# Nightmare-n/GD-MAE

Hardware: AMD Instinct MI355X
Metric: MAE pre-train frames/sec (Waymo-shape, 180k pts, 75% mask) (higher is better)
Workload: dtype bf16

## Files before the change

### gd-mae_amd/csrc/chamfer.hip

```cpp
#include "common.h"

struct GtParams {
  float lo[3], vs[3];
  int ncols;
  int K;
};

__global__ __launch_bounds__(256) void k_group_gt(const float* __restrict__ pts, const int* __restrict__ pt_off,
                                                  const int* __restrict__ csr, const long long* __restrict__ voxel_coords,
                                                  int M, GtParams P, float* __restrict__ gt, int* __restrict__ gidx) {
  const int lane = threadIdx.x & (GD_WAVE - 1);
  const int wib = threadIdx.x / GD_WAVE;
  for (int p = blockIdx.x * 4 + wib; p < M; p += gridDim.x * 4) {
    const int off = pt_off[p];
    const int cnt = pt_off[p + 1] - off;
    const long long* vc = voxel_coords + 4ll * p;
    const float cx = __fadd_rn(__fmul_rn(__fadd_rn((float)vc[3], 0.5f), P.vs[0]), P.lo[0]);
    const float cy = __fadd_rn(__fmul_rn(__fadd_rn((float)vc[2], 0.5f), P.vs[1]), P.lo[1]);
    const float cz = __fadd_rn(__fmul_rn(__fadd_rn((float)vc[1], 0.5f), P.vs[2]), P.lo[2]);
    for (int k = lane; k < P.K; k += GD_WAVE) {
      const int src = k < cnt ? k : k % cnt;
      const int pid = csr[off + src];
      const float* r = pts + (long long)pid * P.ncols;
      float* o = gt + ((long long)p * P.K + k) * 3;
      o[0] = __fsub_rn(r[1], cx);
      o[1] = __fsub_rn(r[2], cy);
      o[2] = __fsub_rn(r[3], cz);
      if (gidx) gidx[(long long)p * P.K + k] = pid;
    }
  }
}

extern "C" int gdmae_group_gt_points(const float* points, int n_cols, const int* pillar_pt_off, const int* pillar_pts,
                                     const long long* voxel_coords, int M, int K, const float* lo, const float* vs,
                                     float* gt_points, int* gt_index, void* stream) {
  if (M <= 0) return 0;
  GtParams P;
  for (int i = 0; i < 3; ++i) {
    P.lo[i] = lo[i];
    P.vs[i] = vs[i];
  }
  P.ncols = n_cols;
  P.K = K;
  int grid = gd_div_up(M, 4);
  if (grid > 8192) grid = 8192;
  hipLaunchKernelGGL(k_group_gt, dim3(grid), dim3(256), 0, (hipStream_t)stream, points, pillar_pt_off, pillar_pts,
                     voxel_coords, M, P, gt_points, gt_index);
  GD_LAUNCH_CHECK();
  return 0;
}

template <int P1MAX>
__global__ __launch_bounds__(256) void k_chamfer(const float* __restrict__ pred, const float* __restrict__ gt,
                                                 const float* __restrict__ w, int M, int P1, int P2,
                                                 float* __restrict__ term, float* __restrict__ dpred) {
  __shared__ float sx[4][P1MAX * 3];
  const int lane = threadIdx.x & (GD_WAVE - 1);
  const int wib = threadIdx.x / GD_WAVE;
  for (int m = blockIdx.x * 4 + wib; m < M; m += gridDim.x * 4) {
    const float wm = w[m];
    float* dp = dpred + (long long)m * P1 * 3;
    if (wm == 0.f) {
      for (int e = lane; e < P1 * 3; e += GD_WAVE) dp[e] = 0.f;
      if (lane == 0) term[m] = 0.f;
      continue;
    }
    for (int e = lane; e < P1 * 3; e += GD_WAVE) sx[wib][e] = pred[(long long)m * P1 * 3 + e];
    __builtin_amdgcn_wave_barrier();
    const bool has = lane < P2;
    float y0 = 0.f, y1 = 0.f, y2 = 0.f;
    if (has) {
      const float* g = gt + ((long long)m * P2 + lane) * 3;
      y0 = g[0];
      y1 = g[1];
      y2 = g[2];
    }
    float best = INFINITY;
    int besti = 0;
    float sumx = 0.f;
    const float cx = wm / (float)P1, cy = wm / (float)P2;
    for (int i = 0; i < P1; ++i) {
      const float x0 = sx[wib][3 * i], x1 = sx[wib][3 * i + 1], x2 = sx[wib][3 * i + 2];
      const float d0 = x0 - y0, d1 = x1 - y1, d2 = x2 - y2;
      const float d = has ? (d0 * d0 + d1 * d1 + d2 * d2) : INFINITY;
      if (d < best) {
        best = d;
        besti = i;
      }
      const float dmin = gd_wave_min(d);
      const unsigned long long bal = __ballot(d == dmin);
      const int jstar = __ffsll((long long)bal) - 1;
      sumx += dmin;
      const float g0 = 2.f * cx * __shfl(d0, jstar, GD_WAVE);
      const float g1 = 2.f * cx * __shfl(d1, jstar, GD_WAVE);
      const float g2 = 2.f * cx * __shfl(d2, jstar, GD_WAVE);
      if (lane == 0) {
        dp[3 * i] = g0;
        dp[3 * i + 1] = g1;
        dp[3 * i + 2] = g2;
      }
    }
    const float sumy = gd_wave_sum(has ? best : 0.f);
    if (lane == 0) term[m] = cx * sumx + cy * sumy;
    __builtin_amdgcn_fence(__ATOMIC_RELEASE, "workgroup");
    for (int i = 0; i < P1; ++i) {
      const bool mine = has && besti == i;
      const float x0 = sx[wib][3 * i], x1 = sx[wib][3 * i + 1], x2 = sx[wib][3 * i + 2];
      const float a0 = gd_wave_sum(mine ? 2.f * cy * (x0 - y0) : 0.f);
      const float a1 = gd_wave_sum(mine ? 2.f * cy * (x1 - y1) : 0.f);
      const float a2 = gd_wave_sum(mine ? 2.f * cy * (x2 - y2) : 0.f);
      if (lane == 0) {
        dp[3 * i] += a0;
        dp[3 * i + 1] += a1;
        dp[3 * i + 2] += a2;
      }
    }
    __builtin_amdgcn_wave_barrier();
  }
}

template <int N>
__device__ __forceinline__ void ch_tstep(unsigned long long (&k)[16], int mask, int lane) {
  const bool hi = (lane & mask) != 0;
#pragma unroll
  for (int t = 0; t < N; ++t) {
    const unsigned long long send = hi ? k[t] : k[t + N];
    const unsigned long long keep = hi ? k[t + N] : k[t];
    const unsigned long long recv = __shfl_xor(send, mask, GD_WAVE);
    k[t] = keep < recv ? keep : recv;
  }
}

__global__ __launch_bounds__(256) void k_chamfer16(const float* __restrict__ pred, const float* __restrict__ gt,
                                                   const float* __restrict__ w, int M, int P2, float* __restrict__ term,
                                                   float* __restrict__ dpred) {
  __shared__ float sx[4][48];
  __shared__ float sy[4][GD_WAVE * 3];
  __shared__ int sb[4][GD_WAVE];
  __shared__ float sg[4][48];
  const int lane = threadIdx.x & (GD_WAVE - 1);
  const int wib = threadIdx.x / GD_WAVE;
  const int my_i = ((lane >> 5) & 1) * 8 + ((lane >> 4) & 1) * 4 + ((lane >> 3) & 1) * 2 + ((lane >> 2) & 1);
  for (int m = blockIdx.x * 4 + wib; m < M; m += gridDim.x * 4) {
    const float wm = w[m];
    float* dp = dpred + (long long)m * 48;
    if (wm == 0.f) {
      if (lane < 48) dp[lane] = 0.f;
      if (lane == 0) term[m] = 0.f;
      continue;
    }
    if (lane < 48) sx[wib][lane] = pred[(long long)m * 48 + lane];
    const bool has = lane < P2;
    float y0 = 0.f, y1 = 0.f, y2 = 0.f;
    if (has) {
      const float* g = gt + ((long long)m * P2 + lane) * 3;
      y0 = g[0];
      y1 = g[1];
      y2 = g[2];
    }
    __builtin_amdgcn_wave_barrier();
    const float cx = wm / 16.f, cy = wm / (float)P2;
    unsigned long long k[16];
    float best = INFINITY;
    int besti = 0;
#pragma unroll
    for (int i = 0; i < 16; ++i) {
      const float d0 = sx[wib][3 * i] - y0, d1 = sx[wib][3 * i + 1] - y1, d2 = sx[wib][3 * i + 2] - y2;
      const float d = has ? (d0 * d0 + d1 * d1 + d2 * d2) : INFINITY;
      if (d < best) {
        best = d;
        besti = i;
      }
      k[i] = ((unsigned long long)__float_as_uint(d) << 32) | (unsigned)lane;
    }
    ch_tstep<8>(k, 32, lane);
    ch_tstep<4>(k, 16, lane);
    ch_tstep<2>(k, 8, lane);
    ch_tstep<1>(k, 4, lane);
    unsigned long long k0 = k[0];
    {
      unsigned long long o = __shfl_xor(k0, 2, GD_WAVE);
      k0 = k0 < o ? k0 : o;
      o = __shfl_xor(k0, 1, GD_WAVE);
      k0 = k0 < o ? k0 : o;
    }
    const float dmin = __uint_as_float((unsigned)(k0 >> 32));
    const int jstar = (int)(k0 & 63u);
    const float ys0 = __shfl(y0, jstar, GD_WAVE), ys1 = __shfl(y1, jstar, GD_WAVE), ys2 = __shfl(y2, jstar, GD_WAVE);
    if ((lane & 3) == 0) {
      sg[wib][3 * my_i] = 2.f * cx * (sx[wib][3 * my_i] - ys0);
      sg[wib][3 * my_i + 1] = 2.f * cx * (sx[wib][3 * my_i + 1] - ys1);
      sg[wib][3 * my_i + 2] = 2.f * cx * (sx[wib][3 * my_i + 2] - ys2);
    }
    const float sumx = gd_wave_sum((lane & 3) == 0 ? dmin : 0.f);
    const float sumy = gd_wave_sum(has ? best : 0.f);
    if (lane == 0) term[m] = cx * sumx + cy * sumy;
    sy[wib][3 * lane] = y0;
    sy[wib][3 * lane + 1] = y1;
    sy[wib][3 * lane + 2] = y2;
    sb[wib][lane] = has ? besti : -1;
    __builtin_amdgcn_fence(__ATOMIC_RELEASE, "workgroup");
    __builtin_amdgcn_wave_barrier();
    if (lane < 48) {
      const int i = lane / 3, c = lane - 3 * i;
      const float xi = sx[wib][lane];
      float acc = 0.f;
      for (int j = 0; j < P2; ++j) {
        const float v = 2.f * cy * (xi - sy[wib][3 * j + c]);
        acc += sb[wib][j] == i ? v : 0.f;
      }
      dp[lane] = sg[wib][lane] + acc;
    }
    __builtin_amdgcn_wave_barrier();
  }
}

extern "C" int gdmae_chamfer(const float* pred, const float* gt, const float* weights, int M, int P1, int P2, float* term,
                             float* dpred, void* stream) {
  if (M <= 0) return 0;
  GD_REQUIRE(P2 >= 1 && P2 <= GD_WAVE, "NUM_GT_POINTS must be <= 64 (one lane per ground-truth point)");
  GD_REQUIRE(P1 >= 1 && P1 <= 64, "NUM_PRD_POINTS must be <= 64");
  int grid = gd_div_up(M, 4);
  if (grid > 8192) grid = 8192;
  if (P1 == 16)
    hipLaunchKernelGGL(k_chamfer16, dim3(grid), dim3(256), 0, (hipStream_t)stream, pred, gt, weights, M, P2, term, dpred);
  else
    hipLaunchKernelGGL((k_chamfer<64>), dim3(grid), dim3(256), 0, (hipStream_t)stream, pred, gt, weights, M, P1, P2, term,
                       dpred);
  GD_LAUNCH_CHECK();
  return 0;
}
```

### gd-mae_amd/csrc/conv_tiles.hip

```cpp
#include "conv_tiles.h"

typedef float f32x16 __attribute__((ext_vector_type(16)));
typedef __bf16 bf16x8 __attribute__((ext_vector_type(8)));
typedef _Float16 f16x8 __attribute__((ext_vector_type(8)));
union CtFrag {
  uint4 q;
  bf16x8 v;
  f16x8 h;
};

#define CT_C 128
#define CT_SITE_PITCH 272
#ifndef CT_CH
#define CT_CH 128
#endif
#ifndef CT_RING
#define CT_RING 8
#endif
#define CT_HALVES (CT_C / CT_CH)
#define CT_KS (CT_CH / 16)
#define CT_NSTEP (9 * CT_KS)
#define CT_CPS (CT_CH / 8)
#define CT_PSITE (CT_CH * 2 + 16)
#define CT_ROW_PITCH (CT_CH == 128 ? 2944 : 1664)
// ... 423 lines not shown
    const int r0 = blockIdx.x * chunk, r1 = r0 + chunk < n_act ? r0 + chunk : n_act;
    float a0 = 0.f, a1 = 0.f, a2 = 0.f, a3 = 0.f;
    int r = r0;
    for (; r + 15 < r1; r += 16) {
      float v[16];
#pragma unroll
      for (int u = 0; u < 16; ++u) v[u] = part[(long long)(r + u) * 256 + tid];
#pragma unroll
      for (int u = 0; u < 16; u += 4) {
        a0 += v[u];
        a1 += v[u + 1];
        a2 += v[u + 2];
        a3 += v[u + 3];
      }
    }
    for (; r + 3 < r1; r += 4) {
      a0 += part[(long long)r * 256 + tid];
      a1 += part[(long long)(r + 1) * 256 + tid];
      a2 += part[(long long)(r + 2) * 256 + tid];
      a3 += part[(long long)(r + 3) * 256 + tid];
    }
    for (; r < r1; ++r) a0 += part[(long long)r * 256 + tid];
    red[(long long)blockIdx.x * 256 + tid] = (a0 + a1) + (a2 + a3);
    return;
  }
  __shared__ int cnt[9];
  if (tid < 9) cnt[tid] = 0;
  __syncthreads();
  int c[9];
#pragma unroll
  for (int k = 0; k < 9; ++k) c[k] = 0;
  for (int i0 = tid; i0 < n_act; i0 += 8 * 256) {
   int tl[8];
#pragma unroll
   for (int u = 0; u < 8; ++u) tl[u] = tile_list[i0 + u * 256 < n_act ? i0 + u * 256 : n_act - 1];
#pragma unroll
   for (int u = 0; u < 8; ++u) {
    if (i0 + u * 256 >= n_act) continue;
    const int tile = tl[u];
    const int tx = tile % TW, ty = (tile / TW) % TH;
    const int y0 = ty * 8, y1 = y0 + 8 < H ? y0 + 8 : H, x0 = tx * 8, x1 = x0 + 8 < W ? x0 + 8 : W;
    const int ry[3] = {y0 == 0 ? 1 : 0, 0, y1 == H ? 1 : 0};
    const int rx[3] = {x0 == 0 ? 1 : 0, 0, x1 == W ? 1 : 0};
    const int my = (y1 - y0) - ry[0] - ry[2], mx = (x1 - x0) - rx[0] - rx[2];
#pragma unroll
    for (int cy = 0; cy < 3; ++cy)
#pragma unroll
      for (int cx = 0; cx < 3; ++cx) c[cy * 3 + cx] += (cy == 1 ? my : ry[cy]) * (cx == 1 ? mx : rx[cx]);
   }
  }
#pragma unroll
  for (int k = 0; k < 9; ++k)
    if (c[k]) atomicAdd(&cnt[k], c[k]);
  __syncthreads();
  const int stat = tid >> 7, ch = tid & 127;
  double acc = 0.0;
#pragma unroll
  for (int cy = 0; cy < 3; ++cy)
#pragma unroll
    for (int cx = 0; cx < 3; ++cx) {
      const long long total = (long long)B * (cy == 1 ? H - 2 : 1) * (cx == 1 ? W - 2 : 1);
      const double n = (double)(total - cnt[cy * 3 + cx]);
      const double v = (double)ct_bf2f(ybg[(cy * 3 + cx) * CT_C + ch]);
      acc += n * (stat ? v * v : v);
    }
  const float hi = (float)acc;
  red[(long long)CT_NRED * 256 + tid] = hi;
  red[(long long)(CT_NRED + 1) * 256 + tid] = (float)(acc - (double)hi);
}

int gd_bn_fold_from_partials(hipStream_t st, const float* part, int nblk, int C, double count, const float* gamma,
                             const float* beta, double eps, double momentum, float* running_mean, float* running_var,
                             long long* num_batches, double* stats, float* ab, float* mv);

extern "C" size_t gdmae_conv3x3_tiles_workspace_bytes(int n_act) {
  return gd_align((size_t)(n_act > 0 ? n_act : 1) * 256 * sizeof(float)) + gd_align((size_t)(CT_NRED + 2) * 256 * sizeof(float));
}

extern "C" int gdmae_conv3x3_tiles_fwd(const void* const* P, const int* const* maps, const float* const* a, const float* const* b,
                                       const int* strides, int k, const void* Wp, const void* ybg, const int* tile_list, int n_act,
                                       int B, int H, int W, void* Yc, const float* gamma, const float* beta, double eps,
                                       double momentum, float* running_mean, float* running_var, long long* num_batches,
                                       double* stats, float* ab, float* mv, void* workspace, void* stream) {
  GD_REQUIRE(k >= 1 && k <= CT_MAX_SRC, "conv3x3_tiles: 1..3 source stages");
  GD_REQUIRE(H >= 2 && W >= 2, "conv3x3_tiles: map too small");
  hipStream_t st = (hipStream_t)stream;
  CtArgs A;
  A.k = k;
  for (int g = 0; g < CT_MAX_SRC; ++g) {
    if (g < k) {
      const int s = strides[g];
      GD_REQUIRE((s == 1 || s == 2 || s == 4 || s == 8) && H % s == 0 && W % s == 0, "conv3x3_tiles: stride");
      A.src[g].P = (const unsigned short*)P[g];
      A.src[g].map = maps[g];
      A.src[g].a = a[g];
      A.src[g].b = b[g];
      A.src[g].ls = s == 1 ? 0 : (s == 2 ? 1 : (s == 4 ? 2 : 3));
    } else {
      A.src[g].P = nullptr; A.src[g].map = nullptr; A.src[g].a = nullptr; A.src[g].b = nullptr; A.src[g].ls = 0;
    }
  }
  A.Wp = (const uint4*)Wp;
  A.tile_list = tile_list;
  A.n_act = n_act;
  A.H = H; A.W = W; A.TH = (H + 7) / 8; A.TW = (W + 7) / 8;
  A.Yc = (unsigned short*)Yc;
  GdArena ar(workspace, gdmae_conv3x3_tiles_workspace_bytes(n_act));
  float* part = ar.take<float>((size_t)(n_act > 0 ? n_act : 1) * 256);
  float* red = ar.take<float>((size_t)(CT_NRED + 2) * 256);
  A.part = part;
  if (n_act > 0) {
    static bool once = false;
    if (!once) {
      GD_CHECK(hipFuncSetAttribute((const void*)k_conv3x3_tiles, hipFuncAttributeMaxDynamicSharedMemorySize, CT_LDS_BYTES));
      once = true;
    }
    hipLaunchKernelGGL(k_conv3x3_tiles, dim3((n_act + CT_TPW - 1) / CT_TPW), dim3(CT_THREADS), CT_LDS_BYTES, st, A);
    GD_LAUNCH_CHECK();
  }
  hipLaunchKernelGGL(k_ct_stats_reduce, dim3(CT_NRED + 1), dim3(256), 0, st, (const float*)part, n_act, tile_list,
                     (const unsigned short*)ybg, B, H, W, A.TH, A.TW, red);
  GD_LAUNCH_CHECK();
  return gd_bn_fold_from_partials(st, red, CT_NRED + 2, CT_C, (double)B * H * W, gamma, beta, eps, momentum, running_mean,
                                  running_var, num_batches, stats, ab, mv);
}

template <int ES>
__global__ __launch_bounds__(256) void k_tiles_gather_rows(const void* __restrict__ Yc, GdTiles T, const int* __restrict__ cell,
                                                           long long n, int H, int W, int C, uint4* __restrict__ out) {
  const int cv = C * ES / 16;
  const long long total = n * cv;
  for (long long i = blockIdx.x * (long long)blockDim.x + threadIdx.x; i < total; i += (long long)gridDim.x * blockDim.x) {
    const long long r = total < (1ll << 31) ? (long long)((unsigned)i / (unsigned)cv) : i / cv;
    const int v = (int)(i - r * cv);
    const int s = cell[r];
    const int x = s % W, q = s / W, y = q % H, b = q / H;
    out[i] = ((const uint4*)gd_y_row<ES>(Yc, T, b, y, x, H, W, C))[v];
  }
}

extern "C" int gdmae_tiles_gather_rows(const void* Yc, const int* tile_slot, const void* ybg, const int* cell, long long n, int H,
                                       int W, int C, int elem_bytes, void* out, void* stream) {
  GD_REQUIRE(tile_slot != nullptr && (elem_bytes == 2 || elem_bytes == 4) && (C * elem_bytes) % 16 == 0, "tiles_gather_rows");
  if (n <= 0) return 0;
  GdTiles T{tile_slot, ybg, (H + 7) / 8, (W + 7) / 8};
  long long g = (n * (C * elem_bytes / 16) + 255) / 256;
  if (g > 16384) g = 16384;
  if (elem_bytes == 2) hipLaunchKernelGGL(k_tiles_gather_rows<2>, dim3((int)g), dim3(256), 0, (hipStream_t)stream, Yc, T, cell, n, H, W, C, (uint4*)out);
  else hipLaunchKernelGGL(k_tiles_gather_rows<4>, dim3((int)g), dim3(256), 0, (hipStream_t)stream, Yc, T, cell, n, H, W, C, (uint4*)out);
  GD_LAUNCH_CHECK();
  return 0;
}

template <int ES>
__global__ __launch_bounds__(256) void k_tiles_to_dense(const void* __restrict__ Yc, GdTiles T, int B, int H, int W, int C,
                                                        uint4* __restrict__ out) {
  const int cv = C * ES / 16;
  const long long total = (long long)B * H * W * cv;
  for (long long i = blockIdx.x * (long long)blockDim.x + threadIdx.x; i < total; i += (long long)gridDim.x * blockDim.x) {
    const long long s = i / cv;
    const int v = (int)(i % cv);
    const int x = (int)(s % W);
    const long long q = s / W;
    const int y = (int)(q % H), b = (int)(q / H);
    out[i] = ((const uint4*)gd_y_row<ES>(Yc, T, b, y, x, H, W, C))[v];
  }
}

__global__ __launch_bounds__(256) void k_tiles_to_dense_affine_relu(const void* __restrict__ Yc, GdTiles T, int B, int H, int W, int C,
                                                                    const float* __restrict__ a, const float* __restrict__ bsh,
                                                                    float* __restrict__ out) {
  const int cv = C / 8;
  const long long total = (long long)B * H * W * cv;
  const unsigned total32 = (unsigned)total, ucv = (unsigned)cv, uW = (unsigned)W, uH = (unsigned)H;
  for (unsigned i = blockIdx.x * blockDim.x + threadIdx.x; i < total32; i += gridDim.x * blockDim.x) {
    const unsigned s32 = i / ucv;
    const int v = (int)(i - s32 * ucv);
    const unsigned q32 = s32 / uW;
    const int x = (int)(s32 - q32 * uW);
    const unsigned b32 = q32 / uH;
    const int y = (int)(q32 - b32 * uH), b = (int)b32;
    const long long s = s32;
    const uint4 u = ((const uint4*)gd_y_row<2>(Yc, T, b, y, x, H, W, C))[v];
    float f[8];
    ct_unpack8(u, f);
    const float4 a0 = *(const float4*)(a + 8 * v), a1 = *(const float4*)(a + 8 * v + 4);
    const float4 b0 = *(const float4*)(bsh + 8 * v), b1 = *(const float4*)(bsh + 8 * v + 4);
    float4 o0, o1;
    o0.x = fmaxf(fmaf(a0.x, f[0], b0.x), 0.f); o0.y = fmaxf(fmaf(a0.y, f[1], b0.y), 0.f);
    o0.z = fmaxf(fmaf(a0.z, f[2], b0.z), 0.f); o0.w = fmaxf(fmaf(a0.w, f[3], b0.w), 0.f);
    o1.x = fmaxf(fmaf(a1.x, f[4], b1.x), 0.f); o1.y = fmaxf(fmaf(a1.y, f[5], b1.y), 0.f);
    o1.z = fmaxf(fmaf(a1.z, f[6], b1.z), 0.f); o1.w = fmaxf(fmaf(a1.w, f[7], b1.w), 0.f);
    typedef float f4v __attribute__((ext_vector_type(4)));
    __builtin_nontemporal_store(f4v{o0.x, o0.y, o0.z, o0.w}, (f4v*)(out + s * C + 8 * v));
    __builtin_nontemporal_store(f4v{o1.x, o1.y, o1.z, o1.w}, (f4v*)(out + s * C + 8 * v + 4));
  }
}

extern "C" int gdmae_tiles_to_dense_affine_relu(const void* Yc, const int* tile_slot, const void* ybg, int B, int H, int W, int C, const float* a,
                                                const float* b, float* out, void* stream) {
  GD_REQUIRE(tile_slot != nullptr && C % 8 == 0 && a != nullptr && b != nullptr, "tiles_to_dense_affine_relu");
  GD_REQUIRE((long long)B * H * W * (C / 8) < (1ll << 31), "tiles_to_dense_affine_relu: B H W C / 8 must fit 31 bits");
  GdTiles T{tile_slot, ybg, (H + 7) / 8, (W + 7) / 8};
  hipLaunchKernelGGL(k_tiles_to_dense_affine_relu, dim3(16384), dim3(256), 0, (hipStream_t)stream, Yc, T, B, H, W, C, a, b, out);
  GD_LAUNCH_CHECK();
  return 0;
}

extern "C" int gdmae_tiles_to_dense(const void* Yc, const int* tile_slot, const void* ybg, int B, int H, int W, int C, int elem_bytes,
                                    void* out, void* stream) {
  GD_REQUIRE(tile_slot != nullptr && (elem_bytes == 2 || elem_bytes == 4) && (C * elem_bytes) % 16 == 0, "tiles_to_dense");
  GdTiles T{tile_slot, ybg, (H + 7) / 8, (W + 7) / 8};
  if (elem_bytes == 2) hipLaunchKernelGGL(k_tiles_to_dense<2>, dim3(16384), dim3(256), 0, (hipStream_t)stream, Yc, T, B, H, W, C, (uint4*)out);
  else hipLaunchKernelGGL(k_tiles_to_dense<4>, dim3(16384), dim3(256), 0, (hipStream_t)stream, Yc, T, B, H, W, C, (uint4*)out);
  GD_LAUNCH_CHECK();
  return 0;
}
```

### gd-mae_amd/csrc/decoder.hip

```cpp
#include "common.h"
#include "conv_tiles.h"

__device__ inline float dec_bf2f(unsigned short h) { return __uint_as_float(((unsigned)h) << 16); }
__device__ inline unsigned short dec_f2bf(float f) { return gd_to_bf16(f); }
template <bool BF>
__device__ inline float dec_ld(const void* p, long long i) {
  return BF ? dec_bf2f(((const unsigned short*)p)[i]) : ((const float*)p)[i];
}
template <bool BF>
__device__ inline void dec_st(void* p, long long i, float v) {
  if (BF) ((unsigned short*)p)[i] = dec_f2bf(v);
  else ((float*)p)[i] = v;
}

template <bool BF>
__device__ inline void dec_ld8(const void* p, long long i, float (&v)[8]) {
  if (BF) {
    const uint4 q = *reinterpret_cast<const uint4*>((const unsigned short*)p + i);
    const unsigned w[4] = {q.x, q.y, q.z, q.w};
#pragma unroll
    for (int j = 0; j < 4; ++j) {
      v[2 * j] = __uint_as_float(w[j] << 16);
      v[2 * j + 1] = __uint_as_float(w[j] & 0xFFFF0000u);
    }
// ... 504 lines not shown
    ia[j] = fabsf(av[j]) >= 1e-30f ? 1.f / av[j] : 0.f;
  }
  for (long long p = r0 + tr; p < r1; p += rows_per_iter) {
    const long long q = p * C + c;
    float ov[8], gv[8];
    dec_ld8<false>(out, q, ov);
    dec_ld8<false>(dout, q, gv);
#pragma unroll
    for (int j = 0; j < 8; ++j)
      if (ov[j] > 0.f) {
        const float xr = (ov[j] - bv[j]) * ia[j];
        const bool recon = ia[j] != 0.f && (fabsf(bv[j]) + ov[j]) * fabsf(ia[j]) <= GD_SEGMAX_RECON_ULPS * fabsf(xr);
        const float xv = recon ? xr : dec_ld<XBF>(x, (long long)arg[q + j] * C + c + j);
        s0[j] += gv[j];
        s1[j] = fmaf(gv[j], xv, s1[j]);
      }
  }
#pragma unroll
  for (int j = 0; j < 8; ++j) {
    sh[(tr * 2 + 0) * C + c + j] = s0[j];
    sh[(tr * 2 + 1) * C + c + j] = s1[j];
  }
  __syncthreads();
  for (int q = threadIdx.x; q < 2 * C; q += 256) {
    float acc = 0.f;
    for (int rr = 0; rr < rows_per_iter; ++rr) acc += sh[rr * 2 * C + q];
    part[(long long)blockIdx.x * 2 * C + q] = acc;
  }
}

extern "C" int gdmae_segmax_bwd_stats(const void* x, int x_bf16, const float* out, const int* arg, const float* dout,
                                      long long M, int C, const float* a, const float* b,
                                      double* sums , void* workspace, void* stream) {
  GD_REQUIRE(C >= 1 && C <= 256, "C <= 256");
  hipStream_t st = (hipStream_t)stream;
  int nblk = (int)(M / 32 > 512 ? 512 : (M / 32 > 0 ? M / 32 : 1));
  const int rpi = 256 / C > 0 ? 256 / C : 1;
  const size_t lds = (size_t)rpi * 2 * C * sizeof(float);
  float* part = (float*)workspace;
  if (a && b && C % 8 == 0 && 256 % (C / 8) == 0) {
    const size_t lds8 = (size_t)(256 / (C / 8)) * 2 * C * sizeof(float);
    if (x_bf16)
      hipLaunchKernelGGL((k_segmax_bwd_stats_v8<true>), dim3(nblk), dim3(256), lds8, st, x, out, arg, dout, M, C, a, b, part);
    else
      hipLaunchKernelGGL((k_segmax_bwd_stats_v8<false>), dim3(nblk), dim3(256), lds8, st, x, out, arg, dout, M, C, a, b, part);
  } else if (x_bf16)
    hipLaunchKernelGGL((k_segmax_bwd_stats<true>), dim3(nblk), dim3(256), lds, st, x, out, arg, dout, M, C, part);
  else
    hipLaunchKernelGGL((k_segmax_bwd_stats<false>), dim3(nblk), dim3(256), lds, st, x, out, arg, dout, M, C, part);
  GD_LAUNCH_CHECK();
  hipLaunchKernelGGL(k_partials_to_f64, dim3(gd_div_up(2 * C, 16)), dim3(256), 0, st, part, nblk, 2 * C, sums);
  GD_LAUNCH_CHECK();
  return 0;
}

extern "C" int gdmae_segmax_bn_bwd(const void* x, int x_bf16, const float* out, const int* arg, const float* dout,
                                   const int* inverse32, long long N, int C, const float* a, const float* c0, const float* c1,
                                   void* dx, int dx_bf16, void* stream) {
  if (N <= 0) return 0;
  hipStream_t st = (hipStream_t)stream;
  const dim3 grid(dec_grid(N * C)), block(256);
  const bool v8 = C % 8 == 0;
  const dim3 grid8(dec_grid(N * C / 8));
#define GD_SB(XB, OB)                                                                                                              \
  do {                                                                                                                             \
    if (v8) hipLaunchKernelGGL((k_segmax_bn_bwd_v8<XB, OB>), grid8, block, 0, st, x, out, arg, dout, inverse32, N, C, a, c0, c1, dx); \
    else hipLaunchKernelGGL((k_segmax_bn_bwd<XB, OB>), grid, block, 0, st, x, out, arg, dout, inverse32, N, C, a, c0, c1, dx);      \
  } while (0)
  if (x_bf16) { if (dx_bf16) GD_SB(true, true); else GD_SB(true, false); }
  else { if (dx_bf16) GD_SB(false, true); else GD_SB(false, false); }
#undef GD_SB
  GD_LAUNCH_CHECK();
  return 0;
}

template <bool BF>
__global__ __launch_bounds__(256) void k_conv_grad_taps(const void* __restrict__ Ymap, GdTiles T, const float* __restrict__ k0,
                                                        const float* __restrict__ k1, const float* __restrict__ rows,
                                                        const int* __restrict__ cell2pillar, const int* __restrict__ site,
                                                        long long n, int H, int W, int C, void* __restrict__ out) {
  const int cv = C >> 3;
  const long long total = n * 9 * cv;
  for (long long i = blockIdx.x * (long long)blockDim.x + threadIdx.x; i < total; i += (long long)gridDim.x * blockDim.x) {
    const int v = (int)(i % cv);
    const long long tk = i / cv;
    const int k = (int)(tk % 9);
    const long long t = tk / 9;
    const int s = site[t];
    const int x = s % W;
    const int r = s / W;
    const int y = r % H;
    const int uy = y - (k / 3 - 1), ux = x - (k % 3 - 1);
    float o[8];
#pragma unroll
    for (int j = 0; j < 8; ++j) o[j] = 0.f;
    if (uy >= 0 && uy < H && ux >= 0 && ux < W) {
      const long long u = (long long)(r - y + uy) * W + ux;
      const int c0 = v * 8;
      float yv[8];
      const char* yrow = gd_y_row<BF ? 2 : 4>(Ymap, T, (r - y) / H, uy, ux, H, W, C);
      if (BF) {
        const uint4 q = ((const uint4*)yrow)[c0 >> 3];
        const unsigned w4[4] = {q.x, q.y, q.z, q.w};
#pragma unroll
        for (int j = 0; j < 4; ++j) {
          yv[2 * j] = __uint_as_float(w4[j] << 16);
          yv[2 * j + 1] = __uint_as_float(w4[j] & 0xFFFF0000u);
        }
      } else {
        const float4 q0 = ((const float4*)yrow)[c0 >> 2], q1 = ((const float4*)yrow)[(c0 >> 2) + 1];
        yv[0] = q0.x; yv[1] = q0.y; yv[2] = q0.z; yv[3] = q0.w; yv[4] = q1.x; yv[5] = q1.y; yv[6] = q1.z; yv[7] = q1.w;
      }
      const float4 ka = ((const float4*)k0)[c0 >> 2], kb = ((const float4*)k0)[(c0 >> 2) + 1];
      const float4 la = ((const float4*)k1)[c0 >> 2], lb = ((const float4*)k1)[(c0 >> 2) + 1];
      const float kk0[8] = {ka.x, ka.y, ka.z, ka.w, kb.x, kb.y, kb.z, kb.w};
      const float kk1[8] = {la.x, la.y, la.z, la.w, lb.x, lb.y, lb.z, lb.w};
#pragma unroll
      for (int j = 0; j < 8; ++j) o[j] = fmaf(kk1[j], yv[j], kk0[j]);
      const int p = cell2pillar[u];
      if (p >= 0) {
        const float4 r0 = ((const float4*)rows)[((long long)p * C + c0) >> 2], r1 = ((const float4*)rows)[(((long long)p * C + c0) >> 2) + 1];
        o[0] += r0.x; o[1] += r0.y; o[2] += r0.z; o[3] += r0.w; o[4] += r1.x; o[5] += r1.y; o[6] += r1.z; o[7] += r1.w;
      }
    }
    if (BF) {
      uint4 q;
      q.x = dec_f2bf(o[0]) | ((unsigned)dec_f2bf(o[1]) << 16);
      q.y = dec_f2bf(o[2]) | ((unsigned)dec_f2bf(o[3]) << 16);
      q.z = dec_f2bf(o[4]) | ((unsigned)dec_f2bf(o[5]) << 16);
      q.w = dec_f2bf(o[6]) | ((unsigned)dec_f2bf(o[7]) << 16);
      ((uint4*)out)[i] = q;
    } else {
      ((float4*)out)[2 * i] = make_float4(o[0], o[1], o[2], o[3]);
      ((float4*)out)[2 * i + 1] = make_float4(o[4], o[5], o[6], o[7]);
    }
  }
}

extern "C" int gdmae_conv3x3_grad_taps(const void* Ymap, int y_bf16, const int* tile_slot, const void* ybg, const float* k0,
                                       const float* k1, const float* rows, const int* cell2pillar, const int* site, long long n,
                                       int H, int W, int C, void* out, void* stream) {
  GD_REQUIRE(C % 8 == 0, "C must be a multiple of 8");
  if (n <= 0) return 0;
  long long g = (n * 9 * (C / 8) + 255) / 256;
  if (g > 65536) g = 65536;
  const GdTiles T{tile_slot, ybg, (H + 7) / 8, (W + 7) / 8};
  if (y_bf16) hipLaunchKernelGGL(k_conv_grad_taps<true>, dim3((int)g), dim3(256), 0, (hipStream_t)stream, Ymap, T, k0, k1, rows, cell2pillar, site, n, H, W, C, out);
  else hipLaunchKernelGGL(k_conv_grad_taps<false>, dim3((int)g), dim3(256), 0, (hipStream_t)stream, Ymap, T, k0, k1, rows, cell2pillar, site, n, H, W, C, out);
  GD_LAUNCH_CHECK();
  return 0;
}

#define DEC_BORDER_CHUNKS 64
template <bool BF>
__global__ __launch_bounds__(256) void k_border_partial(const void* __restrict__ Y, GdTiles T, const float* __restrict__ rows,
                                                        const int* __restrict__ pillar_cell, int M, int B, int H, int W, int C,
                                                        float* __restrict__ part_edge, float* __restrict__ part_rows) {
  extern __shared__ float sh[];
  const int cv = C >> 3;
  if ((int)blockIdx.x < 4 * B) {
    const int e = blockIdx.x / B, b = blockIdx.x % B;
    const int len = e < 2 ? W : H;
    const int slots = 256 / cv;
    const int tr = threadIdx.x / cv, c = (threadIdx.x % cv) << 3;
    float acc[8];
#pragma unroll
    for (int j = 0; j < 8; ++j) acc[j] = 0.f;
    if (tr < slots)
      for (int i0 = tr; i0 < len; i0 += 4 * slots) {
        float v[4][8];
#pragma unroll
        for (int u = 0; u < 4; ++u) {
          const int i = i0 + u * slots < len ? i0 + u * slots : len - 1;
          const int y = e == 0 ? 0 : (e == 1 ? H - 1 : i);
          const int x = e == 2 ? 0 : (e == 3 ? W - 1 : i);
          dec_ld8<BF>(gd_y_row<BF ? 2 : 4>(Y, T, b, y, x, H, W, C), c, v[u]);
        }
#pragma unroll
        for (int u = 0; u < 4; ++u) {
          const bool ok = i0 + u * slots < len;
#pragma unroll
          for (int j = 0; j < 8; ++j) acc[j] = ok ? acc[j] + v[u][j] : acc[j];
        }
      }
    if (tr < slots) {
#pragma unroll
      for (int j = 0; j < 8; ++j) sh[tr * C + c + j] = acc[j];
    }
    __syncthreads();
    for (int q = threadIdx.x; q < C; q += 256) {
      float s = 0.f;
      for (int r = 0; r < slots; ++r) s += sh[r * C + q];
      part_edge[(long long)blockIdx.x * C + q] = s;
    }
    return;
  }
  const int lane = threadIdx.x & 63;
  const int bb = (int)blockIdx.x - 4 * B;
  const int chunk = bb >> 1;
  const int reg = (bb & 1) * 4 + (threadIdx.x >> 6);
  const int per = ((M + DEC_BORDER_CHUNKS - 1) / DEC_BORDER_CHUNKS + 63) / 64 * 64;
  const int pb = chunk * per, pe = pb + per < M ? pb + per : M;
  float acc[4] = {0.f, 0.f, 0.f, 0.f};
  for (int p0 = pb; p0 < pe; p0 += 64) {
    const int p = p0 + lane;
    bool in = false;
    if (p < pe) {
      const int cell = pillar_cell[p];
      const int x = cell % W, y = (cell / W) % H;
      const bool y0 = y == 0, yl = y == H - 1, x0 = x == 0, xl = x == W - 1;
      in = reg == 0 ? y0 : reg == 1 ? yl : reg == 2 ? x0 : reg == 3 ? xl : reg == 4 ? (y0 && x0) : reg == 5 ? (y0 && xl)
                                                                         : reg == 6 ? (yl && x0) : (yl && xl);
    }
    unsigned long long m = __ballot(in);
    while (m) {
      const int k = __ffsll((long long)m) - 1;
      m &= m - 1;
      const float* rp = rows + (long long)(p0 + k) * C;
#pragma unroll
      for (int j = 0; j < 4; ++j)
        if (lane + 64 * j < C) acc[j] += rp[lane + 64 * j];
    }
  }
#pragma unroll
  for (int j = 0; j < 4; ++j)
    if (lane + 64 * j < C) part_rows[((long long)chunk * 8 + reg) * C + lane + 64 * j] = acc[j];
}

template <bool BF>
__global__ __launch_bounds__(256) void k_border_final(const void* __restrict__ Y, GdTiles T, const float* __restrict__ part_edge,
                                                      const float* __restrict__ part_rows, int B, int H, int W, int C,
                                                      double* __restrict__ out) {
  for (int q = blockIdx.x * blockDim.x + threadIdx.x; q < 8 * C; q += gridDim.x * blockDim.x) {
    const int r = q / C, c = q % C;
    double s = 0.0;
    if (r < 4) {
      for (int b = 0; b < B; ++b) s += (double)part_edge[(long long)(r * B + b) * C + c];
    } else {
      const int y = (r == 4 || r == 5) ? 0 : H - 1, x = (r == 4 || r == 6) ? 0 : W - 1;
      for (int b = 0; b < B; ++b) s += (double)dec_ld<BF>(gd_y_row<BF ? 2 : 4>(Y, T, b, y, x, H, W, C), c);
    }
    out[q] = s;
    double t = 0.0;
    for (int ch = 0; ch < DEC_BORDER_CHUNKS; ++ch) t += (double)part_rows[(long long)ch * 8 * C + q];
    out[8 * C + q] = t;
  }
}

extern "C" size_t gdmae_border_sums_workspace_bytes(int B, int C) {
  return (size_t)(4 * B + 8 * DEC_BORDER_CHUNKS) * C * sizeof(float);
}

extern "C" int gdmae_border_sums(const void* Y, int y_bf16, const int* tile_slot, const void* ybg, const float* rows,
                                 const int* pillar_cell, int M, int B, int H, int W, int C, double* out ,
                                 void* workspace, void* stream) {
  const GdTiles T{tile_slot, ybg, (H + 7) / 8, (W + 7) / 8};
  GD_REQUIRE(C % 8 == 0 && C <= 256 && 256 % (C / 8) == 0, "border_sums: C in {64, 128, 256}");
  hipStream_t st = (hipStream_t)stream;
  float* part_edge = (float*)workspace;
  float* part_rows = part_edge + (size_t)4 * B * C;
  const size_t lds = (size_t)(256 / (C / 8)) * C * sizeof(float);
  if (y_bf16) hipLaunchKernelGGL((k_border_partial<true>), dim3(4 * B + 2 * DEC_BORDER_CHUNKS), dim3(256), lds, st, Y, T, rows, pillar_cell, M, B, H, W, C, part_edge, part_rows);
  else hipLaunchKernelGGL((k_border_partial<false>), dim3(4 * B + 2 * DEC_BORDER_CHUNKS), dim3(256), lds, st, Y, T, rows, pillar_cell, M, B, H, W, C, part_edge, part_rows);
  GD_LAUNCH_CHECK();
  if (y_bf16) hipLaunchKernelGGL((k_border_final<true>), dim3(gd_div_up(8 * C, 256)), dim3(256), 0, st, Y, T, part_edge, part_rows, B, H, W, C, out);
  else hipLaunchKernelGGL((k_border_final<false>), dim3(gd_div_up(8 * C, 256)), dim3(256), 0, st, Y, T, part_edge, part_rows, B, H, W, C, out);
  GD_LAUNCH_CHECK();
  return 0;
}

__global__ __launch_bounds__(256) void k_dec_region_S(const double* __restrict__ stats2, const float* __restrict__ ab2,
                                                      const double* __restrict__ st2, const float* __restrict__ k01,
                                                      const double* __restrict__ reg, const double* __restrict__ tap_region,
                                                      const double* __restrict__ cnt, double R, int C2, double* __restrict__ S) {
  const int o = blockIdx.x * blockDim.x + threadIdx.x;
  if (o >= C2) return;
  const double k0 = (double)k01[o], k1 = (double)k01[C2 + o];
  double regD[9];
#pragma unroll
  for (int r = 0; r < 9; ++r) {
    const double y = r == 0 ? stats2[o] * R : reg[(r - 1) * C2 + o];
    const double rr = r == 0 ? (double)ab2[o] * st2[o] : reg[(8 + r - 1) * C2 + o];
    regD[r] = cnt[r] * k0 + y * k1 + rr;
  }
#pragma unroll
  for (int k = 0; k < 9; ++k) {
    double a = 0.0;
#pragma unroll
    for (int r = 0; r < 9; ++r) a += tap_region[k * 9 + r] * regD[r];
    S[k * C2 + o] = a;
  }
}

template <bool BF>
__global__ __launch_bounds__(128) void k_dec_region_W(const double* __restrict__ S, const float* __restrict__ conv_w,
                                                      const void* __restrict__ bgz, int C2, int Cin, float* __restrict__ dWk,
                                                      void* __restrict__ Wd, double* __restrict__ tot_part) {
  const int i = blockIdx.x * 128 + threadIdx.x, oc = blockIdx.y * 8;
  if (i >= Cin) return;
  const double bg = (double)dec_ld<BF>(bgz, i);
  double acc = 0.0;
  for (int oo = 0; oo < 8; ++oo) {
    const int o = oc + oo;
    const float* w = conv_w + ((long long)o * Cin + i) * 9;
#pragma unroll
    for (int k = 0; k < 9; ++k) {
      const float wv = w[k];
      const double s = S[k * C2 + o];
      acc += s * (double)wv;
      const long long e = ((long long)k * C2 + o) * Cin + i;
      dWk[e] = (float)(s * bg);
      dec_st<BF>(Wd, e, wv);
    }
  }
  tot_part[(long long)blockIdx.y * Cin + i] = acc;
}

__global__ __launch_bounds__(256) void k_dec_region_tot(const double* __restrict__ tot_part, int nchunk, int Cin,
                                                        double* __restrict__ tot) {
  const int i = blockIdx.x * blockDim.x + threadIdx.x;
  if (i >= Cin) return;
  double a = 0.0;
  for (int c = 0; c < nchunk; ++c) a += tot_part[(long long)c * Cin + i];
  tot[i] = a;
}

extern "C" size_t gdmae_decoder_region_workspace_bytes(int C2, int Cin) { return (size_t)(C2 / 8 + 1) * Cin * sizeof(double); }

extern "C" int gdmae_decoder_region_algebra(const double* stats2, const float* ab2, const double* st2, const float* k01,
                                            const double* reg, const double* tap_region, const double* cnt, double R, int C2,
                                            int Cin, const float* conv_w, const void* bgz, int cdt_bf16, double* S, double* tot,
                                            float* dWk, void* Wd, void* workspace, void* stream) {
  GD_REQUIRE(C2 > 0 && C2 % 8 == 0 && Cin > 0, "decoder region algebra: C2 must be a multiple of 8");
  hipStream_t st = (hipStream_t)stream;
  hipLaunchKernelGGL(k_dec_region_S, dim3(gd_div_up(C2, 256)), dim3(256), 0, st, stats2, ab2, st2, k01, reg, tap_region, cnt, R, C2, S);
  GD_LAUNCH_CHECK();
  const dim3 grid(gd_div_up(Cin, 128), C2 / 8);
  double* part = (double*)workspace;
  if (cdt_bf16) hipLaunchKernelGGL((k_dec_region_W<true>), grid, dim3(128), 0, st, (const double*)S, conv_w, bgz, C2, Cin, dWk, Wd, part);
  else hipLaunchKernelGGL((k_dec_region_W<false>), grid, dim3(128), 0, st, (const double*)S, conv_w, bgz, C2, Cin, dWk, Wd, part);
  GD_LAUNCH_CHECK();
  hipLaunchKernelGGL(k_dec_region_tot, dim3(gd_div_up(Cin, 256)), dim3(256), 0, st, (const double*)part, C2 / 8, Cin, tot);
  GD_LAUNCH_CHECK();
  return 0;
}


__global__ __launch_bounds__(256) void k_decoder_dy(const unsigned short* __restrict__ Yc, const int* __restrict__ tile_list, int n_act,
                                                    const float* __restrict__ k0, const float* __restrict__ k1,
                                                    const float* __restrict__ rows, const int* __restrict__ cell2pillar, int H, int W,
                                                    int TH, int TW, int C, unsigned short* __restrict__ dYc) {
  const unsigned cv = (unsigned)C >> 3;
  const unsigned total = (unsigned)n_act * GD_TILE_SITES * cv;
  for (unsigned i = blockIdx.x * blockDim.x + threadIdx.x; i < total; i += gridDim.x * blockDim.x) {
    const unsigned row32 = i / cv;
    const int v = (int)(i - row32 * cv);
    const long long row = row32;
    const int slot = (int)(row32 >> 6), loc = (int)(row32 & 63);
    const int tile = tile_list[slot];
    const int tx = tile % TW, r = tile / TW, ty = r % TH, b = r / TH;
    const int y = ty * GD_TILE + (loc >> 3), x = tx * GD_TILE + (loc & 7);
    uint4 q = make_uint4(0u, 0u, 0u, 0u);
    if (y < H && x < W) {
      const int c0 = v * 8;
      const uint4 yq = reinterpret_cast<const uint4*>(Yc + row * C)[v];
      const unsigned w4[4] = {yq.x, yq.y, yq.z, yq.w};
      float yv[8], o[8];
#pragma unroll
      for (int j = 0; j < 4; ++j) {
        yv[2 * j] = __uint_as_float(w4[j] << 16);
        yv[2 * j + 1] = __uint_as_float(w4[j] & 0xFFFF0000u);
      }
      const float4 ka = ((const float4*)k0)[c0 >> 2], kb = ((const float4*)k0)[(c0 >> 2) + 1];
      const float4 la = ((const float4*)k1)[c0 >> 2], lb = ((const float4*)k1)[(c0 >> 2) + 1];
      const float kk0[8] = {ka.x, ka.y, ka.z, ka.w, kb.x, kb.y, kb.z, kb.w};
      const float kk1[8] = {la.x, la.y, la.z, la.w, lb.x, lb.y, lb.z, lb.w};
#pragma unroll
      for (int j = 0; j < 8; ++j) o[j] = fmaf(kk1[j], yv[j], kk0[j]);
      const int p = cell2pillar[((long long)b * H + y) * W + x];
      if (p >= 0) {
        const float4 r0 = ((const float4*)rows)[((long long)p * C + c0) >> 2], r1 = ((const float4*)rows)[(((long long)p * C + c0) >> 2) + 1];
        o[0] += r0.x; o[1] += r0.y; o[2] += r0.z; o[3] += r0.w; o[4] += r1.x; o[5] += r1.y; o[6] += r1.z; o[7] += r1.w;
      }
      q.x = dec_f2bf(o[0]) | ((unsigned)dec_f2bf(o[1]) << 16);
      q.y = dec_f2bf(o[2]) | ((unsigned)dec_f2bf(o[3]) << 16);
      q.z = dec_f2bf(o[4]) | ((unsigned)dec_f2bf(o[5]) << 16);
      q.w = dec_f2bf(o[6]) | ((unsigned)dec_f2bf(o[7]) << 16);
    }
    reinterpret_cast<uint4*>(dYc + row * C)[v] = q;
  }
}
extern "C" int gdmae_decoder_dy(const void* Yc, const int* tile_list, int n_act, const float* k0, const float* k1, const float* rows,
                                const int* cell2pillar, int H, int W, int C, void* dYc, void* stream) {
  GD_REQUIRE(C % 8 == 0, "decoder_dy: C must be a multiple of 8");
  if (n_act <= 0) return 0;
  GD_REQUIRE((long long)n_act * GD_TILE_SITES * (C / 8) < (1ll << 31), "decoder_dy: active tiles x 64 x C / 8 must fit 31 bits");
  long long g = ((long long)n_act * GD_TILE_SITES * (C / 8) + 255) / 256;
  if (g > 65536) g = 65536;
  hipLaunchKernelGGL(k_decoder_dy, dim3((int)g), dim3(256), 0, (hipStream_t)stream, (const unsigned short*)Yc, tile_list, n_act, k0, k1, rows,
                     cell2pillar, H, W, (H + 7) / 8, (W + 7) / 8, C, (unsigned short*)dYc);
  GD_LAUNCH_CHECK();
  return 0;
}

__global__ __launch_bounds__(256) void k_decoder_site_rulebook(const int* __restrict__ site, const int* __restrict__ n_dev, int sites_per_tok,
                                                               const int* __restrict__ tile_slot, int H, int W, int TH, int TW,
                                                               int* __restrict__ nbr) {
  const long long total = (long long)(*n_dev) * sites_per_tok * 9;
  for (long long i = blockIdx.x * (long long)blockDim.x + threadIdx.x; i < total; i += (long long)gridDim.x * blockDim.x) {
    const long long t = total < (1ll << 31) ? (long long)((unsigned)i / 9u) : i / 9;
    const int k = (int)(i - t * 9);
    const int s = site[t];
    const int x = s % W, r = s / W, y = r % H, b = r / H;
    const int uy = y - (k / 3 - 1), ux = x - (k % 3 - 1);
    int v = -1;
    if (uy >= 0 && uy < H && ux >= 0 && ux < W) {
      const int sl = tile_slot[(b * TH + (uy >> 3)) * TW + (ux >> 3)];
      if (sl >= 0) v = sl * GD_TILE_SITES + (uy & 7) * GD_TILE + (ux & 7);
    }
    nbr[i] = v;
  }
}
int gd_decoder_site_rulebook(const int* site, const int* n_dev, int sites_per_tok, long long cap_sites, const int* tile_slot, int H, int W,
                             int* nbr, hipStream_t st) {
  long long g = (cap_sites * 9 + 255) / 256;
  if (g > 4096) g = 4096;
  if (g < 1) g = 1;
  hipLaunchKernelGGL(k_decoder_site_rulebook, dim3((int)g), dim3(256), 0, st, site, n_dev, sites_per_tok, tile_slot, H, W, (H + 7) / 8,
                     (W + 7) / 8, nbr);
  GD_LAUNCH_CHECK();
  return 0;
}
extern "C" int gdmae_decoder_site_rulebook(const int* site, const int* n_dev, int sites_per_tok, long long cap_sites, const int* tile_slot,
                                           int H, int W, int* nbr, void* stream) {
  return gd_decoder_site_rulebook(site, n_dev, sites_per_tok, cap_sites, tile_slot, H, W, nbr, (hipStream_t)stream);
}
```

### gd-mae_amd/gdmae_hip/decoder.py

```python
from __future__ import annotations

import os
from collections import namedtuple
from dataclasses import dataclass
from types import SimpleNamespace
from typing import Optional

import torch
import torch.nn.functional as F

from . import bn as gbn
from . import lib as L
from . import ops, packing
from . import plan as gplan
from . import timing

CONV_BWD = os.environ.get("GDMAE_DEC_BWD", "implicit")
BLOCK_BWD = os.environ.get("GDMAE_DEC_BLOCK", "1")



def colstats(x2d: torch.Tensor):
    R, C = x2d.shape
    assert x2d.is_contiguous() and x2d.dtype in (torch.float32, torch.bfloat16)
    out = torch.empty(2 * C, dtype=torch.float64, device=x2d.device)
    ws = torch.empty(L.load().gdmae_colstats_workspace_bytes(C), dtype=torch.uint8, device=x2d.device)
    L.call("gdmae_colstats", L.ptr(x2d), R, C, int(x2d.dtype == torch.bfloat16), L.ptr(out), L.ptr(ws), L.stream())
    return out[:C], out[C:]


def _gather_slice(table2d, idx, col0, ncol):
    es = table2d.element_size()
    out = torch.empty(idx.numel(), ncol, dtype=table2d.dtype, device=table2d.device)
    L.call("gdmae_gather_rows_strided", L.ptr(table2d), L.ptr(idx), idx.numel(), ncol * es, table2d.shape[1] * es,
           col0 * es, L.ptr(out), L.stream())
    return out


def _scatter_slice(src2d, idx, table2d, col0):
    es = table2d.element_size()
    src2d = src2d.contiguous()
    assert src2d.dtype == table2d.dtype
    L.call("gdmae_scatter_rows_strided", L.ptr(src2d), L.ptr(idx), idx.numel(), src2d.shape[1] * es,
           table2d.shape[1] * es, col0 * es, L.ptr(table2d), L.stream())


def _bf(t):
    return int(t.dtype == torch.bfloat16)


_TAP_REGION = torch.zeros(9, 9, dtype=torch.float64)
for _ky in (-1, 0, 1):
    for _kx in (-1, 0, 1):
        _k = (_ky + 1) * 3 + (_kx + 1)
        _TAP_REGION[_k, 0] = 1
        if _ky:
            _TAP_REGION[_k, 1 if _ky < 0 else 2] = -1
        if _kx:
            _TAP_REGION[_k, 3 if _kx < 0 else 4] = -1
        if _ky and _kx:
            _TAP_REGION[_k, 5 + (0 if _ky < 0 else 2) + (0 if _kx < 0 else 1)] = 1


_REGION_CONSTS = {}


def _region_consts(dev, B, H, W):
    key = (dev, B, H, W)
    if key not in _REGION_CONSTS:
        R = B * H * W
        cnt = torch.tensor([R, B * W, B * W, B * H, B * H, B, B, B, B], dtype=torch.float64)
        _REGION_CONSTS[key] = (_TAP_REGION.to(dev), cnt.to(dev))
    return _REGION_CONSTS[key]


@dataclass(frozen=True, eq=False)
class TileConv:
    tiles: gplan.DecoderTiles
    maps: list
    ups: list


@dataclass(frozen=True, eq=False)
class DecoderGeom:
    B: int
    H: int
    W: int
    eps1: float
    eps2: float
    cdt: torch.dtype
    tile_conv: Optional[TileConv] = None


_Forward = namedtuple("_Forward", "y2 yrows stats2 ab2 mv2 Z tile_slot ybg bgz")


def _forward_tiles(geom, pre_conv_hook, conv_w, gamma2, beta2, pillar_cell, Ps, widths, ab_l, bn2):
    B, H, W, cdt, tc = geom.B, geom.H, geom.W, geom.cdt, geom.tile_conv
    dt, k, dev = tc.tiles, len(Ps), Ps[0].device
    lib = L.load()
    Cin = sum(widths)
    C2 = 128
    Wp = torch.empty(lib.gdmae_conv3x3_tiles_packed_bytes(k), dtype=torch.uint8, device=dev)
    bgz = torch.empty(Cin, dtype=cdt, device=dev)
    ybg = torch.empty(9, C2, dtype=cdt, device=dev)
    a_l, b_l = [ab[:w] for ab, w in zip(ab_l, widths)], [ab[w:] for ab, w in zip(ab_l, widths)]
    L.call("gdmae_conv3x3_tiles_pack", L.ptr(conv_w), C2, Cin, L.host_ptrs(b_l), k, L.ptr(Wp), L.ptr(bgz), L.ptr(ybg),
           L.stream())
    y2 = torch.empty(max(dt.n_act, 1) * 64, C2, dtype=cdt, device=dev)
    stats2 = torch.empty(2 * C2, dtype=torch.float64, device=dev)
    ab2 = torch.empty(2 * C2, dtype=torch.float32, device=dev)
    mv2 = torch.empty(2 * C2, dtype=torch.float32, device=dev)
    ws = torch.empty(lib.gdmae_conv3x3_tiles_workspace_bytes(dt.n_act), dtype=torch.uint8, device=dev)
    rm, rv, nb, mom = gbn.running_stats(bn2)
    flops = 2.0 * dt.n_act * 64 * C2 * 9 * Cin
    if pre_conv_hook is not None:
        pre_conv_hook()
    with timing.kernel("k_conv3x3_tiles", dt.n_act * 64 * (Cin + C2) * 2, flops,
                       {"dense_equivalent_TFLOPs_per_launch": round(2.0 * B * H * W * C2 * 9 * Cin / 1e12, 4), "active_tiles": dt.n_act}):
        L.call("gdmae_conv3x3_tiles_fwd", L.host_ptrs([P.contiguous() for P in Ps]), L.host_ptrs(tc.maps), L.host_ptrs(a_l),
               L.host_ptrs(b_l), L.host_i32(tc.ups), k, L.ptr(Wp), L.ptr(ybg), L.ptr(dt.tile_list), dt.n_act, B, H, W,
               L.ptr(y2), L.ptr(gamma2), L.ptr(beta2), float(geom.eps2), mom, L.ptr(rm), L.ptr(rv), L.ptr(nb), L.ptr(stats2),
               L.ptr(ab2), L.ptr(mv2), L.ptr(ws), L.stream())
    M = pillar_cell.numel()
    yrows = torch.empty(M, C2, dtype=cdt, device=dev)
    L.call("gdmae_tiles_gather_rows", L.ptr(y2), L.ptr(dt.tile_slot), L.ptr(ybg), L.ptr(pillar_cell), M, H, W, C2, 2,
           L.ptr(yrows), L.stream())
    return _Forward(y2, yrows, stats2, ab2, mv2, None, dt.tile_slot, ybg, bgz)


def _forward_dense_map(geom, conv_w, gamma2, beta2, pillar_cell, sites, Ps, widths, ab_l, bn2):
    B, H, W, cdt = geom.B, geom.H, geom.W, geom.cdt
    R = B * H * W
    bgz = torch.relu(torch.cat([ab[w:] for ab, w in zip(ab_l, widths)])).to(cdt)
    Z = torch.empty(R, sum(widths), dtype=cdt, device=Ps[0].device)
    L.call("gdmae_fill_rows", L.ptr(bgz), R, Z.shape[1], Z.element_size(), L.ptr(Z), L.stream())
    col = 0
    for P, st, ab, w in zip(Ps, sites, ab_l, widths):
        L.call("gdmae_rows_affine_relu_scatter", L.ptr(P), _bf(P), L.ptr(st), P.shape[0], w, L.ptr(ab), L.ptr(ab[w:]), L.ptr(Z), _bf(Z),
               Z.shape[1], col, L.stream())
        col += w
    from . import dense as gdense
    C2o = conv_w.shape[0]
    if cdt == torch.bfloat16 and Z.shape[1] % 64 == 0 and conv_w.dtype == torch.float32:
        y2 = gdense.Conv3x3Dense.apply(Z.view(B, H, W, -1).permute(0, 3, 1, 2), conv_w.detach(), None, 1, None).permute(0, 2, 3, 1)
    elif cdt == torch.float32 and Z.shape[1] % 64 == 0:
        y2 = gdense.conv3x3_f32_rows(Z.view(B, H, W, -1), conv_w.detach().float().contiguous(), None, 1)[..., :C2o]
    else:
        wc = ops.shadow(conv_w, cdt)
        with torch.autocast("cuda", enabled=False):
            y2 = F.conv2d(Z.view(B, H, W, -1).permute(0, 3, 1, 2), wc, None, 1, 1).permute(0, 2, 3, 1)
    if not y2.is_contiguous():
        y2 = y2.contiguous()
    y2 = y2.view(R, -1)
    stats2, ab2, mv2 = gbn.fold(y2, R, gamma2, beta2, geom.eps2, bn2)
    yrows = ops.gather_rows_raw(y2, pillar_cell)
    return _Forward(y2, yrows, stats2, ab2, mv2, Z, None, None, bgz)


def _backward_schedule(geom, conv_w, sites, Ps, widths, fwd):
    C2 = fwd.y2.shape[1]
    native = conv_w.dtype == torch.float32 and conv_w.is_contiguous() and C2 % 8 == 0
    tc = geom.tile_conv
    if not (CONV_BWD == "implicit" and fwd.tile_slot is not None and fwd.y2.dtype == torch.bfloat16 and native and C2 == 128
            and all(w == 128 for w in widths) and tc is not None):
        return native, ["taps"] * len(widths)
    stage_bwd = []
    for P, st, u in zip(Ps, sites, tc.ups):
        n, u = P.shape[0], int(u)
        block = (BLOCK_BWD != "0" and u in (2, 4) and P.dtype == torch.bfloat16 and P.is_contiguous() and st.numel() >= n
                 and int(L.load().gdmae_decoder_block_dw_workspace_bytes(n, u)) > 0)
        stage_bwd.append("block" if block else "rulebook")
    return native, stage_bwd


def _save(ctx, **named):
    ctx.saved_names = [(name, len(v) if isinstance(v, (list, tuple)) else None) for name, v in named.items()]
    ctx.save_for_backward(*[t for v in named.values() for t in (v if isinstance(v, (list, tuple)) else (v,))])


def _saved(ctx) -> SimpleNamespace:
    sv, out, j = ctx.saved_tensors, SimpleNamespace(), 0
    for name, n in ctx.saved_names:
        setattr(out, name, sv[j] if n is None else sv[j:j + n])
        j += 1 if n is None else n
    return out


def _bn2_backward(s, dout, R, direct):
    yrows, ab2 = s.yrows, s.ab2
    M, C2 = yrows.shape
    dev = yrows.device
    dout = dout.float().contiguous()
    st2 = torch.empty(3 * C2, dtype=torch.float64, device=dev)
    ws = torch.empty(L.load().gdmae_rows_bwd_stats_workspace_bytes(C2), dtype=torch.uint8, device=dev)
    L.call("gdmae_rows_bwd_stats", L.ptr(yrows), _bf(yrows), None, M, C2, L.ptr(ab2), L.ptr(ab2[C2:]), L.ptr(dout), 0, C2, 0,
           L.ptr(st2), L.ptr(ws), L.stream())
    dgamma2, dbeta2, k01 = gbn.bwd_coeffs(st2, 3, s.stats2, ab2, s.gamma2, R, None, direct)
    zero = torch.zeros(2 * C2, dtype=torch.float32, device=dev)
    rows = torch.empty(M, C2, dtype=torch.float32, device=dev)
    L.call("gdmae_rows_bwd", L.ptr(yrows), _bf(yrows), None, M, C2, L.ptr(ab2), L.ptr(ab2[C2:]), L.ptr(zero), L.ptr(zero[C2:]),
           L.ptr(dout), 0, C2, 0, L.ptr(rows), 0, L.stream())
    return rows, st2, k01, dgamma2, dbeta2


def _region_sums(s, rows, B, H, W):
    y2 = s.y2
    C2 = y2.shape[1]
    reg = torch.empty(16, C2, dtype=torch.float64, device=y2.device)
    ws = torch.empty(L.load().gdmae_border_sums_workspace_bytes(B, C2), dtype=torch.uint8, device=y2.device)
    L.call("gdmae_border_sums", L.ptr(y2), _bf(y2), L.ptr(s.tile_slot), L.ptr(s.ybg), L.ptr(rows), L.ptr(s.pillar_cell),
           rows.shape[0], B, H, W, C2, L.ptr(reg), L.ptr(ws), L.stream())
    return reg



def region_algebra_native(stats2, ab2, st2, k01, reg, tap_region, cnt, R, conv_w, bgz, cdt):
    C2, Cin, dev = conv_w.shape[0], bgz.numel(), conv_w.device
    S = torch.empty(9, C2, dtype=torch.float64, device=dev)
    tot = torch.empty(Cin, dtype=torch.float64, device=dev)
    dWk = torch.empty(9, C2, Cin, dtype=torch.float32, device=dev)
    Wd = torch.empty(9, C2, Cin, dtype=cdt, device=dev)
    ws = torch.empty(L.load().gdmae_decoder_region_workspace_bytes(C2, Cin), dtype=torch.uint8, device=dev)
    L.call("gdmae_decoder_region_algebra", L.ptr(stats2), L.ptr(ab2), L.ptr(st2), L.ptr(k01), L.ptr(reg),
           L.ptr(tap_region), L.ptr(cnt), float(R), C2, Cin, L.ptr(conv_w), L.ptr(bgz), _bf(Wd), L.ptr(S), L.ptr(tot),
           L.ptr(dWk), L.ptr(Wd), L.ptr(ws), L.stream())
    return S, tot, dWk, Wd


def region_algebra_torch(stats2, ab2, st2, k01, reg, tap_region, cnt, R, conv_w, bgz, cdt):
    C2, Cin = conv_w.shape[0], bgz.numel()
    k0, k1 = k01[:C2].double(), k01[C2:].double()
    regY = torch.cat([(stats2[:C2] * R)[None], reg[:8]])
    regR = torch.cat([(ab2[:C2].double() * st2[:C2])[None], reg[8:]])
    regD = cnt[:, None] * k0[None, :] + regY * k1[None, :] + regR
    S = tap_region @ regD
    Wk = conv_w.permute(2, 3, 0, 1).reshape(9, C2, Cin)
    tot = torch.einsum('ko,koi->i', S, Wk.double()).contiguous()
    dWk = (S[:, :, None] * bgz.double()[None, None, :]).to(torch.promote_types(torch.float32, conv_w.dtype))
    Wd = Wk.to(cdt)
    return S, tot, dWk, Wd


def _stage_dx_spconv(b, i, col):
    n, w, C2 = b.Ps[i].shape[0], b.widths[i], b.y2.shape[1]
    nbr = b.tiles.nbr[i]
    assert nbr.shape[0] == n, (nbr.shape, n)
    dX = torch.empty(n, w, dtype=b.cdt, device=b.y2.device)
    L.call("gdmae_spconv", L.ptr(b.dYc), 0, L.ptr(nbr), b.packed.data_ptr() + i * 9 * w * C2 * 2, n, C2, w, L.ptr(dX), 8, L.stream())
    return dX


def _stage_grads_block(b, i, col):
    dX = _stage_dx_spconv(b, i, col)
    P, ab, w, u = b.Ps[i], b.ab_l[i], b.widths[i], int(b.ups[i])
    n = P.shape[0]
    ws = torch.empty(int(L.load().gdmae_decoder_block_dw_workspace_bytes(n, u)), dtype=torch.uint8, device=P.device)
    L.call("gdmae_decoder_block_dw", L.ptr(P), L.ptr(ab), L.ptr(ab[w:]), L.ptr(b.bgz[col:col + w]), L.ptr(b.sites[i]), n, u, L.ptr(b.dYc),
           L.ptr(b.tile_slot), b.H, b.W, L.ptr(b.dWk), b.bgz.numel(), col, L.ptr(ws), L.stream())
    return dX, None


def _stage_grads_rulebook(b, i, col):
    dX = _stage_dx_spconv(b, i, col)
    P, ab, w, C2 = b.Ps[i], b.ab_l[i], b.widths[i], b.y2.shape[1]
    n = P.shape[0]
    n_pad = int(L.load().gdmae_tap_dw_rows(n, w, C2))
    Zd = torch.empty(n_pad, w, dtype=b.cdt, device=P.device)
    L.call("gdmae_rows_affine_relu_sub", L.ptr(P), _bf(P), None, n, w, L.ptr(ab), L.ptr(ab[w:]), L.ptr(b.bgz[col:col + w]), L.ptr(Zd),
           _bf(Zd), w, 0, L.stream())
    ws = torch.empty(L.load().gdmae_tap_dw_workspace_bytes(n, w, C2), dtype=torch.uint8, device=P.device)
    L.call("gdmae_tap_dw", L.ptr(Zd), n, n_pad, w, L.ptr(b.dYc), L.ptr(b.tiles.nbr[i]), C2, L.ptr(b.dWk), b.bgz.numel(), col, L.ptr(ws),
           L.stream())
    return dX, None


def _stage_grads_taps(b, i, col):
    P, ab, w, C2, cdt = b.Ps[i], b.ab_l[i], b.widths[i], b.y2.shape[1], b.cdt
    n, dev = P.shape[0], P.device
    G = torch.empty(n, 9 * C2, dtype=cdt, device=dev)
    with timing.kernel("k_conv_grad_taps", 2.0 * n * 9 * C2 * G.element_size()):
        L.call("gdmae_conv3x3_grad_taps", L.ptr(b.y2), _bf(b.y2), L.ptr(b.tile_slot), L.ptr(b.ybg), L.ptr(b.k01), L.ptr(b.k01[C2:]),
               L.ptr(b.rows), L.ptr(b.cell2pillar), L.ptr(b.sites[i]), n, b.H, b.W, C2, L.ptr(G), L.stream())
    dX = ops.mm(G, b.Wd[:, :, col:col + w].reshape(9 * C2, w))
    bg = b.bgz[col:col + w]
    if b.Z is not None:
        Zd = _gather_slice(b.Z, b.sites[i], col, w) - bg
    else:
        Zd = torch.empty(n, w, dtype=cdt, device=dev)
        L.call("gdmae_rows_affine_relu_sub", L.ptr(P), _bf(P), None, n, w, L.ptr(ab), L.ptr(ab[w:]), L.ptr(bg), L.ptr(Zd),
               _bf(Zd), w, 0, L.stream())
    return dX, ops.splitk_tn(G, Zd)


_STAGE_GRADS = {"block": _stage_grads_block, "rulebook": _stage_grads_rulebook, "taps": _stage_grads_taps}


def _stage_bn_backward(b, i, col, dX, R, direct):
    P, ab, w = b.Ps[i], b.ab_l[i], b.widths[i]
    n = P.shape[0]
    ws = torch.empty(L.load().gdmae_rows_bwd_stats_workspace_bytes(w), dtype=torch.uint8, device=P.device)
    L.call("gdmae_rows_bwd_stats", L.ptr(P), _bf(P), None, n, w, L.ptr(ab), L.ptr(ab[w:]), L.ptr(dX), _bf(dX), w, 0,
           None, L.ptr(ws), L.stream())
    dgamma, dbeta, c01 = gbn.bwd_coeffs((ws, L.load().gdmae_rows_bwd_stats_rows(n)), 3, b.stats_l[i], ab, b.gammas[i], R,
                                        b.tot[col:col + w], direct)
    dP = torch.empty_like(P)
    L.call("gdmae_rows_bwd", L.ptr(P), _bf(P), None, n, w, L.ptr(ab), L.ptr(ab[w:]), L.ptr(c01), L.ptr(c01[w:]), L.ptr(dX),
           _bf(dX), w, 0, L.ptr(dP), _bf(dP), L.stream())
    return dP, dgamma, dbeta


class DecoderHead(torch.autograd.Function):

    @staticmethod
    def forward(ctx, geom, pre_conv_hook, conv_w, gamma2, beta2, pillar_cell, cell2pillar, bn_mods, *args):
        R = geom.B * geom.H * geom.W
        k = len(args) // 4
        sites, Ps, gammas, betas = args[0::4], args[1::4], args[2::4], args[3::4]
        widths = [int(P.shape[1]) for P in Ps]
        bns = list(bn_mods) if bn_mods is not None else [None] * (k + 1)
        ab_l, stats_l, mv_out = [], [], []
        for i in range(k):
            stats, ab, mv = gbn.fold(Ps[i].contiguous(), R, gammas[i], betas[i], geom.eps1, bns[i])
            ab_l.append(ab), stats_l.append(stats)
            mv_out += [mv[:widths[i]], mv[widths[i]:]]
        use_tiles = (geom.tile_conv is not None and geom.cdt == torch.bfloat16 and all(w == 128 for w in widths) and conv_w.shape[0] == 128
                     and conv_w.dtype == torch.float32 and conv_w.is_contiguous() and all(P.dtype == torch.bfloat16 for P in Ps))
        if use_tiles:
            f = _forward_tiles(geom, pre_conv_hook, conv_w, gamma2, beta2, pillar_cell, Ps, widths, ab_l, bns[k])
        else:
            f = _forward_dense_map(geom, conv_w, gamma2, beta2, pillar_cell, sites, Ps, widths, ab_l, bns[k])
        M, C2 = f.yrows.shape
        out = torch.empty(M, C2, dtype=torch.float32, device=f.yrows.device)
        L.call("gdmae_rows_affine_relu_scatter", L.ptr(f.yrows), _bf(f.yrows), None, M, C2, L.ptr(f.ab2), L.ptr(f.ab2[C2:]), L.ptr(out), 0,
               C2, 0, L.stream())
        _save(ctx, sites=sites, Ps=Ps, ab_l=ab_l, stats_l=stats_l, gammas=[g.detach() for g in gammas], Z=f.Z, y2=f.y2, bgz=f.bgz,
              yrows=f.yrows, ab2=f.ab2, stats2=f.stats2, pillar_cell=pillar_cell, cell2pillar=cell2pillar, gamma2=gamma2.detach(),
              conv_w=conv_w.detach(), tile_slot=f.tile_slot, ybg=f.ybg)
        ctx.geom, ctx.widths = geom, widths
        ctx.native_region, ctx.stage_bwd = _backward_schedule(geom, conv_w, sites, Ps, widths, f)
        ctx.direct = [gbn.direct_pair(g, be) for g, be in zip(gammas, betas)] + [gbn.direct_pair(gamma2, beta2)]
        ctx.direct_w = ops.direct_grad(conv_w)
        ctx.conv_param = conv_w
        mean2, var2 = f.mv2[:C2], f.mv2[C2:]
        ctx.mark_non_differentiable(f.y2, mean2, var2, *mv_out, *([] if f.ybg is None else [f.ybg]))
        ctx.set_materialize_grads(False)
        return (out, f.y2, mean2, var2, *mv_out, f.ybg)

    @staticmethod
    def backward(ctx, dout, *_):
        geom, widths, stage_bwd = ctx.geom, ctx.widths, ctx.stage_bwd
        B, H, W = geom.B, geom.H, geom.W
        R, k = B * H * W, len(widths)
        b = _saved(ctx)
        b.H, b.W, b.cdt, b.widths = H, W, geom.cdt, widths
        b.rows, st2, b.k01, dgamma2, dbeta2 = _bn2_backward(b, dout, R, ctx.direct[k])
        reg = _region_sums(b, b.rows, B, H, W)
        tap_region, cnt = _region_consts(reg.device, B, H, W)
        algebra = region_algebra_native if ctx.native_region else region_algebra_torch
        S, b.tot, b.dWk, b.Wd = algebra(b.stats2, b.ab2, st2, b.k01, reg, tap_region, cnt, R, b.conv_w, b.bgz, geom.cdt)
        if stage_bwd[0] != "taps":
            b.packed = packing.decoder_conv_packed(ctx.conv_param, widths, ctx.direct_w is not None)
            if b.packed is None:
                stage_bwd = ["taps"] * k
            else:
                b.tiles, b.ups = geom.tile_conv.tiles, geom.tile_conv.ups
                if b.tiles.nbr is None:
                    b.tiles.nbr = gplan.decoder_site_rulebooks(b.tiles, b.sites, b.ups)
                C2 = b.y2.shape[1]
                b.dYc = torch.empty_like(b.y2)
                L.call("gdmae_decoder_dy", L.ptr(b.y2), L.ptr(b.tiles.tile_list), b.tiles.n_act, L.ptr(b.k01), L.ptr(b.k01[C2:]),
                       L.ptr(b.rows), L.ptr(b.cell2pillar), H, W, C2, L.ptr(b.dYc), L.stream())
        grads = [None] * 8
        dW_rows = []
        col = 0
        for i, w in enumerate(widths):
            dX, dW = _STAGE_GRADS[stage_bwd[i]](b, i, col)
            if dW is not None:
                dW_rows.append(dW)
            grads += [None, *_stage_bn_backward(b, i, col, dX, R, ctx.direct[i])]
            col += w
        dWk = b.dWk
        if dW_rows:
            dWk = dWk + torch.cat(dW_rows, dim=1).view(dWk.shape)
        dW = dWk.permute(1, 2, 0).reshape(b.conv_w.shape[0], b.conv_w.shape[1], 3, 3)
        if ctx.direct_w is not None:
            ctx.direct_w.add_(dW)
        else:
            grads[2] = dW.to(b.conv_w.dtype)
        grads[3], grads[4] = dgamma2, dbeta2
        return tuple(grads)


class DeconvRowsFn(torch.autograd.Function):

    @staticmethod
    def forward(ctx, x, weight, direct):
        cin, cout, s, _ = weight.shape
        n = x.shape[0]
        dev = x.device
        x = x.contiguous()
        nb = L.load().gdmae_deconv_rows_packed_bytes(cin, cout, s)
        pf = torch.empty(nb, dtype=torch.uint8, device=dev)
        pb = torch.empty(nb, dtype=torch.uint8, device=dev)
        L.call("gdmae_deconv_rows_pack", L.ptr(weight), cin, cout, s, L.ptr(pf), L.ptr(pb), L.stream())
        P = torch.empty(n * s * s, cout, dtype=torch.bfloat16, device=dev)
        L.call("gdmae_deconv_rows_fwd", L.ptr(x), n, cin, cout, s, L.ptr(pf), L.ptr(P), L.stream())
        ctx.save_for_backward(x, pb)
        ctx.meta = (cin, cout, s, direct)
        return P

    @staticmethod
    def backward(ctx, dP):
        x, pb = ctx.saved_tensors
        cin, cout, s, direct = ctx.meta
        n = x.shape[0]
        dP = dP.contiguous()
        if dP.dtype != torch.bfloat16:
            dP = dP.to(torch.bfloat16)
        dx = None
        if ctx.needs_input_grad[0]:
            dx = torch.empty(n, cin, dtype=torch.bfloat16, device=x.device)
            L.call("gdmae_deconv_rows_bwd_input", L.ptr(dP), n, cin, cout, s, L.ptr(pb), L.ptr(dx), L.stream())
        ws = torch.empty(L.load().gdmae_deconv_rows_dw_workspace_bytes(n, cin, cout, s), dtype=torch.uint8, device=x.device)
        L.call("gdmae_deconv_rows_bwd_weight", L.ptr(x), L.ptr(dP), n, cin, cout, s, L.ptr(direct), L.ptr(ws), L.stream())
        return dx, None, None


DECONV_ROWS = os.environ.get("GDMAE_DECONV_ROWS", "1") != "0"


def deconv_rows(x, deconv):
    w = deconv.weight
    s = int(deconv.stride[0])
    cin, cout = w.shape[0], w.shape[1]
    direct = ops.direct_grad(w)
    if (DECONV_ROWS and x.is_cuda and torch.is_autocast_enabled() and x.dtype == torch.bfloat16 and direct is not None and w.dtype == torch.float32
            and w.is_contiguous() and cin in (128, 256) and cout == 128 and s in (1, 2, 4) and x.shape[0] > 0):
        return DeconvRowsFn.apply(x, w, direct)
    wmat = w.permute(0, 2, 3, 1).reshape(cin, s * s * cout)
    return ops.linear(x, wmat.t()).view(-1, cout)


class PredHeadFn(torch.autograd.Function):

    @staticmethod
    def forward(ctx, x, weight, bias, direct):
        n, n_out = x.shape[0], weight.shape[0]
        x = x.contiguous()
        packed = torch.empty(L.load().gdmae_pred_head_packed_bytes(), dtype=torch.uint8, device=x.device)
        L.call("gdmae_pred_head_pack", L.ptr(weight), None if bias is None else L.ptr(bias), weight.shape[1], n_out, L.ptr(packed), L.stream())
        xb = torch.empty(n, x.shape[1], dtype=torch.bfloat16, device=x.device)
        y = torch.empty(n, n_out, dtype=torch.float32, device=x.device)
        L.call("gdmae_pred_head_fwd", L.ptr(x), n, n_out, L.ptr(packed), None, L.ptr(xb), L.ptr(y), L.stream())
        ctx.save_for_backward(xb, packed)
        ctx.meta = (n_out, direct, weight.shape, None if bias is None else bias.shape)
        return y

    @staticmethod
    def backward(ctx, dy):
        x, packed = ctx.saved_tensors
        n_out, direct, wshape, bshape = ctx.meta
        n = x.shape[0]
        dy = dy.contiguous()
        if dy.dtype not in (torch.bfloat16, torch.float32):
            dy = dy.float()
        f32 = dy.dtype == torch.float32
        dyb = torch.empty(dy.shape, dtype=torch.bfloat16, device=x.device) if f32 else None
        dx = torch.empty(x.shape, dtype=torch.float32, device=x.device) if ctx.needs_input_grad[0] else None
        if direct is not None:
            dW, db = direct
            ret = (None, None)
        else:
            dW = torch.zeros(wshape, dtype=torch.float32, device=x.device)
            db = None if bshape is None else torch.zeros(bshape, dtype=torch.float32, device=x.device)
            ret = (dW, db)
        ws = torch.empty(L.load().gdmae_pred_head_bwd_workspace_bytes(n), dtype=torch.uint8, device=x.device)
        scale = ops.LAZY_SCALE.pop(dy.data_ptr(), None) if f32 else None
        if scale is None and ops.LAZY_SCALE:
            raise RuntimeError("an unscaled Chamfer gradient was handed over (ops.LAZY_SCALE) but did not arrive here as the same tensor")
        L.call("gdmae_pred_head_bwd", L.ptr(dy), int(f32), None if dyb is None else L.ptr(dyb), None if scale is None else L.ptr(scale[0]),
               None if scale is None else L.ptr(scale[1]), L.ptr(x), n, n_out, L.ptr(packed),
               None if dx is None else L.ptr(dx), L.ptr(dW), None if db is None else L.ptr(db), L.ptr(ws), L.stream())
        return (dx, *ret, None)


def pred_head(x, linear):
    w, b = linear.weight, linear.bias
    if (DECONV_ROWS and x.is_cuda and torch.is_autocast_enabled() and x.dtype == torch.float32 and w.dtype == torch.float32 and w.is_contiguous()
            and w.shape[1] == 128 and 8 <= w.shape[0] <= 64 and w.shape[0] % 8 == 0 and x.shape[0] > 0):
        dw, db = ops.direct_grad(w), (ops.direct_grad(b) if b is not None else None)
        direct = (dw, db) if (dw is not None and (b is None or db is not None)) else None
        y = PredHeadFn.apply(x, w, b, direct)
        y._gd_pred_head = True
        return y
    return ops.linear(x, w, b)


def upsampled_sites(stage_plan, s: int, Y: int, X: int) -> torch.Tensor:
    if s == 1:
        return stage_plan.tok_cell
    pre = getattr(stage_plan, "_up_sites", None)
    if pre is not None and pre[0] == s and stage_plan.Y * s == Y and stage_plan.X * s == X:
        return pre[1]
    return gplan.upsample_cells(stage_plan.tok_cell, stage_plan.Y, stage_plan.X, s).reshape(-1).contiguous()


def expand_dense(y2, ybg, tiles, a2, b2, B, Y, X):
    R = B * Y * X
    C2 = y2.shape[1]
    compact = ybg is not None
    assert y2.shape[0] == (max(tiles.n_act, 1) * 64 if compact else R), (y2.shape, R, compact)
    if compact and y2.dtype == torch.bfloat16 and C2 % 8 == 0:
        dmap = torch.empty(R, C2, dtype=torch.float32, device=y2.device)
        L.call("gdmae_tiles_to_dense_affine_relu", L.ptr(y2), L.ptr(tiles.tile_slot), L.ptr(ybg), B, Y, X, C2,
               L.ptr(a2), L.ptr(b2), L.ptr(dmap), L.stream())
        return dmap.view(B, Y, X, -1).permute(0, 3, 1, 2)
    if compact:
        yd = torch.empty(R, C2, dtype=y2.dtype, device=y2.device)
        L.call("gdmae_tiles_to_dense", L.ptr(y2), L.ptr(tiles.tile_slot), L.ptr(ybg), B, Y, X, C2, y2.element_size(),
               L.ptr(yd), L.stream())
        y2 = yd
    return torch.relu(y2.float() * a2 + b2).view(B, Y, X, -1).permute(0, 3, 1, 2)


# ... 30 lines not shown
```

### gd-mae_amd/gdmae_hip/lib.py

```python
from __future__ import annotations

import ctypes as C
import os

import torch

_HERE = os.path.dirname(os.path.abspath(__file__))
LIB_PATH = os.path.abspath(os.path.join(_HERE, "..", "csrc", "libgdmae_hip.so"))
if os.environ.get("GDMAE_LIB"):
    LIB_PATH = os.path.abspath(os.environ["GDMAE_LIB"])


class GdmaeHipError(RuntimeError):
    pass


_P, _I, _L, _F, _D, _Z = C.c_void_p, C.c_int, C.c_longlong, C.c_float, C.c_double, C.c_size_t

SIGNATURES = {
    "gdmae_abi_version": (_I, []),
    "gdmae_target_arch": (C.c_char_p, []),
    "gdmae_last_error": (C.c_char_p, []),
    "gdmae_voxelize_workspace_bytes": (_Z, [_L, _I, _I, _I, _I]),
    "gdmae_voxelize": (_I, [_P, _L, _I, _P, _P, _P, _I, _P, _P, _P, _P, _P, _P, _P, _P, _P, _P, _P, _P, _P, _P, _Z, _P]),
    "gdmae_decorate_points": (_I, [_P, _P, _P, _P, _L, _I, _P, _P, _P, _P]),
    "gdmae_vfe_infer": (_I, [_P, _P, _P, _P, _L, _L, _I, _P, _P, _P, _P, _I, _P, _P, _I, _P, _P]),
    "gdmae_vfe_point_layer_workspace_bytes": (_Z, [_I]),
    "gdmae_pillar_major_rows": (_I, [_P, _I, _P, _P, _P, _L, _P, _P, _P]),
    "gdmae_vfe_point_layer_fwd": (_I, [_P, _P, _P, _P, _I, _L, _I, _P, _P, _P, _I, _P, _P, _D, _D, _P, _P, _P, _P, _P, _P, _P, _I, _P, _P]),
    "gdmae_vfe_point_layer_bwd": (_I, [_P, _P, _P, _P, _I, _L, _I, _P, _P, _P, _I, _P, _P, _P, _P, _I, _P, _P, _P, _I, _P, _P]),
    "gdmae_vfe_max_layer_workspace_bytes": (_Z, []),
    "gdmae_vfe_max_layer_fwd": (_I, [_P, _L, _P, _P, _P, _I, _P, _P, _D, _D, _P, _P, _P, _P, _P, _P, _P, _P, _P, _P]),
    "gdmae_vfe_max_layer_bwd": (_I, [_P, _L, _P, _P, _I, _P, _P, _P, _P, _P, _P, _P, _P, _P, _P, _P, _I, _P, _P]),
    "gdmae_vfe_max_layer_fwd_f16": (_I, [_P, _L, _P, _P, _P, _I, _P, _P, _D, _D, _P, _P, _P, _P, _P, _P, _P, _P, _P, _P]),
    "gdmae_vfe_max_layer_bwd_f16": (_I, [_P, _L, _P, _P, _I, _P, _P, _P, _P, _P, _P, _P, _P, _P, _P, _P, _I, _P, _P]),
    "gdmae_vfe_max_layer_vis_fwd": (_I, [_P, _L, _P, _P, _P, _L, _I, _P, _P, _D, _D, _P, _P, _P, _P, _P, _P, _P, _P, _P, _P]),
    "gdmae_vfe_max_layer_vis_fwd_f16": (_I, [_P, _L, _P, _P, _P, _L, _I, _P, _P, _D, _D, _P, _P, _P, _P, _P, _P, _P, _P, _P, _P]),
    "gdmae_vfe_max_layer_vis_bwd": (_I, [_P, _L, _P, _P, _P, _I, _I, _P, _P, _P, _P, _P, _P, _P, _P, _P, _P, _P, _I, _P, _P]),
    "gdmae_vfe_max_layer_vis_bwd_f16": (_I, [_P, _L, _P, _P, _P, _I, _I, _P, _P, _P, _P, _P, _P, _P, _P, _P, _P, _P, _I, _P, _P]),
    "gdmae_fill_rows": (_I, [_P, _L, _I, _I, _P, _P]),
    "gdmae_weighted_mean_finish": (_I, [_P, _P, _L, _P, _P]),
    "gdmae_decoder_region_workspace_bytes": (_Z, [_I, _I]),
    "gdmae_decoder_region_algebra": (_I, [_P, _P, _P, _P, _P, _P, _P, _D, _I, _I, _P, _P, _I, _P, _P, _P, _P, _P, _P]),
    "gdmae_segment_max": (_I, [_P, _P, _P, _I, _I, _P, _P, _P]),
    "gdmae_segment_max_bwd": (_I, [_P, _P, _P, _L, _I, _P, _P]),
    "gdmae_random_mask": (_I, [_P, _P, _I, _D, _P, _P, _P]),
    "gdmae_visible_tokens": (_I, [_P, _P, _P, _L, _L, _P, _P, _P, _P, _P, _P]),
    "gdmae_downsample_tokens": (_I, [_P, _P, _L, _I, _I, _I, _P, _P, _P, _P, _P, _P]),
    "gdmae_rulebook": (_I, [_P, _P, _L, _I, _I, _I, _I, _I, _P, _I, _P, _P]),
    "gdmae_window_workspace_bytes": (_Z, [_I, _I, _I, _I, _I]),
    "gdmae_window_partition": (_I, [_P, _I, _I, _I, _I, _I, _I, _I, _P, _P, _P, _P, _P, _P, _P, _P, _P, _P, _P, _P, _Z, _P]),
    "gdmae_gather_rows": (_I, [_P, _P, _L, _I, _P, _P]),
    "gdmae_scatter_rows": (_I, [_P, _P, _L, _I, _P, _P]),
    "gdmae_gather_rows_strided": (_I, [_P, _P, _L, _I, _I, _I, _P, _P]),
    "gdmae_scatter_rows_strided": (_I, [_P, _P, _L, _I, _I, _I, _P, _P]),
    "gdmae_colstats_workspace_bytes": (_Z, [_I]),
    "gdmae_colstats": (_I, [_P, _L, _I, _I, _P, _P, _P]),
    "gdmae_rows_affine_relu_scatter": (_I, [_P, _I, _P, _L, _I, _P, _P, _P, _I, _I, _I, _P]),
    "gdmae_rows_affine_relu_sub": (_I, [_P, _I, _P, _L, _I, _P, _P, _P, _P, _I, _I, _I, _P]),
    "gdmae_rows_affine_relu_add": (_I, [_P, _I, _L, _I, _P, _P, _P, _P, _I, _P]),
    "gdmae_rows_bwd_stats_workspace_bytes": (_Z, [_I]),
    "gdmae_rows_bwd_stats": (_I, [_P, _I, _P, _L, _I, _P, _P, _P, _I, _I, _I, _P, _P, _P]),
    "gdmae_bn_fold": (_I, [_P, _L, _I, _I, _D, _P, _P, _D, _D, _P, _P, _P, _P, _P, _P, _P, _P]),
    "gdmae_bn_bwd_coeffs": (_I, [_P, _I, _P, _P, _P, _I, _D, _P, _P, _P, _I, _P, _P]),
    "gdmae_rows_bwd_stats_rows": (_I, [_L]),
    "gdmae_bn_bwd_coeffs_rows": (_I, [_P, _I, _I, _P, _P, _P, _I, _D, _P, _P, _P, _I, _P, _P]),
    "gdmae_border_sums_workspace_bytes": (_Z, [_I, _I]),
    "gdmae_border_sums": (_I, [_P, _I, _P, _P, _P, _P, _I, _I, _I, _I, _I, _P, _P, _P]),
    "gdmae_conv3x3_grad_taps": (_I, [_P, _I, _P, _P, _P, _P, _P, _P, _P, _L, _I, _I, _I, _P, _P]),
    "gdmae_decoder_tiles_workspace_bytes": (_Z, [_I, _I, _I]),
    "gdmae_decoder_tiles": (_I, [_P, _P, _I, _I, _I, _I, _P, _P, _P, _P, _P]),
    "gdmae_conv3x3_tiles_packed_bytes": (_Z, [_I]),
    "gdmae_conv3x3_tiles_pack": (_I, [_P, _I, _I, _P, _I, _P, _P, _P, _P]),
    "gdmae_conv3x3_tiles_workspace_bytes": (_Z, [_I]),
    "gdmae_conv3x3_tiles_fwd": (_I, [_P, _P, _P, _P, _P, _I, _P, _P, _P, _I, _I, _I, _I, _P, _P, _P, _D, _D, _P, _P, _P, _P, _P, _P,
                                     _P, _P]),
    "gdmae_tiles_gather_rows": (_I, [_P, _P, _P, _P, _L, _I, _I, _I, _I, _P, _P]),
    "gdmae_tiles_to_dense": (_I, [_P, _P, _P, _I, _I, _I, _I, _I, _P, _P]),
    "gdmae_tiles_to_dense_affine_relu": (_I, [_P, _P, _P, _I, _I, _I, _I, _P, _P, _P, _P]),
    "gdmae_rows_bwd": (_I, [_P, _I, _P, _L, _I, _P, _P, _P, _P, _P, _I, _I, _I, _P, _I, _P]),
    "gdmae_segment_max_affine": (_I, [_P, _I, _P, _P, _I, _I, _P, _P, _P, _P, _P]),
    "gdmae_segmax_bwd_stats": (_I, [_P, _I, _P, _P, _P, _L, _I, _P, _P, _P, _P, _P]),
    "gdmae_segmax_bn_bwd": (_I, [_P, _I, _P, _P, _P, _P, _L, _I, _P, _P, _P, _P, _I, _P]),
    "gdmae_window_attention_fwd": (_I, [_P, _P, _P, _I, _P, _P, _P, _I, _I, _I, _I, _P, _F, _P]),
    "gdmae_window_attention_bwd": (_I, [_P, _P, _P, _P, _P, _I, _P, _P, _P, _P, _I, _I, _I, _I, _P, _F, _P]),
    "gdmae_window_attention_levels_writes_lse": (_I, [_I, _I, _P, _I, _I]),
    "gdmae_window_attention_levels_fwd": (_I, [_P, _P, _P, _I, _P, _P, _P, _I, _P, _P, _I, _I, _P, _F, _P, _P]),
    "gdmae_window_attention_levels_bwd": (_I, [_P, _P, _P, _P, _P, _I, _P, _P, _P, _P, _I, _P, _P, _I, _I, _P, _F, _P, _P, _P]),
    "gdmae_conv3x3_dense_packed_bytes": (_Z, [_I, _I]),
    "gdmae_conv3x3_dense_pack": (_I, [_P, _I, _I, _I, _I, _P, _P]),
    "gdmae_conv3x3_dense": (_I, [_P, _I, _I, _I, _I, _I, _I, _P, _P, _P, _P]),
    "gdmae_conv3x3_dense_add": (_I, [_P, _I, _I, _I, _I, _I, _I, _P, _P, _P, _P, _P]),
    "gdmae_conv3x3_dense_relu": (_I, [_P, _I, _I, _I, _I, _I, _I, _P, _P, _P, _P, _P]),
    "gdmae_conv3x3_dense_stats_workspace_bytes": (_Z, [_I, _I, _I, _I]),
    "gdmae_conv3x3_dense_stat_rows": (_I, []),
    "gdmae_conv3x3_dense_stats": (_I, [_P, _I, _I, _I, _I, _I, _I, _P, _P, _P, _P, _P, _P]),
    "gdmae_bn_fold_partials": (_I, [_P, _I, _I, _D, _P, _P, _D, _D, _P, _P, _P, _P, _P, _P, _P]),
    "gdmae_conv3x3_dense_f32out": (_I, [_P, _I, _I, _I, _I, _I, _I, _P, _P, _P, _I, _P]),
    "gdmae_conv3x3_dense_dw_workspace_bytes": (_Z, [_I, _I, _I, _I, _I]),
    "gdmae_conv3x3_dense_bwd_weight": (_I, [_P, _P, _I, _I, _I, _I, _I, _I, _I, _I, _P, _P, _P]),
    "gdmae_attention_timing": (_I, [_I]),
    "gdmae_attention_timing_read": (_I, [_I, _P, _P]),
    "gdmae_kernel_timing": (_I, [_I]),
    "gdmae_kernel_timing_slots": (_I, []),
    "gdmae_kernel_timing_name": (C.c_char_p, [_I]),
    "gdmae_kernel_timing_read": (_I, [_I, _P, _P, _P, _P]),
    "gdmae_kernel_timing_read_side": (_I, [_I, _P]),
    "gdmae_add_layernorm_workspace_bytes": (_Z, [_I]),
    "gdmae_add_layernorm_fwd": (_I, [_P, _P, _I, _P, _P, _L, _I, _F, _P, _P, _P, _P]),
    "gdmae_add_layernorm_bwd": (_I, [_P, _P, _I, _P, _P, _P, _P, _I, _L, _I, _P, _P, _P, _P, _P]),
    "gdmae_prep_tokens": (_I, [_P, _P, _P, _L, _I, _P, _P, _I, _P]),
    "gdmae_sum_bf16": (_I, [_P, _I, _L, _P, _P]),
    "gdmae_add3": (_I, [_P, _P, _I, _P, _I, _L, _P, _P]),
    "gdmae_add3_to": (_I, [_P, _P, _I, _P, _I, _L, _P, _I, _P]),
    "gdmae_set_attention_impl": (_I, [_I]),
    "gdmae_sum_partials": (_I, [_P, _L, _F, _P, _I, _P]),
    "gdmae_sum_partials_gated": (_I, [_P, _L, _F, _P, _P, _F, _P]),
    "gdmae_gemm_workspace_bytes": (_Z, []),
    "gdmae_gemm_stats": (_I, [_P]),
    "gdmae_gemm_tuning": (_I, [_I]),
    "gdmae_gemm": (_I, [_P, _P, _P, _L, _L, _L, _I, _I, _I, _I, _P, _P, _P]),
    "gdmae_gemm_tn_splitk_workspace_bytes": (_Z, [_L, _I, _I]),
    "gdmae_gemm_tn_splitk": (_I, [_P, _P, _P, _L, _I, _I, _I, _I, _P, _P]),
    "gdmae_conv_block_scratch_bytes": (_Z, [_L, _L, _I, _I, _I]),
    "gdmae_spconv_packed_bytes": (_Z, [_I, _I]),
    "gdmae_spconv_pack_jobs": (_I, [_P, _I, _I, _I, _P, _P]),
    "gdmae_spconv": (_I, [_P, _I, _P, _P, _L, _I, _I, _P, _I, _P]),
    "gdmae_spconv_bias_relu": (_I, [_P, _I, _P, _P, _P, _L, _I, _I, _P, _P]),
    "gdmae_spconv_stat_rows": (_I, [_I, _I, _I]),
    "gdmae_spconv_stats": (_I, [_P, _I, _P, _P, _L, _I, _I, _P, _P, _P]),
    "gdmae_decoder_dy": (_I, [_P, _P, _I, _P, _P, _P, _P, _I, _I, _I, _P, _P]),
    "gdmae_decoder_site_rulebook": (_I, [_P, _P, _I, _L, _P, _I, _I, _P, _P]),
    "gdmae_tap_dw_rows": (_L, [_L, _I, _I]),
    "gdmae_tap_dw_workspace_bytes": (_Z, [_L, _I, _I]),
    "gdmae_tap_dw": (_I, [_P, _L, _L, _I, _P, _P, _I, _P, _I, _I, _P, _P]),
    "gdmae_decoder_block_dw_workspace_bytes": (_Z, [_L, _I]),
    "gdmae_decoder_block_dw": (_I, [_P, _P, _P, _P, _P, _L, _I, _P, _P, _I, _I, _P, _I, _I, _P, _P]),
    "gdmae_conv_block_fwd": (_I, [_P, _P]),
    "gdmae_conv_block_bwd": (_I, [_P, _P]),
    "gdmae_encoder_layer_bytes": (_I, [_L, _I, _I, _I, _I, _P, _P, _P]),
    "gdmae_dw_gemm_workspace_bytes": (_Z, [_L, _I, _I]),
    "gdmae_dw_gemm": (_I, [_P, _P, _L, _I, _I, _P, _P, _P, _P]),
    "gdmae_layer_packed_bytes": (_Z, [_I, _I]),
    "gdmae_layer_pack_jobs": (_I, [_P, _P, _P, _P, _I, _I, _P, _P]),
    "gdmae_layer_pack_job_count": (_I, [_I, _I]),
    "gdmae_tok_gemm_pack": (_I, [_P, _I, _P]),
    "gdmae_tok_gemm": (_I, [_P, _P, _P, _L, _L, _I, _I, _I, _P, _P, _P, _P, _P, _P, _F, _P, _P, _P, _P, _P, _P, _P]),
    "gdmae_tok_gemm_qkv": (_I, [_P, _P, _P, _P, _P, _L, _I, _P, _P, _P]),
    "gdmae_tok_gemm_ffn": (_I, [_P, _P, _P, _P, _P, _L, _L, _I, _P, _P, _P, _P, _F, _P, _P, _P, _P, _P, _P, _P, _P]),
    "gdmae_tok_gemm_ln_bwd_rows": (_I, [_I]),
    "gdmae_tok_gemm_ln_bwd": (_I, [_P, _P, _L, _L, _I, _I, _P, _P, _P, _P, _P, _P, _P, _P, _P, _P]),
    "gdmae_encoder_layer_fwd": (_I, [_P, _P]),
    "gdmae_encoder_layer_bwd": (_I, [_P, _P]),
    "gdmae_encoder_stage_fwd": (_I, [_P, _I, _P]),
    "gdmae_encoder_stage_bwd": (_I, [_P, _I, _P]),
    "gdmae_deconv_rows_packed_bytes": (_Z, [_I, _I, _I]),
    "gdmae_deconv_rows_pack": (_I, [_P, _I, _I, _I, _P, _P, _P]),
    "gdmae_deconv_rows_fwd": (_I, [_P, _L, _I, _I, _I, _P, _P, _P]),
    "gdmae_deconv_rows_bwd_input": (_I, [_P, _L, _I, _I, _I, _P, _P, _P]),
    "gdmae_deconv_rows_dw_workspace_bytes": (_Z, [_L, _I, _I, _I]),
    "gdmae_deconv_rows_bwd_weight": (_I, [_P, _P, _L, _I, _I, _I, _P, _P, _P]),
    "gdmae_pred_head_packed_bytes": (_Z, []),
    "gdmae_pred_head_pack": (_I, [_P, _P, _I, _I, _P, _P]),
    "gdmae_pred_head_fwd": (_I, [_P, _L, _I, _P, _P, _P, _P, _P]),
    "gdmae_pred_head_bwd_workspace_bytes": (_Z, [_L]),
    "gdmae_pred_head_bwd": (_I, [_P, _I, _P, _P, _P, _P, _L, _I, _P, _P, _P, _P, _P, _P]),
    "gdmae_encoder_set_layer_path": (_I, [_I]),
    "gdmae_encoder_stage_fused": (_I, [_P, _I]),
    "gdmae_group_gt_points": (_I, [_P, _I, _P, _P, _P, _I, _I, _P, _P, _P, _P, _P]),
    "gdmae_chamfer": (_I, [_P, _P, _P, _I, _I, _I, _P, _P, _P]),
    "gdmae_augment_collate_workspace_bytes": (_Z, [_L]),
    "gdmae_augment_collate": (_I, [_P, _L, _I, _P, _I, _P, _P, _P, _P, _P, _P]),
    "gdmae_gt_sample_workspace_bytes": (_Z, [_L]),
    "gdmae_gt_sample_select": (_I, [_P, _P, _P, _P, _I, _I, _P, _P, _P, _I, _I, _P, _P, _P, _P, _P, _P]),
    "gdmae_gt_sample_collate": (_I, [_P, _P, _I, _P, _I, _L, _I, _P, _P, _P, _P, _P, _P, _P, _P, _P, _P]),
    "gdmae_group_workspace_bytes": (_Z, [_L, _L]),
    "gdmae_ingroup_inds": (_I, [_P, _L, _L, _P, _P, _Z, _P]),
    "gdmae_group_inner_inds": (_I, [_P, _L, _L, _I, _P, _P, _Z, _P]),
    "gdmae_center_head_targets_workspace_bytes": (_Z, [_I, _I]),
    "gdmae_center_head_targets": (_I, [_P, _I, _I, _I, _P, _I, _I, _P, _P, _F, _I, _I, _I, _D, _I, _P, _P, _P, _P, _P, _P]),
    "gdmae_center_head_targets_iou": (_I, [_P, _I, _I, _I, _P, _I, _I, _P, _P, _F, _I, _I, _I, _D, _I, _P, _P, _P, _P, _P, _P, _P]),
    "gdmae_focal_loss_rows": (_I, []),
    "gdmae_focal_loss_fwd": (_I, [_P, _I, _P, _P, _I, _I, _I, _I, _P, _P, _P, _P]),
    "gdmae_focal_loss_bwd": (_I, [_P, _I, _P, _P, _I, _I, _I, _I, _P, _P, _P, _I, _P]),
    "gdmae_center_head_decode": (_I, [_P, _P, _P, _P, _P, _P, _P, _P, _I, _I, _I, _I, _P, _P, _F, _P, _F, _I, _P, _P, _P, _P, _P]),
    "gdmae_center_head_detect_workspace_bytes": (_Z, [_I, _I, _I]),
    "gdmae_center_head_detect": (_I, [_P] * 8 + [_I] * 4 + [_P, _P, _F, _P, _F, _I, _I, _P, _P, _P, _P, _P, _I, _I] + [_P] * 6),
    "gdmae_anchor_targets_workspace_bytes": (_Z, [_I, _I, _I]),
    "gdmae_anchor_targets": (_I, [_P, _I, _I, _I, _I, _I, _I, _I, _I, _P, _P, _P, _P, _P, _P, _P, _P, _P, _F, _I, _P, _P, _P, _P, _P, _P, _P]),
    "gdmae_anchor_loss_rows": (_I, []),
    "gdmae_anchor_loss_fwd": (_I, [_P, _I, _I, _I, _I, _I, _I, _I, _P, _P, _P, _P, _P, _P, _P, _P, _P]),
    "gdmae_anchor_loss_bwd": (_I, [_P, _I, _I, _I, _I, _I, _I, _I, _P, _P, _P, _P, _P, _P, _P, _P, _P]),
    "gdmae_anchor_decode": (_I, [_P, _I, _I, _I, _I, _I, _I, _I, _I, _P, _P, _P, _F, _F, _P, _P, _P]),
    "gdmae_anchor_select": (_I, [_P, _I, _I, _I, _I, _F, _P, _P, _P, _P, _P]),
    "gdmae_anchor_head_infer_packed_bytes": (_Z, [_I]),
    "gdmae_anchor_head_infer_pack": (_I, [_P, _P, _P, _P, _P, _P, _I, _I, _I, _I, _P, _P]),
    "gdmae_anchor_head_infer_workspace_bytes": (_Z, [_I, _I, _I, _I]),
    "gdmae_anchor_head_infer": (_I, [_P, _I, _I, _I, _I, _I, _I, _I, _P, _P, _P, _P, _F, _F, _F, _P, _P, _P, _P, _P, _P, _P, _P]),
    "gdmae_anchor_detect_workspace_bytes": (_Z, [_I, _I]),
    "gdmae_anchor_detect": (_I, [_P, _P, _P, _P, _I, _I, _I, _I, _F, _I, _P, _P, _P, _P, _P, _P]),
    "gdmae_boxes_bev_pairs": (_I, [_P, _I, _P, _I, _I, _P, _P]),
    "gdmae_nms_workspace_bytes": (_Z, [_I]),
    "gdmae_nms_bev": (_I, [_P, _I, _F, _I, _P, _P, _P, _P]),
    "gdmae_geometry_plan_layout": (_I, [_P, _P, _I, _P, _P]),
    "gdmae_geometry_plan": (_I, [_P, _P, _P, _P, _Z, _P]),
    "gdmae_grad_sq_norm": (_I, [_P, _L, _P, _P, _P]),
    "gdmae_adam_step": (_I, [_P, _P, _P, _P, _P, _I, _F, _F, _F, _F, _F, _I, _F, _F, _P, _P]),
    "gdmae_adam_step_shadow": (_I, [_P, _P, _P, _P, _P, _I, _F, _F, _F, _F, _F, _I, _F, _F, _P, _P, _P]),
    "gdmae_roi_dfvs_pool_workspace_bytes": (_Z, [_L, _I, _I, _I, _I]),
    "gdmae_roi_dfvs_pool": (_I, [_P, _L, _I, _P, _I, _I, _I, _P, _P, _I, _I, _P, _I, _I, _I, _F, _F, _I, _I, _P, _P, _P, _P, _P, _Z, _P]),
    "gdmae_roi_targets_workspace_bytes": (_Z, [_I, _I]),
    "gdmae_roi_targets": (_I, [_P, _P, _P, _I, _I, _I, _P, _I, _P, _P, _P, _I, _I, _F, _F, _F, _F, _I, _I, _P, _P, _P, _P, _P, _P, _P, _P, _P, _P, _Z, _P]),
    "gdmae_recall_record": (_I, [_P, _P, _I, _I, _I, _P, _P, _I, _I, _P, _I, _I, _P, _I, _P, _P, _P]),
    "gdmae_kitti_eval_frames_per_chunk": (_I, []),
    "gdmae_kitti_eval_workspace_bytes": (_Z, [_I, _I]),
    "gdmae_kitti_eval": (_I, [_I, _I, _I] + [_P] * 21 + [_I] + [_P] * 9 + [_Z, _P]),
    "gdmae_kitti_annos": (_I, [_P, _I, _P, _P, _P, _P, _P, _I, _I, _I, _P, _I, _P, _I, _P, _P, _P, _P, _P, _P, _P, _P]),
    "gdmae_once_eval_frames_per_chunk": (_I, []),
    "gdmae_once_eval_workspace_bytes": (_Z, [_I, _I]),
    "gdmae_once_eval": (_I, [_I] * 6 + [_P] * 22 + [_Z, _P]),
    "gdmae_roi_graph_folded_floats": (_Z, []),
    "gdmae_roi_graph_packed_bytes": (_Z, []),
    "gdmae_roi_graph_workspace_bytes": (_Z, [_L]),
    "gdmae_roi_graph_pack": (_I, [_P, _P, _P]),
    "gdmae_roi_graph_forward": (_I, [_P, _P, _P, _I, _P, _I, _I, _I, _P, _P, _P, _P, _P, _P, _P, _Z, _P]),
}

class LayerArgs(C.Structure):
    _fields_ = ([("n", _L), ("d", _I), ("ff", _I), ("nhead", _I), ("bf16", _I), ("eps", _F), ("tau_min", _F), ("n_levels", _I),
                 ("n_win", _I * 4), ("max_tokens", _I * 4)]
                + [(k, _P) for k in ("tok_pos", "csr_tok", "win_start", "win_len", "pos_table", "Win", "bin", "Wo", "bo", "W1", "b1",
                                     "W2", "b2", "g1", "be1", "g2", "be2", "tau", "x", "y", "dy", "dx", "dWin", "dbin", "dtau", "dWo",
                                     "dbo", "dW1", "db1", "dW2", "db2", "dg1", "dbe1", "dg2", "dbe2", "saved", "scratch", "packed")]
                + [("x_bf16", _I), ("res_out", _P), ("dres", _P), ("dx_bf16", _P), ("path", _I)])


class PlanParams(C.Structure):
    _fields_ = [("n_points", _L), ("n_cols", _I), ("batch_size", _I), ("lo", _F * 3), ("vs", _F * 3), ("grid", _I * 3), ("n_stages", _I),
                ("stride", _I * 4), ("win_x", _I * 4), ("win_y", _I * 4), ("n_levels", _I * 4), ("drop_lo", (_I * 3) * 4),
                ("drop_hi", (_I * 3) * 4), ("max_tokens", (_I * 3) * 4), ("masked", _I), ("keep_frac", _D), ("n_dec", _I),
                ("dec_sources", _I * 4), ("want_pm", _I), ("cap_points", _L)]


class PlanBuffer(C.Structure):
    _fields_ = [("name", C.c_char * 40), ("offset", _L), ("bytes", _L)]


class ConvBlockArgs(C.Structure):
    _fields_ = ([("n_in", _L), ("n_out", _L), ("cin", _I), ("cout", _I), ("bf16", _I), ("x_f32", _I), ("g_f32", _I),
                 ("eps", _F), ("momentum", _F)]
                + [(k, _P) for k in ("x", "nbr", "nbr_t", "W", "gamma", "beta", "running_mean", "running_var", "num_batches", "cols",
                                     "y", "stats", "ab", "mv", "out", "g", "dx", "dW", "dgamma", "dbeta", "scratch", "packed_fwd", "packed_bwd")]
                + [("out_f32", _I)])


_lib = None


def load():
    global _lib
    if _lib is not None:
        return _lib
    if not os.path.exists(LIB_PATH):
        raise GdmaeHipError(f"{LIB_PATH} not found - build it with `python -m gdmae_hip.build` "
                            "(__graft_entry__.build()); there is no CPU fallback for the product path")
    lib = C.CDLL(LIB_PATH)
    for name, (res, args) in SIGNATURES.items():
        fn = getattr(lib, name)
        fn.restype = res
        fn.argtypes = args
    _lib = lib
    return lib


def ptr(t):
    if t is None:
        return None
    assert t.is_cuda and t.is_contiguous(), "HIP entry points need contiguous device tensors"
    return t.data_ptr()


_raw_stream = getattr(torch._C, "_cuda_getCurrentRawStream", None)


def stream():
    if _raw_stream is not None:
        return _raw_stream(torch.cuda.current_device())
    return torch.cuda.current_stream().cuda_stream


def call(name, *args):
    lib = load()
    rc = getattr(lib, name)(*args)
    if rc != 0:
        raise GdmaeHipError(f"{name} failed ({rc}): {lib.gdmae_last_error().decode()}")


def host_f32(vals):
    return (C.c_float * len(vals))(*[float(v) for v in vals])


def host_i32(vals):
    return (C.c_int * len(vals))(*[int(v) for v in vals])


def host_i64(vals):
    return (C.c_longlong * len(vals))(*[int(v) for v in vals])


def ptr_any(t):
    assert t.is_cuda
    return t.data_ptr()


def host_ptrs(tensors):
    return (C.c_void_p * len(tensors))(*[ptr(t) for t in tensors])


def host_ptrs_any(tensors):
    return (C.c_void_p * len(tensors))(*[ptr_any(t) for t in tensors])
```

### gd-mae_amd/gdmae_hip/ops.py

```python
from __future__ import annotations

import torch

from . import lib as L
from . import timing

I32 = torch.int32


def _f32c(t):
    assert t.dtype == torch.float32
    return t.contiguous()


def gather_rows_raw(src: torch.Tensor, idx: torch.Tensor) -> torch.Tensor:
    src = src.contiguous()
    C = src.shape[-1]
    rb = C * src.element_size()
    out = torch.empty(tuple(idx.shape) + (C,), dtype=src.dtype, device=src.device)
    L.call("gdmae_gather_rows", L.ptr(src), L.ptr(idx.contiguous()), idx.numel(), rb, L.ptr(out), L.stream())
    return out


def scatter_rows_raw(src: torch.Tensor, idx: torch.Tensor, dst: torch.Tensor) -> torch.Tensor:
    src = src.contiguous()
    rb = src.shape[-1] * src.element_size()
    L.call("gdmae_scatter_rows", L.ptr(src), L.ptr(idx.contiguous()), idx.numel(), rb, L.ptr(dst), L.stream())
    return dst


class ScatterToDense(torch.autograd.Function):

    @staticmethod
    def forward(ctx, feat, idx, n_rows):
        ctx.save_for_backward(idx)
        dst = torch.zeros(n_rows, feat.shape[1], dtype=feat.dtype, device=feat.device)
        return scatter_rows_raw(feat, idx, dst)

    @staticmethod
    def backward(ctx, g):
        (idx,) = ctx.saved_tensors
        return gather_rows_raw(g, idx), None, None


class GatherUnique(torch.autograd.Function):

    @staticmethod
    def forward(ctx, dense, idx):
        ctx.save_for_backward(idx)
        ctx.n_rows = dense.shape[0]
        return gather_rows_raw(dense, idx)

    @staticmethod
    def backward(ctx, g):
        (idx,) = ctx.saved_tensors
        dst = torch.zeros(ctx.n_rows, g.shape[1], dtype=g.dtype, device=g.device)
        return scatter_rows_raw(g, idx, dst), None


_BMM_OUT_DTYPE_OK = None
_GEMM_WS = {}


def _gemm_ws(dev, nbytes):
    t = _GEMM_WS.get(dev.index)
    if t is None or t.numel() < nbytes:
        t = torch.empty(int(nbytes), dtype=torch.uint8, device=dev)
        _GEMM_WS[dev.index] = t
    return t


def _gemm_ok(*ts):
    dt = ts[0].dtype
    return dt in (torch.bfloat16, torch.float32) and all(t.dtype == dt and t.is_contiguous() and t.dim() == 2 for t in ts)


def mm(a: torch.Tensor, b: torch.Tensor, trans_b: bool = False, bias: torch.Tensor | None = None) -> torch.Tensor:
    M, K = a.shape
    N = b.shape[0] if trans_b else b.shape[1]
    if not (_gemm_ok(a, b) and K % 8 == 0 and N % 8 == 0 and M > 0 and (bias is None or (bias.dtype == a.dtype and bias.is_contiguous()))):
        y = a @ (b.t() if trans_b else b)
        return y if bias is None else y + bias
    out = torch.empty(M, N, dtype=a.dtype, device=a.device)
    ws = _gemm_ws(a.device, L.load().gdmae_gemm_workspace_bytes())
    L.call("gdmae_gemm", L.ptr(a), L.ptr(b), L.ptr(out), M, N, K, 0, int(trans_b), int(a.dtype == torch.bfloat16), 0,
           None if bias is None else L.ptr(bias), L.ptr(ws), L.stream())
    return out


def splitk_tn_acc(a: torch.Tensor, b: torch.Tensor, dst: torch.Tensor) -> bool:
    K, m = a.shape
    n = b.shape[1]
    if not (_gemm_ok(a, b) and m % 8 == 0 and n % 8 == 0 and K >= 1 and dst.is_contiguous() and dst.dtype == torch.float32
            and dst.numel() == m * n):
        return False
    ws = _gemm_ws(a.device, L.load().gdmae_gemm_tn_splitk_workspace_bytes(K, m, n))
    L.call("gdmae_gemm_tn_splitk", L.ptr(a), L.ptr(b), L.ptr(dst), K, m, n, int(a.dtype == torch.bfloat16), 1, L.ptr(ws), L.stream())
    return True


def splitk_tn(a: torch.Tensor, b: torch.Tensor) -> torch.Tensor:
    K, m = a.shape
    n = b.shape[1]
    if not (_gemm_ok(a, b) and m % 8 == 0 and n % 8 == 0 and K >= 1):
        return _splitk_tn_torch(a, b)
    out = torch.empty(m, n, dtype=torch.float32, device=a.device)
    ws = _gemm_ws(a.device, L.load().gdmae_gemm_tn_splitk_workspace_bytes(K, m, n))
    L.call("gdmae_gemm_tn_splitk", L.ptr(a), L.ptr(b), L.ptr(out), K, m, n, int(a.dtype == torch.bfloat16), 0, L.ptr(ws), L.stream())
    return out


def _splitk_tn_torch(a: torch.Tensor, b: torch.Tensor) -> torch.Tensor:
    global _BMM_OUT_DTYPE_OK
    K, m = a.shape
    n = b.shape[1]
    tiles = max(1, (m + 127) // 128) * max(1, (n + 127) // 128)
    S = max(1, min(K // 256, (1024 + tiles - 1) // tiles, 256))
    if S <= 1:
        return (a.t() @ b).float()
    kc = K // S
    K0 = kc * S
    a3 = a[:K0].view(S, kc, m).transpose(1, 2)
    b3 = b[:K0].view(S, kc, n)
    out = None
    if a.dtype != torch.float32 and _BMM_OUT_DTYPE_OK is not False:
        try:
            out = torch.bmm(a3, b3, out_dtype=torch.float32).sum(0)
            _BMM_OUT_DTYPE_OK = True
        except (TypeError, RuntimeError):
            _BMM_OUT_DTYPE_OK = False
    if out is None:
        out = torch.bmm(a3, b3).sum(0, dtype=torch.float32)
    if K0 < K:
        out = out + (a[K0:].t() @ b[K0:]).float()
    return out


def shadow(t: torch.Tensor, dtype) -> torch.Tensor:
    if t.dtype == dtype:
        return t
    base = t._base if t._base is not None else t
    sh = getattr(base, "_gd_shadow", None)
    if sh is not None and dtype == torch.bfloat16 and sh[1] == base._version:
        s16 = sh[0]
        if t is base:
            return s16
        return s16.as_strided(t.shape, t.stride(), s16.storage_offset() + t.storage_offset() - base.storage_offset())
    return t.to(dtype)


def direct_grad(p):
    g = getattr(p, "_gd_flat_grad", None)
    return g if (g is not None and p.grad is g) else None
# ... 93 lines not shown
        return ga, (ga if ctx.b_dtype == torch.float32 else (g if g.dtype == ctx.b_dtype else g.to(ctx.b_dtype)))


def linear(x, weight, bias=None):
    return LinearSplitK.apply(x, weight, bias)


class SparseConv3x3(torch.autograd.Function):

    @staticmethod
    def forward(ctx, x, weight, nbr, nbr_t):
        cout, _, _, cin = weight.shape
        cdt = torch.bfloat16 if torch.is_autocast_enabled() else x.dtype
        cols = gather_rows_raw(x.to(cdt), nbr).view(nbr.shape[0], 9 * cin)
        wc = shadow(weight, cdt)
        ctx.save_for_backward(cols, wc, nbr_t)
        ctx.w_dtype = weight.dtype
        return mm(cols, wc.reshape(cout, 9 * cin), trans_b=True)

    @staticmethod
    def backward(ctx, g):
        cols, wc, nbr_t = ctx.saved_tensors
        cout, _, _, cin = wc.shape
        g = g.contiguous().to(cols.dtype)
        dw = splitk_tn(g, cols).view(cout, 3, 3, cin).to(ctx.w_dtype)
        gcols = gather_rows_raw(g, nbr_t).view(nbr_t.shape[0], 9 * cout)
        wt = wc.permute(1, 2, 0, 3).reshape(9 * cout, cin)
        return mm(gcols, wt), dw, None, None


class SegmentMax(torch.autograd.Function):
    @staticmethod
    def forward(ctx, x, pt_off, pillar_pts, inverse32):
        x = _f32c(x)
        M = pt_off.numel() - 1
        C = x.shape[1]
        out = torch.empty(M, C, dtype=torch.float32, device=x.device)
        arg = torch.empty(M, C, dtype=I32, device=x.device)
        L.call("gdmae_segment_max", L.ptr(x), L.ptr(pt_off), L.ptr(pillar_pts), M, C, L.ptr(out), L.ptr(arg), L.stream())
        ctx.save_for_backward(arg, inverse32)
        ctx.shape = x.shape
        return out

    @staticmethod
    def backward(ctx, g):
        arg, inv = ctx.saved_tensors
        N, C = ctx.shape
        dx = torch.empty(N, C, dtype=torch.float32, device=g.device)
        L.call("gdmae_segment_max_bwd", L.ptr(_f32c(g)), L.ptr(arg), L.ptr(inv), N, C, L.ptr(dx), L.stream())
        return dx, None, None, None


def decorate_points(vox) -> torch.Tensor:
    F = vox.n_cols - 1
    out = torch.empty(vox.N, F + 6, dtype=torch.float32, device=vox.points.device)
    L.call("gdmae_decorate_points", L.ptr(vox.points), L.ptr(vox.point_coords), L.ptr(vox.inverse32),
           L.ptr(vox.pillar_mean), vox.N, vox.n_cols, L.host_f32(vox.lo), L.host_f32(vox.vs), L.ptr(out), L.stream())
    return out


class AddLayerNorm(torch.autograd.Function):

    @staticmethod
    def forward(ctx, a, b, gamma, beta, eps):
        ctx.a_dtype = a.dtype
        a = a.float().contiguous()
        b = b.contiguous()
        assert b.dtype in (torch.float32, torch.bfloat16) and a.shape == b.shape
        n, d = a.shape
        y = torch.empty_like(a)
        stats = torch.empty(n, 2, dtype=torch.float32, device=a.device)
        L.call("gdmae_add_layernorm_fwd", L.ptr(a), L.ptr(b), int(b.dtype == torch.bfloat16), L.ptr(gamma.detach().contiguous()),
               L.ptr(beta.detach().contiguous()), n, d, float(eps), L.ptr(y), L.ptr(stats), None, L.stream())
        ctx.save_for_backward(a, b, gamma, stats)
        return y

    @staticmethod
    def backward(ctx, g):
        a, b, gamma, stats = ctx.saved_tensors
        n, d = a.shape
        dx = torch.empty_like(a)
        dgb = torch.empty(3 * d, dtype=torch.float32, device=a.device)
        ws = torch.empty(L.load().gdmae_add_layernorm_workspace_bytes(d), dtype=torch.uint8, device=a.device)
        L.call("gdmae_add_layernorm_bwd", L.ptr(a), L.ptr(b), int(b.dtype == torch.bfloat16), L.ptr(gamma.detach().contiguous()),
               L.ptr(stats), L.ptr(_f32c(g)), None, 0, n, d, L.ptr(dx), None, L.ptr(dgb), L.ptr(ws), L.stream())
        return dx.to(ctx.a_dtype), dx.to(b.dtype), dgb[:d], dgb[d:2 * d], None


def add_layer_norm(a, b, norm: torch.nn.LayerNorm):
    return AddLayerNorm.apply(a, b, norm.weight, norm.bias, norm.eps)


class WindowCosineAttention(torch.autograd.Function):

    @staticmethod
    def forward(ctx, qk, v, tau, wplan, nhead, tau_min):
        assert qk.dtype == v.dtype and qk.dtype in (torch.float32, torch.bfloat16)
        qk, v = qk.contiguous(), v.contiguous()
        bf = int(qk.dtype == torch.bfloat16)
        es = qk.element_size()
        n, d = v.shape
        out = torch.empty(n, d, dtype=v.dtype, device=v.device)
        tau_flat = tau.detach().reshape(1).float().contiguous()
        nl = len(wplan.n_win)
        has_lse = bool(L.load().gdmae_window_attention_levels_writes_lse(bf, nl, L.host_i32(wplan.max_tokens), d, nhead))
        lse = torch.empty(n, nhead, dtype=torch.float32, device=v.device) if has_lse else None
        with timing.kernel("k_win_attn_fwd", n * (4 * d * es + 4) + 8 * sum(wplan.n_win)):
            L.call("gdmae_window_attention_levels_fwd", L.ptr(qk), L.ptr(v), L.ptr(out), bf, L.ptr(wplan.csr_tok), L.ptr(wplan.win_start),
                   L.ptr(wplan.win_len), nl, L.host_i32(wplan.n_win), L.host_i32(wplan.max_tokens), d, nhead, L.ptr(tau_flat), float(tau_min),
                   L.ptr(lse), L.stream())
        ctx.has_lse = has_lse
        if has_lse:
            ctx.save_for_backward(qk, v, tau_flat, out, lse)
        else:
            ctx.save_for_backward(qk, v, tau_flat)
        ctx.wplan, ctx.nhead, ctx.tau_min, ctx.tau_shape, ctx.tau_dtype = wplan, nhead, tau_min, tau.shape, tau.dtype
        return out

    @staticmethod
    def backward(ctx, g):
        if ctx.has_lse:
            qk, v, tau_flat, out, lse = ctx.saved_tensors
        else:
            (qk, v, tau_flat), out, lse = ctx.saved_tensors, None, None
        wplan, H = ctx.wplan, ctx.nhead
        n, d = v.shape
        g = g.contiguous().to(v.dtype)
        bf = int(v.dtype == torch.bfloat16)
        es = v.element_size()
        dqk = torch.empty_like(qk)
        dv = torch.empty_like(v)
        n_items = [nw * H for nw in wplan.n_win]
        part = torch.zeros(max(sum(n_items), 1), dtype=torch.float32, device=v.device)
        pbase = sum(n_items)
        with timing.kernel("k_win_attn_bwd", n * (7 * d * es + 4) + 8 * sum(wplan.n_win)):
            L.call("gdmae_window_attention_levels_bwd", L.ptr(qk), L.ptr(v), L.ptr(g), L.ptr(dqk), L.ptr(dv), bf, L.ptr(part), L.ptr(wplan.csr_tok),
                   L.ptr(wplan.win_start), L.ptr(wplan.win_len), len(wplan.n_win), L.host_i32(wplan.n_win), L.host_i32(wplan.max_tokens), d, H,
                   L.ptr(tau_flat), float(ctx.tau_min), L.ptr(out), L.ptr(lse), L.stream())
        dtau = torch.empty(1, dtype=torch.float32, device=v.device)
        L.call("gdmae_sum_partials_gated", L.ptr(part), pbase, 1.0, L.ptr(dtau), L.ptr(tau_flat), float(ctx.tau_min),
               L.stream())
        return dqk, dv, dtau.view(ctx.tau_shape).to(ctx.tau_dtype), None, None, None


def group_gt_points(vox, K: int, want_index: bool = False):
    dev = vox.points.device
    gt = torch.empty(vox.M, K, 3, dtype=torch.float32, device=dev)
    gi = torch.empty(vox.M, K, dtype=I32, device=dev) if want_index else None
    L.call("gdmae_group_gt_points", L.ptr(vox.points), vox.n_cols, L.ptr(vox.pt_off), L.ptr(vox.pillar_pts),
           L.ptr(vox.voxel_coords), vox.M, K, L.host_f32(vox.lo), L.host_f32(vox.vs), L.ptr(gt), L.ptr(gi), L.stream())
    return (gt, gi) if want_index else gt


LAZY_SCALE = {}


class ChamferLoss(torch.autograd.Function):

    @staticmethod
    def forward(ctx, pred, gt, weights, lazy_scale=False):
        ctx.pred_dtype = pred.dtype
        ctx.lazy = bool(lazy_scale and pred.dtype == torch.float32)
        pred, gt, weights = _f32c(pred.float()), _f32c(gt), _f32c(weights)
        M, P1, _ = pred.shape
        P2 = gt.shape[1]
        term = torch.empty(max(M, 1), dtype=torch.float32, device=pred.device)
        dpred = torch.empty_like(pred)
        L.call("gdmae_chamfer", L.ptr(pred), L.ptr(gt), L.ptr(weights), M, P1, P2, L.ptr(term), L.ptr(dpred), L.stream())
        res = torch.empty(2, dtype=torch.float32, device=pred.device)
        L.call("gdmae_weighted_mean_finish", L.ptr(term), L.ptr(weights), M, L.ptr(res), L.stream())
        ctx.save_for_backward(dpred, res)
        return res[0]

    @staticmethod
    def backward(ctx, g):
        dpred, res = ctx.saved_tensors
        inv = res[1]
        if ctx.lazy:
            LAZY_SCALE.clear()
            LAZY_SCALE[dpred.data_ptr()] = (g.detach().reshape(1).float().contiguous(), res[1:2])
            return dpred, None, None, None
        if ctx.pred_dtype == torch.float32:
            return dpred * (g * inv), None, None, None
        out = torch.empty_like(dpred, dtype=ctx.pred_dtype)
        torch.mul(dpred, g * inv, out=out)
        return out, None, None, None
```

### gd-mae_amd/pcdet/models/backbones_3d/spt_backbone_mae.py

```python
import torch
import torch.nn as nn

from .spt_backbone import SSTBlockV1, build_decoder, run_decoder, stage_plan_args
from ...utils.spconv_utils import SparseConvTensor
from gdmae_hip import decoder as gdec, ops, plan as gplan


def _only_the_pred_head_sees_the_gradient(pred) -> bool:
    fn = pred.grad_fn
    if fn is None or not type(fn).__name__.startswith('ViewBackward') or pred._backward_hooks or pred.retains_grad:
        return False
    nxt = [f for f, _ in fn.next_functions if f is not None]
    if len(nxt) != 1 or 'PredHeadFn' not in type(nxt[0]).__name__:
        return False
    return not getattr(nxt[0], '_tensor_pre_hooks', None) and not getattr(nxt[0], '_pre_hooks', None) and not getattr(nxt[0], '_retains_grad_hooks', None)


class _DeferredPlan:
    __slots__ = ("_mod", "_args", "_pf")

    def __init__(self, mod, args):
        self._mod, self._args, self._pf = mod, args, None

    def __call__(self):
        if self._pf is None and self._args is not None:
            points, batch_size, noise, ready = self._args
            self._args = None
            self._pf = self._mod.prefetch_plan(points, batch_size, noise=noise, ready=ready)

    def ensure_issued(self):
        if self._mod is not None and getattr(self._mod, '_pre_conv_hook', None) is self:
            self._mod._pre_conv_hook = None
        self()

    def finish(self):
        self.ensure_issued()
        pf, self._pf, self._mod = self._pf, None, None
        return pf.finish()


class SPTBackboneMAE(nn.Module):
    decoder_impl = 'sparse'
    dense_spatial_features = True
    decoder_conv_impl = 'tiles'

    def __init__(self, model_cfg, input_channels, grid_size, voxel_size, point_cloud_range, **kwargs):
        super().__init__()
        self.model_cfg, self.grid_size, self.voxel_size, self.point_cloud_range = model_cfg, grid_size, voxel_size, point_cloud_range
        self.sparse_shape = grid_size[[1, 0]]
        self.mask_cfg = model_cfg.get('MASK_CONFIG', None)
        self.mask_ratio = self.mask_cfg.RATIO if self.mask_cfg is not None else 0.0
        c = input_channels
        self.sst_blocks = nn.ModuleList()
        for b in model_cfg.SST_BLOCK_LIST:
            self.sst_blocks.append(SSTBlockV1(b, c, b.NAME))
            c = b.ENCODER.D_MODEL
        self.decoder_deblocks, self.decoder_conv_out, c = build_decoder(model_cfg)
        self.decoder_pred = nn.Linear(c, self.mask_cfg.NUM_PRD_POINTS * 3, bias=True)
        self.forward_ret_dict = {}
        self.num_point_features = c

    def get_loss(self, tb_dict=None):
        tb_dict = {} if tb_dict is None else tb_dict
        r = self.forward_ret_dict
        pred = r['pred_points']
        lazy = bool(r.get('pred_lazy_scale', False)) and _only_the_pred_head_sees_the_gradient(pred)
        return ops.ChamferLoss.apply(pred, r['gt_points'], r['mask'], lazy), tb_dict

    def forward(self, batch_dict):
        vox = batch_dict['_gdmae_vox']
        all_feat, all_coords = batch_dict['voxel_features'], batch_dict['voxel_coords']
        ep = batch_dict.get('_gdmae_plan', None)
        if ep is None:
            ep = gplan.encoder_plan(vox, *stage_plan_args(self.model_cfg.SST_BLOCK_LIST),
                                    keep_frac=1 - self.mask_ratio, noise=batch_dict.get('mae_noise', None),
                                    dec_sources=self._dec_sources())
        batch_dict['voxel_mae_mask'] = ep.mask
        batch_dict['_gdmae_plan'] = ep
        tok = batch_dict.pop('_gdmae_tok_features', None)
        if tok is not None:
            if tok[1] is not ep:
                raise RuntimeError("DynVFE's token features belong to another geometry plan than batch_dict['_gdmae_plan']")
            tok_feat = tok[0]
        else:
            tok_feat = ops.GatherUnique.apply(all_feat, ep.tok_pillar)
        x = SparseConvTensor(tok_feat, ep, 0)
        sync = batch_dict.get('_gdmae_grad_sync', None)
        hidden = []
        for i, blk in enumerate(self.sst_blocks):
            if sync is not None:
                sync.mark(x.features, [f'backbone_3d.sst_blocks.{i}'])
            x = blk(x)
            hidden.append(x)
        if sync is not None:
            sync.mark(x.features, ['backbone_3d.decoder'])
        feats, strides = {}, {}
        Y0 = int(self.sparse_shape[0])
        for i, h in enumerate(hidden):
            feats[f'x_conv{i + 1}'] = h
            strides[f'x_conv{i + 1}'] = Y0 // h.spatial_shape[0]
        B, X, Y = int(batch_dict['batch_size']), int(self.grid_size[0]), int(self.grid_size[1])
        if self.decoder_impl == 'sparse' and self.training:
            hook, self._pre_conv_hook = getattr(self, '_pre_conv_hook', None), None
            pyramid, sf = gdec.sparse_decoder(self.model_cfg, self.decoder_deblocks, self.decoder_conv_out, hidden,
                                              vox.pillar_cell, vox.cell2pillar, B, Y, X,
                                              want_dense=self.dense_spatial_features, conv_impl=self.decoder_conv_impl,
                                              pre_conv_hook=hook)
        else:
            sf = run_decoder(self.model_cfg, self.decoder_deblocks, self.decoder_conv_out, hidden)
            assert sf.shape[0] == B and sf.shape[2] == Y and sf.shape[3] == X
            pyramid = ops.GatherUnique.apply(sf.permute(0, 2, 3, 1).reshape(B * Y * X, sf.shape[1]), vox.pillar_cell)
        src0 = self.model_cfg.FEATURES_SOURCE[0]
        batch_dict.update({'encoded_spconv_tensor': hidden[-1], 'encoded_spconv_tensor_stride': Y0 // hidden[-1].spatial_shape[0],
                           'multi_scale_3d_features': feats, 'multi_scale_3d_strides': strides, 'spatial_features': sf,
                           'spatial_features_stride': strides[src0] // self.model_cfg.FUSE_LAYER[src0].UPSAMPLE_STRIDE})
        batch_dict.update({'voxel_features': pyramid, 'voxel_coords': all_coords,
                           'voxel_shuffle_inds': torch.arange(all_coords.shape[0], device=all_coords.device)})
        self.forward_ret_dict = self.target_assigner(batch_dict)
        return batch_dict

    def prefetch_plan(self, points, batch_size, noise=None, ready=None):
        return gplan.PlanPrefetch(points, self.point_cloud_range, self.voxel_size, self.grid_size, int(batch_size),
                                  *stage_plan_args(self.model_cfg.SST_BLOCK_LIST), keep_frac=1 - self.mask_ratio, noise=noise,
                                  ready=ready, dec_sources=self._dec_sources())

    def prefetch_plan_under_decoder(self, points, batch_size, noise=None, ready=None):
        self._pre_conv_hook = d = _DeferredPlan(self, (points, batch_size, noise, ready))
        return d

    def _dec_sources(self):
        if self.decoder_impl != 'sparse' or self.decoder_conv_impl != 'tiles':
            return None
        return [int(src[-1]) - 1 for src in self.model_cfg.FEATURES_SOURCE]

    def target_assigner(self, batch_dict):
        vox = batch_dict['_gdmae_vox']
        gt = ops.group_gt_points(vox, self.mask_cfg.NUM_GT_POINTS)
        flat = gdec.pred_head(batch_dict['voxel_features'], self.decoder_pred)
        return {'pred_points': flat.view(vox.M, -1, 3), 'gt_points': gt, 'mask': batch_dict['voxel_mae_mask'],
                'pred_lazy_scale': bool(getattr(flat, '_gd_pred_head', False))}
```

### include/gdmae_hip.h

```cpp
#ifndef GDMAE_HIP_H
#define GDMAE_HIP_H

#include <stddef.h>
#include <stdint.h>

#ifdef __cplusplus
extern "C" {
#endif

int gdmae_abi_version(void);
const char* gdmae_target_arch(void);
const char* gdmae_last_error(void);

size_t gdmae_voxelize_workspace_bytes(long long n_points, int batch_size, int gx, int gy, int gz);
int gdmae_voxelize(const float* points, long long n_points, int n_cols, const float* lo, const float* vs,
                   const int* grid_xyz, int batch_size, float* points_out, long long* point_coords,
                   long long* inverse, int* inverse32, long long* voxel_coords, int* pillar_cell,
                   int* pillar_pt_off, int* pillar_pts, int* point_rank, int* sample_pillar_off,
                   float* pillar_mean, int* cell2pillar, int* counts, void* workspace, size_t workspace_bytes,
                   void* stream);

int gdmae_decorate_points(const float* points, const long long* point_coords, const int* inverse32,
                          const float* pillar_mean, long long N, int n_cols, const float* lo, const float* vs,
                          float* out, void* stream);
int gdmae_pillar_major_rows(const float* points, int n_cols, const int* pillar_pts, const int* inverse32, const int* n_dev,
                            long long capacity, float* points_pm, int* row_pillar, void* stream);
int gdmae_vfe_infer(const float* points_pm, const long long* voxel_coords, const int* row_pillar, const float* pillar_mean,
                    long long N, long long M, int n_cols, const float* lo, const float* vs, const float* W1, const float* b1,
                    int c1, const float* W2, const float* b2, int c2, float* out, void* stream);
size_t gdmae_vfe_point_layer_workspace_bytes(int n_cols);
int gdmae_vfe_point_layer_fwd(const float* points, const long long* point_coords, const int* inverse32,
                              const float* pillar_mean, int coords_per_pillar, long long N, int n_cols, const float* lo,
                              const float* vs,
                              const float* W, int C, const float* gamma, const float* beta, double eps, double momentum,
                              float* running_mean, float* running_var, long long* num_batches, double* stats, float* ab,
                              float* mv, void* out, int out_bf16, void* workspace, void* stream);
int gdmae_vfe_point_layer_bwd(const float* points, const long long* point_coords, const int* inverse32,
                              const float* pillar_mean, int coords_per_pillar, long long N, int n_cols, const float* lo,
                              const float* vs,
                              const float* W, int C, const float* gamma, const double* stats, const float* ab,
                              const void* g, int g_bf16, float* dgamma, float* dbeta, float* dW, int accumulate,
                              void* workspace, void* stream);
size_t gdmae_vfe_max_layer_workspace_bytes(void);
int gdmae_vfe_max_layer_fwd(const void* y1, long long N, const void* W, const int* pillar_pt_off, const int* row_pillar,
                            int M, const float* gamma, const float* beta, double eps, double momentum,
                            float* running_mean, float* running_var, long long* num_batches, double* stats, float* ab,
                            float* mv, float* out, int* arg, void* workspace, void* stream);
int gdmae_vfe_max_layer_bwd(const void* y1, long long N, const void* W, const int* row_pillar, int M, const float* gamma,
                            const double* stats, const float* ab, const float* out, const int* arg, const float* g, void* gm,
                            void* dy1, float* dgamma, float* dbeta, float* dW, int accumulate,
                            void* workspace, void* stream);
int gdmae_vfe_max_layer_fwd_f16(const void* y1, long long N, const float* W, const int* pillar_pt_off, const int* row_pillar,
                                int M, const float* gamma, const float* beta, double eps, double momentum,
                                float* running_mean, float* running_var, long long* num_batches, double* stats, float* ab,
                                float* mv, float* out, int* arg, void* workspace, void* stream);
int gdmae_vfe_max_layer_bwd_f16(const void* y1, long long N, const float* W, const int* row_pillar, int M, const float* gamma,
                                const double* stats, const float* ab, const float* out, const int* arg, const float* g, void* gm,
                                void* dy1, float* dgamma, float* dbeta, float* dW, int accumulate,
                                void* workspace, void* stream);
int gdmae_vfe_max_layer_vis_fwd(const void* y1, long long N, const void* W, const int* vis_rows, const int* vis_tok, long long Nv,
                                int n_tok, const float* gamma, const float* beta, double eps, double momentum,
                                float* running_mean, float* running_var, long long* num_batches, double* stats, float* ab,
                                float* mv, float* out, int* arg, void* workspace, void* stream);
int gdmae_vfe_max_layer_vis_fwd_f16(const void* y1, long long N, const float* W, const int* vis_rows, const int* vis_tok, long long Nv,
                                    int n_tok, const float* gamma, const float* beta, double eps, double momentum,
                                    float* running_mean, float* running_var, long long* num_batches, double* stats, float* ab,
                                    float* mv, float* out, int* arg, void* workspace, void* stream);
int gdmae_vfe_max_layer_vis_bwd(const void* y1, long long N, const void* W, const int* row_tok, const int* tok_pillar, int n_tok, int M,
                                const float* gamma, const double* stats, const float* ab, const float* out, const int* arg,
                                const float* g, void* gm, void* dy1, float* dgamma, float* dbeta, float* dW, int accumulate,
                                void* workspace, void* stream);
int gdmae_vfe_max_layer_vis_bwd_f16(const void* y1, long long N, const float* W, const int* row_tok, const int* tok_pillar, int n_tok, int M,
                                    const float* gamma, const double* stats, const float* ab, const float* out, const int* arg,
                                    const float* g, void* gm, void* dy1, float* dgamma, float* dbeta, float* dW, int accumulate,
                                    void* workspace, void* stream);
int gdmae_segment_max(const float* x, const int* pillar_pt_off, const int* pillar_pts, int M, int C, float* out,
                      int* arg, void* stream);
int gdmae_segment_max_bwd(const float* dout, const int* arg, const int* inverse32, long long N, int C, float* dx,
                          void* stream);

int gdmae_random_mask(const float* noise, const int* sample_pillar_off, int batch_size, double keep_frac,
                      float* mask_out, int* len_keep_out, void* stream);

int gdmae_visible_tokens(const float* mask, const int* pillar_cell, const int* vox_counts, long long m_cap,
                         long long n_cells, int* tok_pillar, int* tok_cell, int* map, int* n_tok, void* scan_ws,
                         void* stream);
int gdmae_downsample_tokens(const int* n_in, const int* tok_cell_in, long long cap_in, int B, int Yi, int Xi,
                            int* tok_cell_out, int* map_out, int* n_out, int* flag_ws, void* scan_ws, void* stream);
int gdmae_rulebook(const int* n_tok, const int* tok_cell, long long cap, int B, int Yt, int Xt, int Ym, int Xm,
                   const int* map, int mode, int* nbr, void* stream);

size_t gdmae_window_workspace_bytes(int B, int Y, int X, int wx, int wy);
int gdmae_window_partition(const int* map, int B, int Y, int X, int wx, int wy, int shifted, int nlev,
                           const int* drop_lo, const int* drop_hi, const int* max_tokens, int* tok_win,
                           int* tok_level, int* tok_slot, int* tok_pos, int* csr_tok, int* win_start, int* win_len,
                           int* counts, void* workspace, size_t workspace_bytes, void* stream);

int gdmae_gather_rows(const void* src, const int* idx, long long n_slots, int row_bytes, void* out, void* stream);
int gdmae_scatter_rows(const void* src, const int* idx, long long n_rows, int row_bytes, void* dst, void* stream);

int gdmae_gather_rows_strided(const void* src, const int* idx, long long n_slots, int row_bytes, int table_row_bytes,
                              int table_col_bytes, void* out, void* stream);
int gdmae_scatter_rows_strided(const void* src, const int* idx, long long n_rows, int row_bytes, int table_row_bytes,
                               int table_col_bytes, void* dst, void* stream);
size_t gdmae_colstats_workspace_bytes(int C);
int gdmae_colstats(const void* x, long long R, int C, int is_bf16, double* out, void* workspace, void* stream);

size_t gdmae_decoder_region_workspace_bytes(int C2, int Cin);
int gdmae_decoder_region_algebra(const double* stats2, const float* ab2, const double* st2, const float* k01,
                                 const double* reg, const double* tap_region, const double* cnt, double R, int C2, int Cin,
                                 const float* conv_w, const void* bgz, int cdt_bf16, double* S, double* tot, float* dWk,
                                 void* Wd, void* workspace, void* stream);
int gdmae_fill_rows(const void* v, long long R, int C, int elem_bytes, void* Z, void* stream);
int gdmae_rows_affine_relu_scatter(const void* P, int p_bf16, const int* site, long long n, int C, const float* a,
                                   const float* b, void* Z, int z_bf16, int z_row_elems, int col0, void* stream);
int gdmae_rows_affine_relu_sub(const void* P, int p_bf16, const int* site, long long n, int C, const float* a, const float* b,
                               const void* sub, void* Z, int z_bf16, int z_row_elems, int col0, void* stream);
int gdmae_rows_affine_relu_add(const void* P, int p_bf16, long long n, int C, const float* a, const float* b, const void* R, void* Z,
                               int z_bf16, void* stream);
size_t gdmae_rows_bwd_stats_workspace_bytes(int C);
int gdmae_rows_bwd_stats(const void* P, int p_bf16, const int* site, long long n, int C, const float* a, const float* b,
                         const void* dZ, int z_bf16, int z_row_elems, int col0, double* out, void* workspace, void* stream);
int gdmae_rows_bwd(const void* P, int p_bf16, const int* site, long long n, int C, const float* a, const float* b,
                   const float* c0, const float* c1, const void* dZ, int z_bf16, int z_row_elems, int col0, void* dP,
                   int dp_bf16, void* stream);

int gdmae_bn_fold(const void* x, long long R, int C, int is_bf16, double count, const float* gamma, const float* beta,
                  double eps, double momentum, float* running_mean, float* running_var, long long* num_batches,
                  double* stats, float* ab, float* mv, void* workspace, void* stream);
int gdmae_bn_fold_partials(const float* part, int nblk, int C, double count, const float* gamma, const float* beta, double eps,
                           double momentum, float* running_mean, float* running_var, long long* num_batches, double* stats, float* ab,
                           float* mv, void* stream);
int gdmae_bn_bwd_coeffs(const double* st, int n_st, const double* stats, const float* ab, const float* gamma, int C,
                        double count, const double* tot, float* dgamma, float* dbeta, int accumulate, float* c01,
                        void* stream);
int gdmae_rows_bwd_stats_rows(long long n);
int gdmae_bn_bwd_coeffs_rows(const float* part, int nblk, int n_st, const double* stats, const float* ab, const float* gamma, int C,
                             double count, const double* tot, float* dgamma, float* dbeta, int accumulate, float* c01,
                             void* stream);

int gdmae_conv3x3_grad_taps(const void* Y, int y_bf16, const int* tile_slot, const void* ybg, const float* k0,
                            const float* k1, const float* rows, const int* cell2pillar, const int* site, long long n, int H,
                            int W, int C, void* out, void* stream);

size_t gdmae_border_sums_workspace_bytes(int B, int C);
int gdmae_border_sums(const void* Y, int y_bf16, const int* tile_slot, const void* ybg, const float* rows,
                      const int* pillar_cell, int M, int B, int H, int W, int C, double* out, void* workspace, void* stream);

size_t gdmae_decoder_tiles_workspace_bytes(int B, int H, int W);
int gdmae_decoder_tiles(const int* const* maps, const int* strides, int k, int B, int H, int W, int* tile_slot, int* tile_list,
                        int* n_act, void* workspace, void* stream);
size_t gdmae_conv3x3_tiles_packed_bytes(int k);
int gdmae_conv3x3_tiles_pack(const float* conv_w, int C2, int Cin, const float* const* b, int k, void* Wp, void* bgz, void* ybg,
                             void* stream);
size_t gdmae_conv3x3_tiles_workspace_bytes(int n_act);
int gdmae_conv3x3_tiles_fwd(const void* const* P, const int* const* maps, const float* const* a, const float* const* b,
                            const int* strides, int k, const void* Wp, const void* ybg, const int* tile_list, int n_act, int B,
                            int H, int W, void* Yc, const float* gamma, const float* beta, double eps, double momentum,
                            float* running_mean, float* running_var, long long* num_batches, double* stats, float* ab,
                            float* mv, void* workspace, void* stream);
int gdmae_tiles_gather_rows(const void* Yc, const int* tile_slot, const void* ybg, const int* cell, long long n, int H, int W,
                            int C, int elem_bytes, void* out, void* stream);
int gdmae_tiles_to_dense(const void* Yc, const int* tile_slot, const void* ybg, int B, int H, int W, int C, int elem_bytes,
                         void* out, void* stream);
int gdmae_tiles_to_dense_affine_relu(const void* Yc, const int* tile_slot, const void* ybg, int B, int H, int W, int C, const float* a,
                                     const float* b, float* out, void* stream);

int gdmae_segment_max_affine(const void* x, int x_bf16, const int* pillar_pt_off, const int* pillar_pts, int M, int C,
                             const float* a, const float* b, float* out, int* arg, void* stream);
int gdmae_segmax_bwd_stats(const void* x, int x_bf16, const float* out, const int* arg, const float* dout, long long M,
                           int C, const float* a ,
                           const float* b, double* sums, void* workspace, void* stream);
int gdmae_segmax_bn_bwd(const void* x, int x_bf16, const float* out, const int* arg, const float* dout,
                        const int* inverse32, long long N, int C, const float* a, const float* c0, const float* c1,
                        void* dx, int dx_bf16, void* stream);

int gdmae_set_attention_impl(int impl);
int gdmae_window_attention_fwd(const void* qk, const void* v, void* out, int io_bf16, const int* csr_tok,
                               const int* win_start, const int* win_len, int n_win, int T, int d, int H,
                               const float* tau, float tau_min, void* stream);
int gdmae_window_attention_bwd(const void* qk, const void* v, const void* dout, void* dqk, void* dv, int io_bf16,
                               float* dtau_part, const int* csr_tok, const int* win_start, const int* win_len,
                               int n_win, int T, int d, int H, const float* tau, float tau_min, void* stream);
int gdmae_window_attention_levels_writes_lse(int io_bf16, int n_levels, const int* max_tokens, int d, int H);
int gdmae_window_attention_levels_fwd(const void* qk, const void* v, void* out, int io_bf16, const int* csr_tok,
                                      const int* win_start, const int* win_len, int n_levels, const int* n_win,
                                      const int* max_tokens, int d, int H, const float* tau, float tau_min, float* lse, void* stream);
int gdmae_window_attention_levels_bwd(const void* qk, const void* v, const void* dout, void* dqk, void* dv, int io_bf16,
                                      float* dtau_part, const int* csr_tok, const int* win_start, const int* win_len,
                                      int n_levels, const int* n_win, const int* max_tokens, int d, int H, const float* tau,
                                      float tau_min, const void* out, const float* lse, void* stream);
int gdmae_attention_timing(int on);
int gdmae_attention_timing_read(int which, double* total_ms, long long* calls);
int gdmae_kernel_timing(int on);
int gdmae_kernel_timing_slots(void);
const char* gdmae_kernel_timing_name(int slot);
int gdmae_kernel_timing_read(int slot, double* total_ms, long long* calls, double* bytes, double* flops);
int gdmae_kernel_timing_read_side(int slot, double* side_bytes);
int gdmae_weighted_mean_finish(const float* term, const float* weights, long long n, float* out, void* stream);
int gdmae_sum_partials(const float* part, long long n, float scale, float* out, int accumulate, void* stream);
int gdmae_sum_partials_gated(const float* part, long long n, float scale, float* out, const float* gate, float gate_min,
                             void* stream);

size_t gdmae_add_layernorm_workspace_bytes(int d);
int gdmae_add_layernorm_fwd(const float* a, const void* b, int b_is_bf16, const float* gamma, const float* beta,
                            long long n, int d, float eps, float* y, float* stats, void* y_bf16 ,
                            void* stream);
int gdmae_add_layernorm_bwd(const float* a, const void* b, int b_is_bf16, const float* gamma, const float* stats,
                            const float* dy, const void* dy2, int dy2_bf16, long long n, int d, float* dx, void* dx_bf16,
                            float* sums, void* workspace, void* stream);
int gdmae_prep_tokens(const float* x, const float* pos_table, const int* tok_pos, long long n, int d, void* x_out,
                      void* xpos_out, int out_bf16, void* stream);
int gdmae_sum_bf16(const void* const* src, int k, long long total, void* out, void* stream);
int gdmae_add3(const float* a, const void* b, int b_bf16, const void* c, int c_bf16, long long total, float* out, void* stream);
int gdmae_add3_to(const float* a, const void* b, int b_bf16, const void* c, int c_bf16, long long total, void* out, int out_bf16,
                  void* stream);

int gdmae_gemm_stats(long long* calls);
int gdmae_gemm_tuning(int mode);
size_t gdmae_gemm_workspace_bytes(void);
int gdmae_gemm(const void* A, const void* B, void* C, long long M, long long N, long long K, int trans_a, int trans_b,
               int ab_bf16, int c_f32, const void* bias, void* workspace, void* stream);
size_t gdmae_gemm_tn_splitk_workspace_bytes(long long K, int m, int n);
int gdmae_gemm_tn_splitk(const void* A, const void* B, float* C, long long K, int m, int n, int ab_bf16, int accumulate,
                         void* workspace, void* stream);

size_t gdmae_dw_gemm_workspace_bytes(long long rows, int M, int N);
int gdmae_dw_gemm(const void* G, const void* X, long long rows, int M, int N, float* dW, float* dbias, void* workspace,
                  void* stream);

typedef struct gdmae_conv_block_args {
  long long n_in, n_out;
  int cin, cout, bf16, x_f32, g_f32;
  float eps, momentum;
  const void* x;
  const int* nbr;
  const int* nbr_t;
  const void* W;
  const float *gamma, *beta;
  float *running_mean, *running_var;
  long long* num_batches;
  void* cols;
  void* y;
  double* stats;
  float* ab;
  float* mv;
  void* out;
  const void* g;
  void* dx;
  float *dW, *dgamma, *dbeta;
  void* scratch;
  const void* packed_fwd;
  const void* packed_bwd;
  int out_f32;
} gdmae_conv_block_args;
size_t gdmae_conv_block_scratch_bytes(long long n_in, long long n_out, int cin, int cout, int bf16);
size_t gdmae_spconv_packed_bytes(int cin, int cout);
int gdmae_spconv_pack_jobs(const float* W , int cin, int cout, int transposed, void* packed, long long* jobs);
int gdmae_spconv(const void* X, int x_f32, const int* nbr, const void* packed, long long n, int cin, int cout, void* Y,
                 int timing_slot , void* stream);
int gdmae_spconv_bias_relu(const void* X, int x_f32, const int* nbr, const void* packed, const float* bias, long long n, int cin, int cout,
                           void* Y, void* stream);
int gdmae_spconv_stat_rows(int cin, int cout, int x_f32);
int gdmae_spconv_stats(const void* X, int x_f32, const int* nbr, const void* packed, long long n, int cin, int cout, void* Y, float* part,
                       void* stream);
int gdmae_decoder_dy(const void* Yc, const int* tile_list, int n_act, const float* k0, const float* k1, const float* rows,
                     const int* cell2pillar, int H, int W, int C, void* dYc, void* stream);
int gdmae_decoder_site_rulebook(const int* site, const int* n_dev, int sites_per_tok, long long cap_sites, const int* tile_slot,
                                int H, int W, int* nbr, void* stream);
long long gdmae_tap_dw_rows(long long n, int M, int N);
size_t gdmae_tap_dw_workspace_bytes(long long n, int M, int N);
int gdmae_tap_dw(const void* G, long long n, long long n_pad, int M, const void* X, const int* nbr, int N, float* out, int ld_out,
                 int m_off, void* workspace, void* stream);
size_t gdmae_decoder_block_dw_workspace_bytes(long long n, int u);
int gdmae_decoder_block_dw(const void* P, const float* a, const float* b, const void* bg, const int* site, long long n, int u,
                           const void* dYc, const int* tile_slot, int H, int W, float* out, int ld_out, int m_off, void* workspace,
                           void* stream);
int gdmae_conv_block_fwd(const gdmae_conv_block_args* args , void* stream);
int gdmae_conv_block_bwd(const gdmae_conv_block_args* args , void* stream);

typedef struct gdmae_layer_args {
  long long n;
  int d, ff, nhead, bf16;
  float eps, tau_min;
  int n_levels;
  int n_win[4], max_tokens[4];
  const int* tok_pos;
  const int* csr_tok;
  const int* win_start;
  const int* win_len;
  const float* pos_table;
  const void *Win, *bin, *Wo, *bo, *W1, *b1, *W2, *b2;
  const float *g1, *be1, *g2, *be2, *tau;
  const float* x;
  float* y;
  const float* dy;
  float* dx;
  float *dWin, *dbin, *dtau, *dWo, *dbo, *dW1, *db1, *dW2, *db2, *dg1, *dbe1, *dg2, *dbe2;
  void* saved;
  void* scratch;
  const void* packed;
  int x_bf16;
  void* res_out;
  const void* dres;
  void* dx_bf16;
  int path;
} gdmae_layer_args;
size_t gdmae_layer_packed_bytes(int d, int ff);
int gdmae_layer_pack_jobs(const float* Win, const float* Wo, const float* W1, const float* W2, int d, int ff, void* packed,
                          long long* jobs_host );
int gdmae_layer_pack_job_count(int d, int ff);
int gdmae_tok_gemm_pack(const long long* jobs_dev, int n_jobs, void* stream);
int gdmae_tok_gemm(const void* X, const void* Wp, const void* bias, long long n, long long n_pad, int K, int N, int epilogue,
                   void* out0, void* out1, const void* aux, const float* res, const float* gamma, const float* beta, float eps,
                   float* y, float* stats, void* y_bf16, const float* pos_table, const int* tok_pos, void* ypos_bf16,
                   void* stream);

int gdmae_tok_gemm_qkv(const void* Xpos, const void* X, const void* Wp_qk, const void* Wp_v, const void* bias3, long long n_pad,
                       int d, void* qk, void* v, void* stream);

int gdmae_tok_gemm_ffn(const void* X, const void* W1p, const void* b1, const void* W2p, const void* b2, long long n, long long n_pad,
                       int d, void* h, const float* res, const float* gamma, const float* beta, float eps, float* y, float* stats,
                       void* y_bf16, const float* pos_table, const int* tok_pos, void* ypos_bf16, void* f_out, void* stream);

int gdmae_tok_gemm_ln_bwd_rows(int N);
int gdmae_tok_gemm_ln_bwd(const void* X, const void* Wp, long long n, long long n_pad, int K, int N, const float* dy,
                          const void* dy2_bf16, const float* ln_a, const void* ln_b_bf16, const float* stats,
                          const float* gamma, float* dx, void* dx_bf16, float* part, void* stream);
int gdmae_encoder_layer_bytes(long long n, int d, int ff, int nhead, int bf16, size_t* saved_bytes,
                              size_t* fwd_scratch_bytes, size_t* bwd_scratch_bytes);
int gdmae_encoder_layer_fwd(const gdmae_layer_args* args , void* stream);
int gdmae_encoder_layer_bwd(const gdmae_layer_args* args , void* stream);
int gdmae_encoder_stage_fwd(const gdmae_layer_args* layers , int n_layers, void* stream);
int gdmae_encoder_stage_bwd(const gdmae_layer_args* layers , int n_layers, void* stream);
int gdmae_encoder_set_layer_path(int path);
int gdmae_encoder_stage_fused(const gdmae_layer_args* layers , int n_layers);

size_t gdmae_deconv_rows_packed_bytes(int cin, int cout, int s);
int gdmae_deconv_rows_pack(const float* weight, int cin, int cout, int s, void* packed_fwd, void* packed_bwd, void* stream);
int gdmae_deconv_rows_fwd(const void* X, long long n, int cin, int cout, int s, const void* packed_fwd, void* P, void* stream);
int gdmae_deconv_rows_bwd_input(const void* dP, long long n, int cin, int cout, int s, const void* packed_bwd, void* dX, void* stream);
size_t gdmae_deconv_rows_dw_workspace_bytes(long long n, int cin, int cout, int s);
int gdmae_deconv_rows_bwd_weight(const void* X, const void* dP, long long n, int cin, int cout, int s, float* dW, void* workspace,
                                 void* stream);

size_t gdmae_pred_head_packed_bytes(void);
int gdmae_pred_head_pack(const float* weight, const float* bias, int n_in, int n_out, void* packed, void* stream);
int gdmae_pred_head_fwd(const float* X, long long n, int n_out, const void* packed, void* Y, void* X_bf16 , float* Y_f32 ,
                        void* stream);
size_t gdmae_pred_head_bwd_workspace_bytes(long long n);
int gdmae_pred_head_bwd(const void* dY, int dy_f32 ,
                        void* dY_bf16 ,
                        const float* scale_a, const float* scale_b ,
                        const void* X_bf16, long long n, int n_out,
                        const void* packed, float* dX, float* dW, float* db, void* workspace, void* stream);

size_t gdmae_conv3x3_dense_packed_bytes(int cin, int cout);
int gdmae_conv3x3_dense_pack(const float* weight, int cin, int cout, int dil, int transposed, void* packed, void* stream);
int gdmae_conv3x3_dense(const void* X, int B, int H, int W, int cin_l, int cout_l, int dil, const void* packed, const float* bias,
                        void* Y, void* stream);
int gdmae_conv3x3_dense_add(const void* X, int B, int H, int W, int cin_l, int cout_l, int dil, const void* packed, const float* bias,
                            const void* addend, void* Y, void* stream);
int gdmae_conv3x3_dense_relu(const void* X, int B, int H, int W, int cin_l, int cout_l, int dil, const void* packed, const float* bias,
                             const void* shortcut, void* Y, void* stream);
size_t gdmae_conv3x3_dense_stats_workspace_bytes(int B, int H, int W, int cout_l);
int gdmae_conv3x3_dense_stat_rows(void);
int gdmae_conv3x3_dense_stats(const void* X, int B, int H, int W, int cin_l, int cout_l, int dil, const void* packed, const float* bias,
                              void* Y, float* stat_rows, void* workspace, void* stream);
int gdmae_conv3x3_dense_f32out(const void* X, int B, int H, int W, int cin_l, int cout_l, int dil, const void* packed, const float* bias,
                               float* Y, int accumulate, void* stream);
size_t gdmae_conv3x3_dense_dw_workspace_bytes(int B, int H, int W, int cin_l, int cout_l);
int gdmae_conv3x3_dense_bwd_weight(const void* X, const void* dY, int B, int H, int W, int cin_l, int cout_l, int cin, int cout, int dil,
                                   float* dW, void* workspace, void* stream);

int gdmae_group_gt_points(const float* points, int n_cols, const int* pillar_pt_off, const int* pillar_pts,
                          const long long* voxel_coords, int M, int K, const float* lo, const float* vs,
                          float* gt_points, int* gt_index, void* stream);
int gdmae_chamfer(const float* pred, const float* gt, const float* weights, int M, int P1, int P2, float* term,
                  float* dpred, void* stream);

size_t gdmae_augment_collate_workspace_bytes(long long n_raw);
int gdmae_augment_collate(const float* raw, long long n_raw, int F, const int* frame_off, int B, const float* frame_params,
                          const float* xy_range , float* out, int* kept_off, void* workspace, void* stream);

size_t gdmae_gt_sample_workspace_bytes(long long n_rows);
int gdmae_gt_sample_select(const float* boxes, const int* frame_desc_host, const int* frame_desc, const int* cand_group, int B,
                           int n_groups, const float* frame_params, const float* range ,
                           const float* extra_width , int min_corners, int cap, int* valid, float* rm_boxes,
                           int* n_valid, float* gt_boxes, int* num_gt, void* stream);
int gdmae_gt_sample_collate(const float* raw, const float* db, int F, const int* seg, int S, long long n_rows, int B,
                            const float* frame_params, const float* boxes, const int* valid, const float* rm_boxes,
                            const int* n_valid, const float* xy_range , float* out, int* kept_off, void* workspace,
                            void* stream);

size_t gdmae_group_workspace_bytes(long long n, long long n_groups);
int gdmae_ingroup_inds(const long long* group_inds, long long n, long long n_groups, long long* out_inds,
                       void* workspace, size_t workspace_bytes, void* stream);
int gdmae_group_inner_inds(const long long* inverse_inds, long long n, long long M, int K, long long* group_inds,
                           void* workspace, size_t workspace_bytes, void* stream);

#define GDMAE_PLAN_MAX_STAGES 4
typedef struct gdmae_plan_params {
  long long n_points;
  int n_cols, batch_size;
  float lo[3], vs[3];
  int grid[3];
  int n_stages;
  int stride[GDMAE_PLAN_MAX_STAGES];
  int win_x[GDMAE_PLAN_MAX_STAGES], win_y[GDMAE_PLAN_MAX_STAGES];
  int n_levels[GDMAE_PLAN_MAX_STAGES];
  int drop_lo[GDMAE_PLAN_MAX_STAGES][3], drop_hi[GDMAE_PLAN_MAX_STAGES][3], max_tokens[GDMAE_PLAN_MAX_STAGES][3];
  int masked;
  double keep_frac;
  int n_dec;
  int dec_sources[GDMAE_PLAN_MAX_STAGES];
  int want_pm;
  long long cap_points;
} gdmae_plan_params;
typedef struct gdmae_plan_buffer {
  char name[40];
  long long offset, bytes;
} gdmae_plan_buffer;
int gdmae_geometry_plan_layout(const gdmae_plan_params* p, gdmae_plan_buffer* table, int max_entries, int* n_entries,
                               size_t* total_bytes);
int gdmae_geometry_plan(const gdmae_plan_params* p, const float* points, const float* noise, void* arena, size_t arena_bytes,
                        void* stream);

size_t gdmae_center_head_targets_workspace_bytes(int B, int num_max_objs);
int gdmae_center_head_targets(const float* gt_boxes, int B, int n_max, int box_dim, const int* class_map, int n_class_total,
                              int n_cls, const float* pc_range , const float* voxel_size ,
                              float feature_map_stride, int fw, int fh, int num_max_objs, double gaussian_overlap, int min_radius,
                              float* heatmap, float* ret_boxes, long long* inds, long long* mask, void* workspace, void* stream);
int gdmae_focal_loss_rows(void);
int gdmae_focal_loss_fwd(const void* logits, int logits_bf16, const long long* strides_byxc, const float* gt, int B, int C, int H, int W,
                         float* prob, float* partials, float* out4, void* stream);
int gdmae_focal_loss_bwd(const void* logits, int logits_bf16, const long long* strides_byxc, const float* gt, int B, int C, int H, int W,
                         const float* out4, const float* grad_out, void* dlogits, int dlogits_bf16, void* stream);
int gdmae_center_head_targets_iou(const float* gt_boxes, int B, int n_max, int box_dim, const int* class_map, int n_class_total,
                                  int n_cls, const float* pc_range, const float* voxel_size, float feature_map_stride, int fw, int fh,
                                  int num_max_objs, double gaussian_overlap, int min_radius, float* heatmap, float* ret_boxes,
                                  float* iou_boxes, long long* inds, long long* mask, void* workspace, void* stream);
int gdmae_center_head_decode(const long long* cell, const float* score, const float* center, const float* center_z,
                             const float* dim, const float* rot, const float* vel, const float* iou, int B, int K, int H, int W,
                             const float* pc_range , const float* voxel_size ,
                             float feature_map_stride, const float* post_center_limit_range , float score_thresh,
                             int use_score_thresh, float* boxes, int* labels, float* ious, unsigned char* valid, void* stream);
size_t gdmae_center_head_detect_workspace_bytes(int B, int K, int box_dim);
int gdmae_center_head_detect(const long long* cell, const float* score, const float* center, const float* center_z, const float* dim,
                             const float* rot, const float* vel, const float* iou, int B, int K, int H, int W, const float* pc_range,
                             const float* voxel_size, float feature_map_stride, const float* post_center_limit_range, float score_thresh,
                             int use_score_thresh, int C, const float* thresh, const int* pre_max, const int* post_max,
                             const float* rectifier, const int* to_global, int class_aware, int n_out, float* boxes, float* scores,
                             long long* labels, int* count, void* workspace, void* stream);

int gdmae_boxes_bev_pairs(const float* boxes_a, int n, const float* boxes_b, int m, int mode, float* out, void* stream);
size_t gdmae_nms_workspace_bytes(int n);
int gdmae_nms_bev(const float* boxes, int n, float thresh, int rotated, long long* keep, int* n_keep, void* workspace,
                  void* stream);

size_t gdmae_anchor_targets_workspace_bytes(int B, int n_cls, int n_max);
int gdmae_anchor_targets(const float* gt_boxes, int B, int n_max, int box_dim, int H, int W, int K, int n_cls, int n_names,
                         const int* name_idx, const int* slot_cls, const float* xr, const float* yr, const float* xc, const float* yc,
                         const float* slot, const float* matched, const float* unmatched, float dir_offset, int num_bins,
                         int* labels, int* gt_ids, float* reg_targets, int* dir_bins, int* num_pos, void* workspace, void* stream);
int gdmae_anchor_loss_rows(void);
int gdmae_anchor_loss_fwd(const void* rows, int rows_bf16, int ld, int B, int n_loc, int K, int C, int nb, const int* labels,
                          const float* reg_targets, const int* dir_bins, const int* num_pos, const float* code_weights,
                          const float* scale, float* partials, float* out4, void* stream);
int gdmae_anchor_loss_bwd(const void* rows, int rows_bf16, int ld, int B, int n_loc, int K, int C, int nb, const int* labels,
                          const float* reg_targets, const int* dir_bins, const int* num_pos, const float* code_weights,
                          const float* scale, const float* grad3, void* drows, void* stream);
int gdmae_anchor_decode(const void* rows, int rows_bf16, int ld, int B, int H, int W, int K, int C, int nb, const float* xc,
                        const float* yc, const float* slot, float dir_offset, float dir_limit_offset, float* cls_out, float* boxes,
                        void* stream);
int gdmae_anchor_select(const float* cls, int B, int n, int C, int normalized, float thresh, int* idx, float* score, int* label,
                        int* count, void* stream);

size_t gdmae_anchor_head_infer_packed_bytes(int cin);
int gdmae_anchor_head_infer_pack(const float* w_cls, const float* b_cls, const float* w_box, const float* b_box, const float* w_dir,
                                 const float* b_dir, int cin, int K, int C, int nb, void* packed, void* stream);
size_t gdmae_anchor_head_infer_workspace_bytes(int B, int H, int W, int K);
int gdmae_anchor_head_infer(const void* X, int B, int H, int W, int cin, int K, int C, int nb, const void* packed, const float* xc,
                            const float* yc, const float* slot, float dir_offset, float dir_limit_offset, float thresh,
                            float* rows_out, int* count, int* idx, float* score, int* label, float* box, void* workspace,
                            void* stream);
size_t gdmae_anchor_detect_workspace_bytes(int B, int pre_max);
int gdmae_anchor_detect(const int* count, const float* score, const int* label, const float* box, int B, int A, int pre_max,
                        int post_max, float nms_thresh, int n_out, float* boxes, float* scores, long long* labels, int* num,
                        void* workspace, void* stream);

int gdmae_grad_sq_norm(const float* grad, long long n, float* partials , float* sq_norm_out, void* stream);
int gdmae_adam_step(float* param, const float* grad, float* exp_avg, float* exp_avg_sq, const long long* segments,
                    int n_segments, float lr, float beta1, float beta2, float eps, float weight_decay, int step,
                    float max_norm, float grad_scale, const float* sq_norm, void* stream);
int gdmae_adam_step_shadow(float* param, const float* grad, float* exp_avg, float* exp_avg_sq, const long long* segments,
                           int n_segments, float lr, float beta1, float beta2, float eps, float weight_decay, int step,
                           float max_norm, float grad_scale, const float* sq_norm, void* param_bf16, void* stream);

size_t gdmae_roi_dfvs_pool_workspace_bytes(long long n_points, int batch, int n_rois, int patches_x, int patches_y);
int gdmae_roi_dfvs_pool(const float* points, long long n_points, int n_cols, const float* rois, int batch, int n_rois,
                        int roi_cols, const float* range_xy, const float* patch_lo, int patches_x, int patches_y,
                        const float* extra_width, int num_dvs_points, int num_fps_points, int hash_size, float lambda,
                        float delta, int boxes_per_patch, int phases, int* pooled_idx, int* pooled_num, float* feats_local,
                        float* xyz_global, void* workspace, size_t workspace_bytes, void* stream);

size_t gdmae_roi_graph_folded_floats(void);
size_t gdmae_roi_graph_packed_bytes(void);
size_t gdmae_roi_graph_workspace_bytes(long long n_rois_total);
int gdmae_roi_graph_pack(const float* folded, void* packed, void* stream);
int gdmae_roi_graph_forward(const float* feats_local, const int* pooled_num, const float* rois, int roi_cols,
                            const float* roi_scores, int batch, int n_rois, int scores_normalized, const void* packed,
                            float* rcnn_cls, float* rcnn_reg, float* batch_box_preds, float* batch_cls_preds, int* nbr_debug,
                            void* workspace, size_t workspace_bytes, void* stream);

size_t gdmae_roi_targets_workspace_bytes(int batch, int n_rois);
int gdmae_roi_targets(const float* rois, const float* roi_scores, const int* roi_labels, int batch, int n_rois, int roi_cols,
                      const float* gt_boxes, int n_gt, const float* u_fg, const float* u_bg, const int* hard_quota,
                      int rois_per_image, int fg_per_image, float reg_fg_thresh, float cls_fg_thresh, float cls_bg_thresh,
                      float cls_bg_thresh_lo, int by_class, int cls_score_type, float* out_rois, float* out_roi_scores,
                      int* out_roi_labels, int* out_roi_indices, float* out_gt_iou, float* out_gt_src, float* out_gt_of_rois,
                      int* out_reg_valid, float* out_cls_labels, void* workspace, size_t workspace_bytes, void* stream);

int gdmae_recall_record(const float* pred_boxes, const int* pred_num, int batch, int n_pred, int pred_cols, const float* rois,
                        const int* roi_num, int n_rois, int roi_cols, const float* gt_boxes, int n_gt, int gt_cols,
                        const float* thresholds, int n_thresh, long long* counters, float* best_iou, void* stream);

int gdmae_kitti_eval_frames_per_chunk(void);
size_t gdmae_kitti_eval_workspace_bytes(int n_frames, int n_combos);
int gdmae_kitti_eval(int stages, int n_frames, int n_combos, const int* host_gt_off, const int* host_dt_off, const int* host_dc_off,
                     const int* gt_off, const int* dt_off, const int* dc_off, const long long* pair_off, const float* gt_box,
                     const float* gt_geo, const float* gt_alpha, const float* dt_box, const float* dt_geo, const float* dt_alpha,
                     const float* dt_score, const float* dc_box, const signed char* ignored_gt, const signed char* ignored_dt,
// ... 23 lines not shown
```

Baseline: 1098.

## Fuse GT point grouping into chamfer kernel and fuse decoder affine-ReLU backward into gathers

The chamfer kernel for 16 predicted points can now read raw points through the pillar CSR and compute ground-truth offsets in place, so the separate group_gt kernel and its M×K×3 buffer are skipped. Targets become lazy and are only built when some other consumer asks for them. The decoder border-sum and dY kernels also gain fused variants that apply the affine-ReLU backward mask on the fly, and a new gather kernel emits both the raw rows and the affine-ReLU output in one pass. This trades extra pointer chasing inside the loss kernel and more code paths for less memory traffic and fewer launches.

```diff
diff --git a/gd-mae_amd/csrc/chamfer.hip b/gd-mae_amd/csrc/chamfer.hip
--- a/gd-mae_amd/csrc/chamfer.hip
+++ b/gd-mae_amd/csrc/chamfer.hip
@@ -5,6 +5,11 @@
   int ncols;
   int K;
 };
+
+__device__ __forceinline__ int gt_slot(int k, int cnt) { return k < cnt ? k : k % cnt; }
+__device__ __forceinline__ float gt_centre(long long idx, float vs, float lo) {
+  return __fadd_rn(__fmul_rn(__fadd_rn((float)idx, 0.5f), vs), lo);
+}
 
 __global__ __launch_bounds__(256) void k_group_gt(const float* __restrict__ pts, const int* __restrict__ pt_off,
                                                   const int* __restrict__ csr, const long long* __restrict__ voxel_coords,
@@ -15,11 +20,11 @@
     const int off = pt_off[p];
     const int cnt = pt_off[p + 1] - off;
     const long long* vc = voxel_coords + 4ll * p;
-    const float cx = __fadd_rn(__fmul_rn(__fadd_rn((float)vc[3], 0.5f), P.vs[0]), P.lo[0]);
-    const float cy = __fadd_rn(__fmul_rn(__fadd_rn((float)vc[2], 0.5f), P.vs[1]), P.lo[1]);
-    const float cz = __fadd_rn(__fmul_rn(__fadd_rn((float)vc[1], 0.5f), P.vs[2]), P.lo[2]);
+    const float cx = gt_centre(vc[3], P.vs[0], P.lo[0]);
+    const float cy = gt_centre(vc[2], P.vs[1], P.lo[1]);
+    const float cz = gt_centre(vc[1], P.vs[2], P.lo[2]);
     for (int k = lane; k < P.K; k += GD_WAVE) {
-      const int src = k < cnt ? k : k % cnt;
+      const int src = gt_slot(k, cnt);
       const int pid = csr[off + src];
       const float* r = pts + (long long)pid * P.ncols;
       float* o = gt + ((long long)p * P.K + k) * 3;
@@ -131,9 +136,12 @@
   }
 }
 
+template <bool POINTS>
 __global__ __launch_bounds__(256) void k_chamfer16(const float* __restrict__ pred, const float* __restrict__ gt,
-                                                   const float* __restrict__ w, int M, int P2, float* __restrict__ term,
-                                                   float* __restrict__ dpred) {
+                                                   const float* __restrict__ pts, const int* __restrict__ pt_off,
+                                                   const int* __restrict__ csr, const long long* __restrict__ voxel_coords,
+                                                   GtParams G, const float* __restrict__ w, int M, int P2,
+                                                   float* __restrict__ term, float* __restrict__ dpred) {
   __shared__ float sx[4][48];
   __shared__ float sy[4][GD_WAVE * 3];
   __shared__ int sb[4][GD_WAVE];
@@ -152,7 +160,20 @@
     if (lane < 48) sx[wib][lane] = pred[(long long)m * 48 + lane];
     const bool has = lane < P2;
     float y0 = 0.f, y1 = 0.f, y2 = 0.f;
-    if (has) {
+    if (POINTS) {
+      const int off = pt_off[m];
+      const int cnt = pt_off[m + 1] - off;
+      const long long* vc = voxel_coords + 4ll * m;
+      const int pid = csr[off + gt_slot(has ? lane : P2 - 1, cnt)];
+      const float* r = pts + (long long)pid * G.ncols;
+      const float r1 = r[1], r2 = r[2], r3 = r[3];
+      const float t0 = __fsub_rn(r1, gt_centre(vc[3], G.vs[0], G.lo[0]));
+      const float t1 = __fsub_rn(r2, gt_centre(vc[2], G.vs[1], G.lo[1]));
+      const float t2 = __fsub_rn(r3, gt_centre(vc[1], G.vs[2], G.lo[2]));
+      y0 = has ? t0 : 0.f;
+      y1 = has ? t1 : 0.f;
+      y2 = has ? t2 : 0.f;
+    } else if (has) {
       const float* g = gt + ((long long)m * P2 + lane) * 3;
       y0 = g[0];
       y1 = g[1];
@@ -195,9 +216,15 @@
     const float sumx = gd_wave_sum((lane & 3) == 0 ? dmin : 0.f);
     const float sumy = gd_wave_sum(has ? best : 0.f);
     if (lane == 0) term[m] = cx * sumx + cy * sumy;
-    sy[wib][3 * lane] = y0;
-    sy[wib][3 * lane + 1] = y1;
-    sy[wib][3 * lane + 2] = y2;
+    if (POINTS) {
+      sy[wib][3 * lane] = 2.f * cy * (sx[wib][3 * besti] - y0);
+      sy[wib][3 * lane + 1] = 2.f * cy * (sx[wib][3 * besti + 1] - y1);
+      sy[wib][3 * lane + 2] = 2.f * cy * (sx[wib][3 * besti + 2] - y2);
+    } else {
+      sy[wib][3 * lane] = y0;
+      sy[wib][3 * lane + 1] = y1;
+      sy[wib][3 * lane + 2] = y2;
+    }
     sb[wib][lane] = has ? besti : -1;
     __builtin_amdgcn_fence(__ATOMIC_RELEASE, "workgroup");
     __builtin_amdgcn_wave_barrier();
@@ -206,7 +233,7 @@
       const float xi = sx[wib][lane];
       float acc = 0.f;
       for (int j = 0; j < P2; ++j) {
-        const float v = 2.f * cy * (xi - sy[wib][3 * j + c]);
+        const float v = POINTS ? sy[wib][3 * j + c] : 2.f * cy * (xi - sy[wib][3 * j + c]);
         acc += sb[wib][j] == i ? v : 0.f;
       }
       dp[lane] = sg[wib][lane] + acc;
@@ -223,10 +250,33 @@
   int grid = gd_div_up(M, 4);
   if (grid > 8192) grid = 8192;
   if (P1 == 16)
-    hipLaunchKernelGGL(k_chamfer16, dim3(grid), dim3(256), 0, (hipStream_t)stream, pred, gt, weights, M, P2, term, dpred);
+    hipLaunchKernelGGL(k_chamfer16<false>, dim3(grid), dim3(256), 0, (hipStream_t)stream, pred, gt, nullptr, nullptr, nullptr, nullptr,
+                       GtParams{}, weights, M, P2, term, dpred);
   else
     hipLaunchKernelGGL((k_chamfer<64>), dim3(grid), dim3(256), 0, (hipStream_t)stream, pred, gt, weights, M, P1, P2, term,
                        dpred);
   GD_LAUNCH_CHECK();
   return 0;
 }
+
+extern "C" int gdmae_chamfer_points(const float* pred, const float* points, int n_cols, const int* pillar_pt_off, const int* pillar_pts,
+                                    const long long* voxel_coords, const float* lo, const float* vs, const float* weights, int M,
+                                    int P1, int P2, float* term, float* dpred, void* stream) {
+  if (M <= 0) return 0;
+  GD_REQUIRE(P1 == 16, "chamfer_points serves NUM_PRD_POINTS = 16 (gdmae_group_gt_points + gdmae_chamfer for the others)");
+  GD_REQUIRE(P2 >= 1 && P2 <= GD_WAVE, "NUM_GT_POINTS must be <= 64 (one lane per ground-truth point)");
+  GD_REQUIRE(n_cols >= 4, "point rows are (b, x, y, z, ...)");
+  GtParams G;
+  for (int i = 0; i < 3; ++i) {
+    G.lo[i] = lo[i];
+    G.vs[i] = vs[i];
+  }
+  G.ncols = n_cols;
+  G.K = P2;
+  int grid = gd_div_up(M, 4);
+  if (grid > 8192) grid = 8192;
+  hipLaunchKernelGGL(k_chamfer16<true>, dim3(grid), dim3(256), 0, (hipStream_t)stream, pred, nullptr, points, pillar_pt_off, pillar_pts,
+                     voxel_coords, G, weights, M, P2, term, dpred);
+  GD_LAUNCH_CHECK();
+  return 0;
+}
diff --git a/gd-mae_amd/csrc/conv_tiles.hip b/gd-mae_amd/csrc/conv_tiles.hip
--- a/gd-mae_amd/csrc/conv_tiles.hip
+++ b/gd-mae_amd/csrc/conv_tiles.hip
@@ -599,6 +599,51 @@
   return 0;
 }
 
+__global__ __launch_bounds__(256) void k_tiles_gather_rows_affine_relu(const void* __restrict__ Yc, GdTiles T, const int* __restrict__ cell,
+                                                                       long long n, int H, int W, int C, const float* __restrict__ a,
+                                                                       const float* __restrict__ b, uint4* __restrict__ yrows,
+                                                                       float4* __restrict__ out) {
+  const int cv = C / 8;
+  const long long total = n * cv;
+  for (long long i = blockIdx.x * (long long)blockDim.x + threadIdx.x; i < total; i += (long long)gridDim.x * blockDim.x) {
+    const long long r = total < (1ll << 31) ? (long long)((unsigned)i / (unsigned)cv) : i / cv;
+    const int v = (int)(i - r * cv);
+    const int s = cell[r];
+    const int x = s % W, q = s / W, y = q % H, bb = q / H;
+    const uint4 yq = ((const uint4*)gd_y_row<2>(Yc, T, bb, y, x, H, W, C))[v];
+    const float4 a0 = ((const float4*)a)[2 * v], a1 = ((const float4*)a)[2 * v + 1];
+    const float4 b0 = ((const float4*)b)[2 * v], b1 = ((const float4*)b)[2 * v + 1];
+    const unsigned w4[4] = {yq.x, yq.y, yq.z, yq.w};
+    const float av[8] = {a0.x, a0.y, a0.z, a0.w, a1.x, a1.y, a1.z, a1.w};
+    const float bv[8] = {b0.x, b0.y, b0.z, b0.w, b1.x, b1.y, b1.z, b1.w};
+    float o[8];
+#pragma unroll
+    for (int j = 0; j < 4; ++j) {
+      const float h0 = fmaf(av[2 * j], __uint_as_float(w4[j] << 16), bv[2 * j]);
+      const float h1 = fmaf(av[2 * j + 1], __uint_as_float(w4[j] & 0xFFFF0000u), bv[2 * j + 1]);
+      o[2 * j] = h0 > 0.f ? h0 : 0.f;
+      o[2 * j + 1] = h1 > 0.f ? h1 : 0.f;
+    }
+    yrows[i] = yq;
+    out[2 * i] = make_float4(o[0], o[1], o[2], o[3]);
+    out[2 * i + 1] = make_float4(o[4], o[5], o[6], o[7]);
+  }
+}
+
+extern "C" int gdmae_tiles_gather_rows_affine_relu(const void* Yc, const int* tile_slot, const void* ybg, const int* cell, long long n,
+                                                   int H, int W, int C, const float* a, const float* b, void* yrows, float* out,
+                                                   void* stream) {
+  GD_REQUIRE(tile_slot != nullptr && C % 8 == 0 && a != nullptr && b != nullptr, "tiles_gather_rows_affine_relu: bf16 rows, C % 8 == 0");
+  if (n <= 0) return 0;
+  GdTiles T{tile_slot, ybg, (H + 7) / 8, (W + 7) / 8};
+  long long g = (n * (C / 8) + 255) / 256;
+  if (g > 16384) g = 16384;
+  hipLaunchKernelGGL(k_tiles_gather_rows_affine_relu, dim3((int)g), dim3(256), 0, (hipStream_t)stream, Yc, T, cell, n, H, W, C, a, b,
+                     (uint4*)yrows, (float4*)out);
+  GD_LAUNCH_CHECK();
+  return 0;
+}
+
 template <int ES>
 __global__ __launch_bounds__(256) void k_tiles_to_dense(const void* __restrict__ Yc, GdTiles T, int B, int H, int W, int C,
                                                         uint4* __restrict__ out) {
diff --git a/gd-mae_amd/csrc/decoder.hip b/gd-mae_amd/csrc/decoder.hip
--- a/gd-mae_amd/csrc/decoder.hip
+++ b/gd-mae_amd/csrc/decoder.hip
@@ -680,10 +680,12 @@
 }
 
 #define DEC_BORDER_CHUNKS 64
-template <bool BF>
+template <bool BF, bool FUSED>
 __global__ __launch_bounds__(256) void k_border_partial(const void* __restrict__ Y, GdTiles T, const float* __restrict__ rows,
-                                                        const int* __restrict__ pillar_cell, int M, int B, int H, int W, int C,
-                                                        float* __restrict__ part_edge, float* __restrict__ part_rows) {
+                                                        const void* __restrict__ yrows, const float* __restrict__ a2,
+                                                        const float* __restrict__ b2, const int* __restrict__ pillar_cell, int M,
+                                                        int B, int H, int W, int C, float* __restrict__ part_edge,
+                                                        float* __restrict__ part_rows) {
   extern __shared__ float sh[];
   const int cv = C >> 3;
   if ((int)blockIdx.x < 4 * B) {
@@ -730,6 +732,15 @@
   const int per = ((M + DEC_BORDER_CHUNKS - 1) / DEC_BORDER_CHUNKS + 63) / 64 * 64;
   const int pb = chunk * per, pe = pb + per < M ? pb + per : M;
   float acc[4] = {0.f, 0.f, 0.f, 0.f};
+  float av[4] = {0.f, 0.f, 0.f, 0.f}, bv[4] = {0.f, 0.f, 0.f, 0.f};
+  if (FUSED) {
+#pragma unroll
+    for (int j = 0; j < 4; ++j)
+      if (lane + 64 * j < C) {
+        av[j] = a2[lane + 64 * j];
+        bv[j] = b2[lane + 64 * j];
+      }
+  }
   for (int p0 = pb; p0 < pe; p0 += 64) {
     const int p = p0 + lane;
     bool in = false;
@@ -747,7 +758,15 @@
       const float* rp = rows + (long long)(p0 + k) * C;
 #pragma unroll
       for (int j = 0; j < 4; ++j)
-        if (lane + 64 * j < C) acc[j] += rp[lane + 64 * j];
+        if (lane + 64 * j < C) {
+          float v = rp[lane + 64 * j];
+          if (FUSED) {
+            const float y = dec_ld<BF>(yrows, (long long)(p0 + k) * C + lane + 64 * j);
+            const float dh = fmaf(av[j], y, bv[j]) > 0.f ? v : 0.f;
+            v = fmaf(av[j], dh, fmaf(0.f, y, 0.f));
+          }
+          acc[j] += v;
+        }
     }
   }
 #pragma unroll
@@ -779,22 +798,37 @@
   return (size_t)(4 * B + 8 * DEC_BORDER_CHUNKS) * C * sizeof(float);
 }
 
-extern "C" int gdmae_border_sums(const void* Y, int y_bf16, const int* tile_slot, const void* ybg, const float* rows,
-                                 const int* pillar_cell, int M, int B, int H, int W, int C, double* out ,
-                                 void* workspace, void* stream) {
+static int border_sums(const void* Y, int y_bf16, const int* tile_slot, const void* ybg, const float* rows, const void* yrows,
+                       const float* a2, const float* b2, const int* pillar_cell, int M, int B, int H, int W, int C,
+                       double* out , void* workspace, void* stream) {
   const GdTiles T{tile_slot, ybg, (H + 7) / 8, (W + 7) / 8};
   GD_REQUIRE(C % 8 == 0 && C <= 256 && 256 % (C / 8) == 0, "border_sums: C in {64, 128, 256}");
   hipStream_t st = (hipStream_t)stream;
   float* part_edge = (float*)workspace;
   float* part_rows = part_edge + (size_t)4 * B * C;
   const size_t lds = (size_t)(256 / (C / 8)) * C * sizeof(float);
-  if (y_bf16) hipLaunchKernelGGL((k_border_partial<true>), dim3(4 * B + 2 * DEC_BORDER_CHUNKS), dim3(256), lds, st, Y, T, rows, pillar_cell, M, B, H, W, C, part_edge, part_rows);
-  else hipLaunchKernelGGL((k_border_partial<false>), dim3(4 * B + 2 * DEC_BORDER_CHUNKS), dim3(256), lds, st, Y, T, rows, pillar_cell, M, B, H, W, C, part_edge, part_rows);
+  const dim3 grid(4 * B + 2 * DEC_BORDER_CHUNKS);
+#define GD_LAUNCH(BF, FU) \
+  hipLaunchKernelGGL((k_border_partial<BF, FU>), grid, dim3(256), lds, st, Y, T, rows, yrows, a2, b2, pillar_cell, M, B, H, W, C, part_edge, part_rows)
+  if (y_bf16) { if (yrows) GD_LAUNCH(true, true); else GD_LAUNCH(true, false); }
+  else { if (yrows) GD_LAUNCH(false, true); else GD_LAUNCH(false, false); }
+#undef GD_LAUNCH
   GD_LAUNCH_CHECK();
   if (y_bf16) hipLaunchKernelGGL((k_border_final<true>), dim3(gd_div_up(8 * C, 256)), dim3(256), 0, st, Y, T, part_edge, part_rows, B, H, W, C, out);
   else hipLaunchKernelGGL((k_border_final<false>), dim3(gd_div_up(8 * C, 256)), dim3(256), 0, st, Y, T, part_edge, part_rows, B, H, W, C, out);
   GD_LAUNCH_CHECK();
   return 0;
+}
+extern "C" int gdmae_border_sums(const void* Y, int y_bf16, const int* tile_slot, const void* ybg, const float* rows,
+                                 const int* pillar_cell, int M, int B, int H, int W, int C, double* out ,
+                                 void* workspace, void* stream) {
+  return border_sums(Y, y_bf16, tile_slot, ybg, rows, nullptr, nullptr, nullptr, pillar_cell, M, B, H, W, C, out, workspace, stream);
+}
+extern "C" int gdmae_border_sums_rows(const void* Y, int y_bf16, const int* tile_slot, const void* ybg, const float* dout,
+                                      const void* yrows, const float* a2, const float* b2, const int* pillar_cell, int M, int B, int H,
+                                      int W, int C, double* out , void* workspace, void* stream) {
+  GD_REQUIRE(dout != nullptr && yrows != nullptr && a2 != nullptr && b2 != nullptr, "border_sums_rows: dout, yrows, a2 and b2 are required");
+  return border_sums(Y, y_bf16, tile_slot, ybg, dout, yrows, a2, b2, pillar_cell, M, B, H, W, C, out, workspace, stream);
 }
 
 __global__ __launch_bounds__(256) void k_dec_region_S(const double* __restrict__ stats2, const float* __restrict__ ab2,
@@ -874,9 +908,11 @@
 }
 
 
+template <bool FUSED>
 __global__ __launch_bounds__(256) void k_decoder_dy(const unsigned short* __restrict__ Yc, const int* __restrict__ tile_list, int n_act,
                                                     const float* __restrict__ k0, const float* __restrict__ k1,
-                                                    const float* __restrict__ rows, const int* __restrict__ cell2pillar, int H, int W,
+                                                    const float* __restrict__ rows, const float* __restrict__ a2,
+                                                    const float* __restrict__ b2, const int* __restrict__ cell2pillar, int H, int W,
                                                     int TH, int TW, int C, unsigned short* __restrict__ dYc) {
   const unsigned cv = (unsigned)C >> 3;
   const unsigned total = (unsigned)n_act * GD_TILE_SITES * cv;
@@ -908,7 +944,19 @@
       const int p = cell2pillar[((long long)b * H + y) * W + x];
       if (p >= 0) {
         const float4 r0 = ((const float4*)rows)[((long long)p * C + c0) >> 2], r1 = ((const float4*)rows)[(((long long)p * C + c0) >> 2) + 1];
-        o[0] += r0.x; o[1] += r0.y; o[2] += r0.z; o[3] += r0.w; o[4] += r1.x; o[5] += r1.y; o[6] += r1.z; o[7] += r1.w;
+        float rv[8] = {r0.x, r0.y, r0.z, r0.w, r1.x, r1.y, r1.z, r1.w};
+        if (FUSED) {
+          float av[8], bv[8];
+          dec_ld8<false>(a2, c0, av);
+          dec_ld8<false>(b2, c0, bv);
+#pragma unroll
+          for (int j = 0; j < 8; ++j) {
+            const float dh = fmaf(av[j], yv[j], bv[j]) > 0.f ? rv[j] : 0.f;
+            rv[j] = fmaf(av[j], dh, fmaf(0.f, yv[j], 0.f));
+          }
+        }
+#pragma unroll
+        for (int j = 0; j < 8; ++j) o[j] += rv[j];
       }
       q.x = dec_f2bf(o[0]) | ((unsigned)dec_f2bf(o[1]) << 16);
       q.y = dec_f2bf(o[2]) | ((unsigned)dec_f2bf(o[3]) << 16);
@@ -918,17 +966,29 @@
     reinterpret_cast<uint4*>(dYc + row * C)[v] = q;
   }
 }
-extern "C" int gdmae_decoder_dy(const void* Yc, const int* tile_list, int n_act, const float* k0, const float* k1, const float* rows,
-                                const int* cell2pillar, int H, int W, int C, void* dYc, void* stream) {
+static int decoder_dy(const void* Yc, const int* tile_list, int n_act, const float* k0, const float* k1, const float* rows, const float* a2,
+                      const float* b2, const int* cell2pillar, int H, int W, int C, void* dYc, void* stream) {
   GD_REQUIRE(C % 8 == 0, "decoder_dy: C must be a multiple of 8");
   if (n_act <= 0) return 0;
   GD_REQUIRE((long long)n_act * GD_TILE_SITES * (C / 8) < (1ll << 31), "decoder_dy: active tiles x 64 x C / 8 must fit 31 bits");
   long long g = ((long long)n_act * GD_TILE_SITES * (C / 8) + 255) / 256;
   if (g > 65536) g = 65536;
-  hipLaunchKernelGGL(k_decoder_dy, dim3((int)g), dim3(256), 0, (hipStream_t)stream, (const unsigned short*)Yc, tile_list, n_act, k0, k1, rows,
-                     cell2pillar, H, W, (H + 7) / 8, (W + 7) / 8, C, (unsigned short*)dYc);
-  GD_LAUNCH_CHECK();
-  return 0;
+  if (a2) hipLaunchKernelGGL(k_decoder_dy<true>, dim3((int)g), dim3(256), 0, (hipStream_t)stream, (const unsigned short*)Yc, tile_list, n_act, k0,
+                             k1, rows, a2, b2, cell2pillar, H, W, (H + 7) / 8, (W + 7) / 8, C, (unsigned short*)dYc);
+  else hipLaunchKernelGGL(k_decoder_dy<false>, dim3((int)g), dim3(256), 0, (hipStream_t)stream, (const unsigned short*)Yc, tile_list, n_act, k0,
+                          k1, rows, a2, b2, cell2pillar, H, W, (H + 7) / 8, (W + 7) / 8, C, (unsigned short*)dYc);
+  GD_LAUNCH_CHECK();
+  return 0;
+}
+extern "C" int gdmae_decoder_dy(const void* Yc, const int* tile_list, int n_act, const float* k0, const float* k1, const float* rows,
+                                const int* cell2pillar, int H, int W, int C, void* dYc, void* stream) {
+  return decoder_dy(Yc, tile_list, n_act, k0, k1, rows, nullptr, nullptr, cell2pillar, H, W, C, dYc, stream);
+}
+extern "C" int gdmae_decoder_dy_rows(const void* Yc, const int* tile_list, int n_act, const float* k0, const float* k1, const float* dout,
+                                     const float* a2, const float* b2, const int* cell2pillar, int H, int W, int C, void* dYc,
+                                     void* stream) {
+  GD_REQUIRE(dout != nullptr && a2 != nullptr && b2 != nullptr, "decoder_dy_rows: dout, a2 and b2 are required");
+  return decoder_dy(Yc, tile_list, n_act, k0, k1, dout, a2, b2, cell2pillar, H, W, C, dYc, stream);
 }
 
 __global__ __launch_bounds__(256) void k_decoder_site_rulebook(const int* __restrict__ site, const int* __restrict__ n_dev, int sites_per_tok,
diff --git a/gd-mae_amd/gdmae_hip/decoder.py b/gd-mae_amd/gdmae_hip/decoder.py
--- a/gd-mae_amd/gdmae_hip/decoder.py
+++ b/gd-mae_amd/gdmae_hip/decoder.py
@@ -17,6 +17,8 @@
 
 CONV_BWD = os.environ.get("GDMAE_DEC_BWD", "implicit")
 BLOCK_BWD = os.environ.get("GDMAE_DEC_BLOCK", "1")
+DY_ROWS = os.environ.get("GDMAE_DEC_DY_ROWS", "1") != "0"
+GATHER_FUSED = os.environ.get("GDMAE_DEC_GATHER_FUSED", "1") != "0"
 
 
 
@@ -92,7 +94,7 @@
     tile_conv: Optional[TileConv] = None
 
 
-_Forward = namedtuple("_Forward", "y2 yrows stats2 ab2 mv2 Z tile_slot ybg bgz")
+_Forward = namedtuple("_Forward", "y2 yrows stats2 ab2 mv2 Z tile_slot ybg bgz out", defaults=(None,))
 
 
 def _forward_tiles(geom, pre_conv_hook, conv_w, gamma2, beta2, pillar_cell, Ps, widths, ab_l, bn2):
@@ -124,9 +126,15 @@
                L.ptr(ab2), L.ptr(mv2), L.ptr(ws), L.stream())
     M = pillar_cell.numel()
     yrows = torch.empty(M, C2, dtype=cdt, device=dev)
-    L.call("gdmae_tiles_gather_rows", L.ptr(y2), L.ptr(dt.tile_slot), L.ptr(ybg), L.ptr(pillar_cell), M, H, W, C2, 2,
-           L.ptr(yrows), L.stream())
-    return _Forward(y2, yrows, stats2, ab2, mv2, None, dt.tile_slot, ybg, bgz)
+    out = None
+    if GATHER_FUSED:
+        out = torch.empty(M, C2, dtype=torch.float32, device=dev)
+        L.call("gdmae_tiles_gather_rows_affine_relu", L.ptr(y2), L.ptr(dt.tile_slot), L.ptr(ybg), L.ptr(pillar_cell), M, H, W, C2,
+               L.ptr(ab2), L.ptr(ab2[C2:]), L.ptr(yrows), L.ptr(out), L.stream())
+    else:
+        L.call("gdmae_tiles_gather_rows", L.ptr(y2), L.ptr(dt.tile_slot), L.ptr(ybg), L.ptr(pillar_cell), M, H, W, C2, 2,
+               L.ptr(yrows), L.stream())
+    return _Forward(y2, yrows, stats2, ab2, mv2, None, dt.tile_slot, ybg, bgz, out)
 
 
 def _forward_dense_map(geom, conv_w, gamma2, beta2, pillar_cell, sites, Ps, widths, ab_l, bn2):
@@ -197,20 +205,30 @@
     L.call("gdmae_rows_bwd_stats", L.ptr(yrows), _bf(yrows), None, M, C2, L.ptr(ab2), L.ptr(ab2[C2:]), L.ptr(dout), 0, C2, 0,
            L.ptr(st2), L.ptr(ws), L.stream())
     dgamma2, dbeta2, k01 = gbn.bwd_coeffs(st2, 3, s.stats2, ab2, s.gamma2, R, None, direct)
-    zero = torch.zeros(2 * C2, dtype=torch.float32, device=dev)
-    rows = torch.empty(M, C2, dtype=torch.float32, device=dev)
+    return dout, st2, k01, dgamma2, dbeta2
+
+
+def _pillar_rows(s, dout):
+    yrows, ab2 = s.yrows, s.ab2
+    M, C2 = yrows.shape
+    zero = torch.zeros(2 * C2, dtype=torch.float32, device=yrows.device)
+    rows = torch.empty(M, C2, dtype=torch.float32, device=yrows.device)
     L.call("gdmae_rows_bwd", L.ptr(yrows), _bf(yrows), None, M, C2, L.ptr(ab2), L.ptr(ab2[C2:]), L.ptr(zero), L.ptr(zero[C2:]),
            L.ptr(dout), 0, C2, 0, L.ptr(rows), 0, L.stream())
-    return rows, st2, k01, dgamma2, dbeta2
-
-
-def _region_sums(s, rows, B, H, W):
+    return rows
+
+
+def _region_sums(s, rows, dout, B, H, W):
     y2 = s.y2
     C2 = y2.shape[1]
     reg = torch.empty(16, C2, dtype=torch.float64, device=y2.device)
     ws = torch.empty(L.load().gdmae_border_sums_workspace_bytes(B, C2), dtype=torch.uint8, device=y2.device)
-    L.call("gdmae_border_sums", L.ptr(y2), _bf(y2), L.ptr(s.tile_slot), L.ptr(s.ybg), L.ptr(rows), L.ptr(s.pillar_cell),
-           rows.shape[0], B, H, W, C2, L.ptr(reg), L.ptr(ws), L.stream())
+    if rows is None:
+        L.call("gdmae_border_sums_rows", L.ptr(y2), _bf(y2), L.ptr(s.tile_slot), L.ptr(s.ybg), L.ptr(dout), L.ptr(s.yrows), L.ptr(s.ab2),
+               L.ptr(s.ab2[C2:]), L.ptr(s.pillar_cell), dout.shape[0], B, H, W, C2, L.ptr(reg), L.ptr(ws), L.stream())
+    else:
+        L.call("gdmae_border_sums", L.ptr(y2), _bf(y2), L.ptr(s.tile_slot), L.ptr(s.ybg), L.ptr(rows), L.ptr(s.pillar_cell),
+               rows.shape[0], B, H, W, C2, L.ptr(reg), L.ptr(ws), L.stream())
     return reg
 
 
@@ -331,14 +349,17 @@
         else:
             f = _forward_dense_map(geom, conv_w, gamma2, beta2, pillar_cell, sites, Ps, widths, ab_l, bns[k])
         M, C2 = f.yrows.shape
-        out = torch.empty(M, C2, dtype=torch.float32, device=f.yrows.device)
-        L.call("gdmae_rows_affine_relu_scatter", L.ptr(f.yrows), _bf(f.yrows), None, M, C2, L.ptr(f.ab2), L.ptr(f.ab2[C2:]), L.ptr(out), 0,
-               C2, 0, L.stream())
+        out = f.out
+        if out is None:
+            out = torch.empty(M, C2, dtype=torch.float32, device=f.yrows.device)
+            L.call("gdmae_rows_affine_relu_scatter", L.ptr(f.yrows), _bf(f.yrows), None, M, C2, L.ptr(f.ab2), L.ptr(f.ab2[C2:]), L.ptr(out), 0,
+                   C2, 0, L.stream())
         _save(ctx, sites=sites, Ps=Ps, ab_l=ab_l, stats_l=stats_l, gammas=[g.detach() for g in gammas], Z=f.Z, y2=f.y2, bgz=f.bgz,
               yrows=f.yrows, ab2=f.ab2, stats2=f.stats2, pillar_cell=pillar_cell, cell2pillar=cell2pillar, gamma2=gamma2.detach(),
               conv_w=conv_w.detach(), tile_slot=f.tile_slot, ybg=f.ybg)
         ctx.geom, ctx.widths = geom, widths
         ctx.native_region, ctx.stage_bwd = _backward_schedule(geom, conv_w, sites, Ps, widths, f)
+        ctx.dy_rows = DY_ROWS and C2 % 8 == 0 and all(sb != "taps" for sb in ctx.stage_bwd)
         ctx.direct = [gbn.direct_pair(g, be) for g, be in zip(gammas, betas)] + [gbn.direct_pair(gamma2, beta2)]
         ctx.direct_w = ops.direct_grad(conv_w)
         ctx.conv_param = conv_w
@@ -354,8 +375,9 @@
         R, k = B * H * W, len(widths)
         b = _saved(ctx)
         b.H, b.W, b.cdt, b.widths = H, W, geom.cdt, widths
-        b.rows, st2, b.k01, dgamma2, dbeta2 = _bn2_backward(b, dout, R, ctx.direct[k])
-        reg = _region_sums(b, b.rows, B, H, W)
+        dout, st2, b.k01, dgamma2, dbeta2 = _bn2_backward(b, dout, R, ctx.direct[k])
+        b.rows = None if ctx.dy_rows else _pillar_rows(b, dout)
+        reg = _region_sums(b, b.rows, dout, B, H, W)
         tap_region, cnt = _region_consts(reg.device, B, H, W)
         algebra = region_algebra_native if ctx.native_region else region_algebra_torch
         S, b.tot, b.dWk, b.Wd = algebra(b.stats2, b.ab2, st2, b.k01, reg, tap_region, cnt, R, b.conv_w, b.bgz, geom.cdt)
@@ -363,14 +385,20 @@
             b.packed = packing.decoder_conv_packed(ctx.conv_param, widths, ctx.direct_w is not None)
             if b.packed is None:
                 stage_bwd = ["taps"] * k
+                if b.rows is None:
+                    b.rows = _pillar_rows(b, dout)
             else:
                 b.tiles, b.ups = geom.tile_conv.tiles, geom.tile_conv.ups
                 if b.tiles.nbr is None:
                     b.tiles.nbr = gplan.decoder_site_rulebooks(b.tiles, b.sites, b.ups)
                 C2 = b.y2.shape[1]
                 b.dYc = torch.empty_like(b.y2)
-                L.call("gdmae_decoder_dy", L.ptr(b.y2), L.ptr(b.tiles.tile_list), b.tiles.n_act, L.ptr(b.k01), L.ptr(b.k01[C2:]),
-                       L.ptr(b.rows), L.ptr(b.cell2pillar), H, W, C2, L.ptr(b.dYc), L.stream())
+                if b.rows is None:
+                    L.call("gdmae_decoder_dy_rows", L.ptr(b.y2), L.ptr(b.tiles.tile_list), b.tiles.n_act, L.ptr(b.k01), L.ptr(b.k01[C2:]),
+                           L.ptr(dout), L.ptr(b.ab2), L.ptr(b.ab2[C2:]), L.ptr(b.cell2pillar), H, W, C2, L.ptr(b.dYc), L.stream())
+                else:
+                    L.call("gdmae_decoder_dy", L.ptr(b.y2), L.ptr(b.tiles.tile_list), b.tiles.n_act, L.ptr(b.k01), L.ptr(b.k01[C2:]),
+                           L.ptr(b.rows), L.ptr(b.cell2pillar), H, W, C2, L.ptr(b.dYc), L.stream())
         grads = [None] * 8
         dW_rows = []
         col = 0
diff --git a/gd-mae_amd/gdmae_hip/lib.py b/gd-mae_amd/gdmae_hip/lib.py
--- a/gd-mae_amd/gdmae_hip/lib.py
+++ b/gd-mae_amd/gdmae_hip/lib.py
@@ -67,6 +67,7 @@
     "gdmae_bn_bwd_coeffs_rows": (_I, [_P, _I, _I, _P, _P, _P, _I, _D, _P, _P, _P, _I, _P, _P]),
     "gdmae_border_sums_workspace_bytes": (_Z, [_I, _I]),
     "gdmae_border_sums": (_I, [_P, _I, _P, _P, _P, _P, _I, _I, _I, _I, _I, _P, _P, _P]),
+    "gdmae_border_sums_rows": (_I, [_P, _I, _P, _P, _P, _P, _P, _P, _P, _I, _I, _I, _I, _I, _P, _P, _P]),
     "gdmae_conv3x3_grad_taps": (_I, [_P, _I, _P, _P, _P, _P, _P, _P, _P, _L, _I, _I, _I, _P, _P]),
     "gdmae_decoder_tiles_workspace_bytes": (_Z, [_I, _I, _I]),
     "gdmae_decoder_tiles": (_I, [_P, _P, _I, _I, _I, _I, _P, _P, _P, _P, _P]),
@@ -76,6 +77,7 @@
     "gdmae_conv3x3_tiles_fwd": (_I, [_P, _P, _P, _P, _P, _I, _P, _P, _P, _I, _I, _I, _I, _P, _P, _P, _D, _D, _P, _P, _P, _P, _P, _P,
                                      _P, _P]),
     "gdmae_tiles_gather_rows": (_I, [_P, _P, _P, _P, _L, _I, _I, _I, _I, _P, _P]),
+    "gdmae_tiles_gather_rows_affine_relu": (_I, [_P, _P, _P, _P, _L, _I, _I, _I, _P, _P, _P, _P, _P]),
     "gdmae_tiles_to_dense": (_I, [_P, _P, _P, _I, _I, _I, _I, _I, _P, _P]),
     "gdmae_tiles_to_dense_affine_relu": (_I, [_P, _P, _P, _I, _I, _I, _I, _P, _P, _P, _P]),
     "gdmae_rows_bwd": (_I, [_P, _I, _P, _L, _I, _P, _P, _P, _P, _P, _I, _I, _I, _P, _I, _P]),
@@ -130,6 +132,7 @@
     "gdmae_spconv_stat_rows": (_I, [_I, _I, _I]),
     "gdmae_spconv_stats": (_I, [_P, _I, _P, _P, _L, _I, _I, _P, _P, _P]),
     "gdmae_decoder_dy": (_I, [_P, _P, _I, _P, _P, _P, _P, _I, _I, _I, _P, _P]),
+    "gdmae_decoder_dy_rows": (_I, [_P, _P, _I, _P, _P, _P, _P, _P, _P, _I, _I, _I, _P, _P]),
     "gdmae_decoder_site_rulebook": (_I, [_P, _P, _I, _L, _P, _I, _I, _P, _P]),
     "gdmae_tap_dw_rows": (_L, [_L, _I, _I]),
     "gdmae_tap_dw_workspace_bytes": (_Z, [_L, _I, _I]),
@@ -169,6 +172,7 @@
     "gdmae_encoder_stage_fused": (_I, [_P, _I]),
     "gdmae_group_gt_points": (_I, [_P, _I, _P, _P, _P, _I, _I, _P, _P, _P, _P, _P]),
     "gdmae_chamfer": (_I, [_P, _P, _P, _I, _I, _I, _P, _P, _P]),
+    "gdmae_chamfer_points": (_I, [_P, _P, _I, _P, _P, _P, _P, _P, _P, _I, _I, _I, _P, _P, _P]),
     "gdmae_augment_collate_workspace_bytes": (_Z, [_L]),
     "gdmae_augment_collate": (_I, [_P, _L, _I, _P, _I, _P, _P, _P, _P, _P, _P]),
     "gdmae_gt_sample_workspace_bytes": (_Z, [_L]),
diff --git a/gd-mae_amd/gdmae_hip/ops.py b/gd-mae_amd/gdmae_hip/ops.py
--- a/gd-mae_amd/gdmae_hip/ops.py
+++ b/gd-mae_amd/gdmae_hip/ops.py
@@ -1,4 +1,6 @@
 from __future__ import annotations
+
+import os
 
 import torch
 
@@ -398,6 +400,44 @@
     return (gt, gi) if want_index else gt
 
 
+CHAMFER_POINTS = os.environ.get("GDMAE_CHAMFER_POINTS", "1") != "0"
+
+
+class LazyTargets:
+    __slots__ = ("vox", "K", "_gt")
+
+    def __init__(self, vox, K: int):
+        self.vox, self.K, self._gt = vox, int(K), None
+
+    @property
+    def shape(self):
+        return (self.vox.M, self.K, 3)
+
+    def materialize(self):
+        if self._gt is None:
+            self._gt = group_gt_points(self.vox, self.K)
+        return self._gt
+
+
+def chamfer_targets(vox, K: int, P1: int):
+    if CHAMFER_POINTS and P1 == 16 and 1 <= K <= 64 and vox.n_cols >= 4:
+        return LazyTargets(vox, K)
+    return group_gt_points(vox, K)
+
+
+class TargetDict(dict):
+
+    def raw(self, key):
+        return dict.__getitem__(self, key)
+
+    def __getitem__(self, key):
+        v = dict.__getitem__(self, key)
+        return v.materialize() if isinstance(v, LazyTargets) else v
+
+    def get(self, key, default=None):
+        return self[key] if key in self else default
+
+
 LAZY_SCALE = {}
 
 
@@ -407,12 +447,20 @@
     def forward(ctx, pred, gt, weights, lazy_scale=False):
         ctx.pred_dtype = pred.dtype
         ctx.lazy = bool(lazy_scale and pred.dtype == torch.float32)
-        pred, gt, weights = _f32c(pred.float()), _f32c(gt), _f32c(weights)
+        pred, weights = _f32c(pred.float()), _f32c(weights)
         M, P1, _ = pred.shape
-        P2 = gt.shape[1]
+        if isinstance(gt, LazyTargets) and not (P1 == 16 and gt.K <= 64 and gt.vox.M == M):
+            gt = gt.materialize()
         term = torch.empty(max(M, 1), dtype=torch.float32, device=pred.device)
         dpred = torch.empty_like(pred)
-        L.call("gdmae_chamfer", L.ptr(pred), L.ptr(gt), L.ptr(weights), M, P1, P2, L.ptr(term), L.ptr(dpred), L.stream())
+        if isinstance(gt, LazyTargets):
+            vox = gt.vox
+            L.call("gdmae_chamfer_points", L.ptr(pred), L.ptr(vox.points), vox.n_cols, L.ptr(vox.pt_off), L.ptr(vox.pillar_pts),
+                   L.ptr(vox.voxel_coords), L.host_f32(vox.lo), L.host_f32(vox.vs), L.ptr(weights), M, P1, gt.K, L.ptr(term), L.ptr(dpred),
+                   L.stream())
+        else:
+            gt = _f32c(gt)
+            L.call("gdmae_chamfer", L.ptr(pred), L.ptr(gt), L.ptr(weights), M, P1, gt.shape[1], L.ptr(term), L.ptr(dpred), L.stream())
         res = torch.empty(2, dtype=torch.float32, device=pred.device)
         L.call("gdmae_weighted_mean_finish", L.ptr(term), L.ptr(weights), M, L.ptr(res), L.stream())
         ctx.save_for_backward(dpred, res)
diff --git a/gd-mae_amd/pcdet/models/backbones_3d/spt_backbone_mae.py b/gd-mae_amd/pcdet/models/backbones_3d/spt_backbone_mae.py
--- a/gd-mae_amd/pcdet/models/backbones_3d/spt_backbone_mae.py
+++ b/gd-mae_amd/pcdet/models/backbones_3d/spt_backbone_mae.py
@@ -65,7 +65,8 @@
         r = self.forward_ret_dict
         pred = r['pred_points']
         lazy = bool(r.get('pred_lazy_scale', False)) and _only_the_pred_head_sees_the_gradient(pred)
-        return ops.ChamferLoss.apply(pred, r['gt_points'], r['mask'], lazy), tb_dict
+        gt = r.raw('gt_points') if isinstance(r, ops.TargetDict) else r['gt_points']
+        return ops.ChamferLoss.apply(pred, gt, r['mask'], lazy), tb_dict
 
     def forward(self, batch_dict):
         vox = batch_dict['_gdmae_vox']
@@ -135,7 +136,7 @@
 
     def target_assigner(self, batch_dict):
         vox = batch_dict['_gdmae_vox']
-        gt = ops.group_gt_points(vox, self.mask_cfg.NUM_GT_POINTS)
+        gt = ops.chamfer_targets(vox, self.mask_cfg.NUM_GT_POINTS, self.mask_cfg.NUM_PRD_POINTS)
         flat = gdec.pred_head(batch_dict['voxel_features'], self.decoder_pred)
-        return {'pred_points': flat.view(vox.M, -1, 3), 'gt_points': gt, 'mask': batch_dict['voxel_mae_mask'],
-                'pred_lazy_scale': bool(getattr(flat, '_gd_pred_head', False))}
+        return ops.TargetDict({'pred_points': flat.view(vox.M, -1, 3), 'gt_points': gt, 'mask': batch_dict['voxel_mae_mask'],
+                               'pred_lazy_scale': bool(getattr(flat, '_gd_pred_head', False))})
diff --git a/include/gdmae_hip.h b/include/gdmae_hip.h
--- a/include/gdmae_hip.h
+++ b/include/gdmae_hip.h
@@ -146,6 +146,9 @@
 size_t gdmae_border_sums_workspace_bytes(int B, int C);
 int gdmae_border_sums(const void* Y, int y_bf16, const int* tile_slot, const void* ybg, const float* rows,
                       const int* pillar_cell, int M, int B, int H, int W, int C, double* out, void* workspace, void* stream);
+int gdmae_border_sums_rows(const void* Y, int y_bf16, const int* tile_slot, const void* ybg, const float* dout, const void* yrows,
+                           const float* a2, const float* b2, const int* pillar_cell, int M, int B, int H, int W, int C, double* out,
+                           void* workspace, void* stream);
 
 size_t gdmae_decoder_tiles_workspace_bytes(int B, int H, int W);
 int gdmae_decoder_tiles(const int* const* maps, const int* strides, int k, int B, int H, int W, int* tile_slot, int* tile_list,
@@ -161,6 +164,8 @@
                             float* mv, void* workspace, void* stream);
 int gdmae_tiles_gather_rows(const void* Yc, const int* tile_slot, const void* ybg, const int* cell, long long n, int H, int W,
                             int C, int elem_bytes, void* out, void* stream);
+int gdmae_tiles_gather_rows_affine_relu(const void* Yc, const int* tile_slot, const void* ybg, const int* cell, long long n, int H, int W,
+                                        int C, const float* a, const float* b, void* yrows, float* out, void* stream);
 int gdmae_tiles_to_dense(const void* Yc, const int* tile_slot, const void* ybg, int B, int H, int W, int C, int elem_bytes,
                          void* out, void* stream);
 int gdmae_tiles_to_dense_affine_relu(const void* Yc, const int* tile_slot, const void* ybg, int B, int H, int W, int C, const float* a,
@@ -266,6 +271,8 @@
                        void* stream);
 int gdmae_decoder_dy(const void* Yc, const int* tile_list, int n_act, const float* k0, const float* k1, const float* rows,
                      const int* cell2pillar, int H, int W, int C, void* dYc, void* stream);
+int gdmae_decoder_dy_rows(const void* Yc, const int* tile_list, int n_act, const float* k0, const float* k1, const float* dout,
+                          const float* a2, const float* b2, const int* cell2pillar, int H, int W, int C, void* dYc, void* stream);
 int gdmae_decoder_site_rulebook(const int* site, const int* n_dev, int sites_per_tok, long long cap_sites, const int* tile_slot,
                                 int H, int W, int* nbr, void* stream);
 long long gdmae_tap_dw_rows(long long n, int M, int N);
@@ -378,6 +385,9 @@
                           float* gt_points, int* gt_index, void* stream);
 int gdmae_chamfer(const float* pred, const float* gt, const float* weights, int M, int P1, int P2, float* term,
                   float* dpred, void* stream);
+int gdmae_chamfer_points(const float* pred, const float* points, int n_cols, const int* pillar_pt_off, const int* pillar_pts,
+                         const long long* voxel_coords, const float* lo, const float* vs, const float* weights, int M, int P1, int P2,
+                         float* term, float* dpred, void* stream);
 
 size_t gdmae_augment_collate_workspace_bytes(long long n_raw);
 int gdmae_augment_collate(const float* raw, long long n_raw, int F, const int* frame_off, int B, const float* frame_params,
```

Result: faster. 1111, median of 6 (+1.2%).
